# RoyiAvital/QuadraticProgramSolver

Hardware: AMD Instinct MI355X
Metric: ADMM iterations/sec (higher is better)
Workload: dtype f64

## Files before the change

### quadraticprogramsolver_amd/csrc/k_loop.hip

```cpp
#include <cstdlib>

#include "qps_kernels.h"
#include "wave_reduce.h"
#include <hip/hip_ext.h>

namespace qps {

namespace {

template <typename T> __device__ __forceinline__ T wave_sum(T v) { return wave_sum_all(v); }
__device__ __forceinline__ unsigned long long absbits(double v) { return (unsigned long long)__double_as_longlong(fabs(v)); }
__device__ __forceinline__ unsigned long long wave_max_u64(unsigned long long v) {
#pragma unroll
    for (int o = 32; o > 0; o >>= 1) { unsigned long long t = __shfl_xor(v, o, 64); v = t > v ? t : v; }
    return v;
}

template <typename T, int RB, int TRI, int THREADS>
__global__ __launch_bounds__(THREADS) void k_gemv_rows(const T* __restrict__ S, int64_t ld, const T* __restrict__ v,
                                                   T* __restrict__ out, const T* __restrict__ out0, T alpha, T beta,
                                                   int r0, int c0, int c1, BatchStride bs) {
    using V = typename VecOf<T>::type;
    if (bs.active && !bs.active[blockIdx.y]) return;
    S += (int64_t)blockIdx.y * bs.mat; v += (int64_t)blockIdx.y * bs.vin; out += (int64_t)blockIdx.y * bs.vout;
    if (out0) out0 += (int64_t)blockIdx.y * bs.vout;
    constexpr int VN = VecOf<T>::N;
    constexpr int CHUNK = THREADS * VN;
    const int tid = threadIdx.x;
    const int rb = r0 + (TRI == 1 ? (int)(gridDim.x - 1 - blockIdx.x) : (int)blockIdx.x) * RB;
    int cb = c0, ce = c1;
    if (TRI == 1) ce = min(c1, rb + RB);
    if (TRI == 2) cb = max(c0, rb);
    T acc[RB];
#pragma unroll
    for (int i = 0; i < RB; ++i) acc[i] = T(0);
    const T* Srow = S + (int64_t)rb * ld;
#pragma unroll 4
    for (int c = cb + tid * VN; c < ce; c += CHUNK) {
        const V vv = *reinterpret_cast<const V*>(v + c);
        const T* vp = reinterpret_cast<const T*>(&vv);
#pragma unroll
        for (int i = 0; i < RB; ++i) {
            typedef T NV __attribute__((ext_vector_type(VN)));
            const NV* src = reinterpret_cast<const NV*>(Srow + (int64_t)i * ld + c);
            const NV a = (TRI == 0) ? __builtin_nontemporal_load(src) : *src;
            T ap[VN];
#pragma unroll
            for (int e = 0; e < VN; ++e) ap[e] = a[e];
#pragma unroll
            for (int e = 0; e < VN; ++e) {
                bool ok = true;
                if (TRI == 1) ok = (c + e) <= (rb + i);
                if (TRI == 2) ok = (c + e) >= (rb + i);
                acc[i] += ok ? ap[e] * vp[e] : T(0);
            }
        }
    }
    __shared__ T red[THREADS / 64][RB];
#pragma unroll
    for (int i = 0; i < RB; ++i) acc[i] = wave_sum(acc[i]);
    if ((tid & 63) == 0) {
#pragma unroll
        for (int i = 0; i < RB; ++i) red[tid >> 6][i] = acc[i];
    }
    __syncthreads();
    if (tid < RB) {
        T s = T(0);
#pragma unroll
        for (int w = 0; w < THREADS / 64; ++w) s += red[w][tid];
        T r = alpha * s;
        if (beta != T(0)) r += beta * out0[rb + tid];
        out[rb + tid] = r;
    }
}

constexpr int GC_RT = 32;
template <typename T>
__global__ __launch_bounds__(256) void k_gemv_cols(const T* __restrict__ S, int64_t ld, const T* __restrict__ va,
                                                   const T* __restrict__ vb, T ca, T cb, T* __restrict__ part,
                                                   int64_t part_ld, int ncols) {
    using V = typename VecOf<T>::type;
    constexpr int VN = VecOf<T>::N;
    const int c = (blockIdx.x * 256 + threadIdx.x) * VN;
    if (c >= ncols) return;
    const int rt = blockIdx.y;
    const int rbase = rt * GC_RT;
    T acc[VN];
#pragma unroll
    for (int e = 0; e < VN; ++e) acc[e] = T(0);
    const T* Sp = S + (int64_t)rbase * ld + c;
#pragma unroll 8
    for (int i = 0; i < GC_RT; ++i) {
        T w = ca * va[rbase + i];
        if (vb) w += cb * vb[rbase + i];
        typedef T NV __attribute__((ext_vector_type(VN)));
        const NV a = __builtin_nontemporal_load(reinterpret_cast<const NV*>(Sp + (int64_t)i * ld));
#pragma unroll
        for (int e = 0; e < VN; ++e) acc[e] += a[e] * w;
    }
    V o;
    T* op = reinterpret_cast<T*>(&o);
#pragma unroll
    for (int e = 0; e < VN; ++e) op[e] = acc[e];
    *reinterpret_cast<V*>(part + (int64_t)rt * part_ld + c) = o;
}

template <typename T>
__global__ __launch_bounds__(256) void k_colsum(const T* __restrict__ part, int64_t part_ld, int ntiles,
                                                const T* __restrict__ a0, T s0, const T* __restrict__ a1, T s1,
                                                T* __restrict__ out, int ncols, BatchStride bs) {
    using V = typename VecOf<T>::type;
    constexpr int VN = VecOf<T>::N;
    if (bs.active && !bs.active[blockIdx.y]) return;
    part += (int64_t)blockIdx.y * bs.mat; out += (int64_t)blockIdx.y * bs.vout;
    if (a0) a0 += (int64_t)blockIdx.y * bs.vin;
    if (a1) a1 += (int64_t)blockIdx.y * bs.vin;
    constexpr int COLS = 128 / (int)sizeof(T);
    constexpr int CL = COLS / VN;
    constexpr int TL = 256 / CL;
    const int cl = threadIdx.x % CL, tl = threadIdx.x / CL;
    const int c = blockIdx.x * COLS + cl * VN;
    T acc[VN];
#pragma unroll
    for (int e = 0; e < VN; ++e) acc[e] = T(0);
    if (c < ncols) {
        int t = tl;
        for (; t + 7 * TL < ntiles; t += 8 * TL) {
            V v[8];
#pragma unroll
            for (int j = 0; j < 8; ++j) v[j] = *reinterpret_cast<const V*>(part + (int64_t)(t + TL * j) * part_ld + c);
#pragma unroll
            for (int j = 0; j < 8; ++j) {
                const T* vp = reinterpret_cast<const T*>(&v[j]);
#pragma unroll
                for (int e = 0; e < VN; ++e) acc[e] += vp[e];
            }
        }
        for (; t < ntiles; t += TL) {
            const V v = *reinterpret_cast<const V*>(part + (int64_t)t * part_ld + c);
            const T* vp = reinterpret_cast<const T*>(&v);
#pragma unroll
            for (int e = 0; e < VN; ++e) acc[e] += vp[e];
        }
    }
    __shared__ T red[TL][COLS + 1];
#pragma unroll
    for (int e = 0; e < VN; ++e) red[tl][cl * VN + e] = acc[e];
    __syncthreads();
    constexpr int PL = 256 / COLS;
    static_assert(TL % PL == 0 && (PL == 16 || PL == 8), "slab lanes per output");
    const int o = threadIdx.x / PL, pl = threadIdx.x % PL;
    T s = T(0);
#pragma unroll
    for (int k = 0; k < TL / PL; ++k) s += red[pl * (TL / PL) + k][o];
    s = (PL == 16) ? row16_sum_last(s) : oct_sum_all(s);
    const int oc = blockIdx.x * COLS + o;
    if (pl == PL - 1 && oc < ncols) {
        T r = s;
        if (a0) r += s0 * a0[oc];
        if (a1) r += s1 * a1[oc];
        out[oc] = r;
    }
}

template <typename T>
__global__ __launch_bounds__(256) void k_admm_update(int NP, int MP, const T* __restrict__ xx, const T* __restrict__ zz,
                                                     T* __restrict__ x, T* __restrict__ xp, T* __restrict__ z,
                                                     T* __restrict__ zp, T* __restrict__ y, const T* __restrict__ l,
                                                     const T* __restrict__ u, T alpha, T rho) {
    const int i = blockIdx.x * 256 + threadIdx.x;
    const T alpha1 = T(1) - alpha, rho1 = T(1) / rho;
    if (i < NP) {
        const T xo = x[i];
        xp[i] = xo;
        x[i] = alpha * xx[i] + alpha1 * xo;
    }
    if (i < MP) {
        const T zo = z[i], yo = y[i], zt = zz[i];
        zp[i] = zo;
        T t = alpha * zt + alpha1 * zo + rho1 * yo;
        const T lo = l[i], hi = u[i];
        const T zn = t > hi ? hi : (t < lo ? lo : t);
        z[i] = zn;
        y[i] = yo + rho * (alpha * zt + alpha1 * zo - zn);
    }
}

template <typename T>
__global__ __launch_bounds__(256) void k_check_norms(int n, int m, const T* __restrict__ Ax, const T* __restrict__ Px,
                                                     const T* __restrict__ Aty, const T* __restrict__ q,
                                                     const T* __restrict__ x, const T* __restrict__ xp,
                                                     const T* __restrict__ z, const T* __restrict__ zp,
                                                     unsigned long long* __restrict__ slots, int dual_only, BatchStride bs) {
    if (bs.active && !bs.active[blockIdx.y]) return;
    {
        const int64_t on = (int64_t)blockIdx.y * bs.vin, om = (int64_t)blockIdx.y * bs.vout;
        Ax += om; z += om; zp += om; Px += on; Aty += on; q += on; x += on; xp += on; slots += (int64_t)blockIdx.y * 16;
    }
    unsigned long long v[9];
#pragma unroll
    for (int k = 0; k < 9; ++k) v[k] = 0ull;
    for (int i = blockIdx.x * 256 + threadIdx.x; i < max(n, m); i += gridDim.x * 256) {
        if (i < m && !dual_only) {
            const double ax = (double)Ax[i], zi = (double)z[i];
            v[0] = max(v[0], absbits((double)(Ax[i] - z[i])));
            v[2] = max(v[2], absbits(ax));
            v[3] = max(v[3], absbits(zi));
            v[8] = max(v[8], absbits((double)(z[i] - zp[i])));
        }
        if (i < n) {
            v[1] = max(v[1], absbits((double)(Px[i] + q[i] + Aty[i])));
            v[4] = max(v[4], absbits((double)Px[i]));
            v[5] = max(v[5], absbits((double)Aty[i]));
            v[6] = max(v[6], absbits((double)q[i]));
            if (!dual_only) v[7] = max(v[7], absbits((double)(x[i] - xp[i])));
        }
    }
#pragma unroll
    for (int k = 0; k < 9; ++k) {
        v[k] = wave_max_u64(v[k]);
        if ((threadIdx.x & 63) == 0 && v[k] != 0ull) atomicMax(&slots[k], v[k]);
    }
}

__device__ __forceinline__ double jmax(double a, double b) { return (isnan(a) || isnan(b)) ? (double)NAN : (a > b ? a : b); }

__global__ void k_check_decide(const unsigned long long* __restrict__ slots, double* __restrict__ res, CheckScalars cs,
                               const double* __restrict__ rho_arr, const double* __restrict__ rhorho_arr,
                               const int* __restrict__ active) {
    if (threadIdx.x != 0) return;
    const int b = blockIdx.x;
    if (active && !active[b]) return;
    slots += (int64_t)b * 16; res += (int64_t)b * 8;
    if (rho_arr) { cs.rho = rho_arr[b]; cs.rhorho = rhorho_arr[b]; cs.convFlag = 1; }
    double nv[9];
    for (int k = 0; k < 9; ++k) nv[k] = __longlong_as_double((long long)slots[k]);
    const double MIN_VAL_RHO = 1e-3, MAX_VAL_RHO = 1e6;
    const double normResPrim = nv[0], normResDual = nv[1];
    const double maxNormPrim = jmax(nv[2], nv[3]);
    const double maxNormDual = jmax(jmax(nv[4], nv[5]), nv[6]);
    double rhorho = cs.rhorho;
    if (cs.adptRho) {
        const double numeratorVal = normResPrim * maxNormDual;
        const double denominatorVal = normResDual * maxNormPrim;
        const double t = cs.rho * sqrt(numeratorVal / denominatorVal);
        rhorho = t > MAX_VAL_RHO ? MAX_VAL_RHO : (t < MIN_VAL_RHO ? MIN_VAL_RHO : t);
    }
    const double epsPrim = cs.epsAbs + cs.epsRel * maxNormPrim;
    const double epsDual = cs.epsAbs + cs.epsRel * maxNormDual;
    int flag = cs.convFlag;
    if ((normResPrim < epsPrim) && (normResDual < epsDual)) flag = 3;
    if ((nv[7] <= cs.epsAdmm) && (nv[8] <= cs.epsAdmm)) flag = 2;
    res[0] = normResPrim; res[1] = normResDual; res[2] = maxNormPrim; res[3] = maxNormDual;
    res[4] = rhorho; res[5] = (double)flag; res[6] = nv[7]; res[7] = nv[8];
}

template <typename T> __global__ void k_fill(T* p, int64_t n, T v) {
    int64_t i = (int64_t)blockIdx.x * 256 + threadIdx.x;
    if (i < n) p[i] = v;
}
template <typename T> __global__ void k_convert(const double* __restrict__ s, T* __restrict__ d, int64_t n) {
    int64_t i = (int64_t)blockIdx.x * 256 + threadIdx.x;
    if (i < n) d[i] = (T)s[i];
}
template <typename T> __global__ void k_convert_back(const T* __restrict__ s, double* __restrict__ d, int64_t n) {
    int64_t i = (int64_t)blockIdx.x * 256 + threadIdx.x;
    if (i < n) d[i] = (double)s[i];
}

}

static int env_int(const char* name, int dflt) { const char* e = getenv(name); return e ? atoi(e) : dflt; }

template <typename T, int RB, int TH>
static void gemv_rows_launch(hipStream_t st, const T* S, int64_t ld, const T* v, T* out, const T* out0, T alpha, T beta, int r0,
                             int r1, int c0, int c1, int tri, BatchStride bs) {
    dim3 grid((r1 - r0 + RB - 1) / RB, bs.count);
#define QPS_GR(TRI) hipLaunchKernelGGL((k_gemv_rows<T, RB, TRI, TH>), grid, dim3(TH), 0, st, S, ld, v, out, out0, alpha, beta, r0, c0, c1, bs)
    if (tri == 0) QPS_GR(0); else if (tri == 1) QPS_GR(1); else QPS_GR(2);
#undef QPS_GR
}

template <typename T>
void gemv_rows(hipStream_t st, const T* S, int64_t ld, const T* v, T* out, const T* out0, T alpha, T beta, int r0, int r1,
               int c0, int c1, int tri, BatchStride bs) {
    if (r1 <= r0) return;
    static const int wide_th = env_int("QPS_GEMV_WIDE_THREADS", 512);
    static const int wide_rb = env_int("QPS_GEMV_WIDE_RB", 2);
    const bool wide = (c1 - c0) >= 4 * 256 * VecOf<T>::N;
    if (!wide) { gemv_rows_launch<T, 4, 256>(st, S, ld, v, out, out0, alpha, beta, r0, r1, c0, c1, tri, bs); return; }
#define QPS_W(RB, TH) gemv_rows_launch<T, RB, TH>(st, S, ld, v, out, out0, alpha, beta, r0, r1, c0, c1, tri, bs)
    if (wide_th == 512) { if (wide_rb == 4) QPS_W(4, 512); else QPS_W(VecOf<T>::N == 2 ? 2 : 4, 512); }
    else if (wide_th == 256) { if (wide_rb == 4) QPS_W(4, 256); else QPS_W(VecOf<T>::N == 2 ? 2 : 4, 256); }
    else { if (wide_rb == 4) QPS_W(4, 1024); else QPS_W(VecOf<T>::N == 2 ? 2 : 4, 1024); }
#undef QPS_W
}

int gemv_cols_tiles(int nrows) { return (nrows + GC_RT - 1) / GC_RT; }

template <typename T>
int gemv_cols_partial(hipStream_t st, const T* S, int64_t ld, const T* va, const T* vb, T ca, T cb, T* part,
                      int64_t part_ld, int nrows, int ncols) {
    constexpr int VN = VecOf<T>::N;
    const int tiles = gemv_cols_tiles(nrows);
    if (tiles == 0) return 0;
    dim3 grid((ncols + 256 * VN - 1) / (256 * VN), tiles), block(256);
    hipLaunchKernelGGL((k_gemv_cols<T>), grid, block, 0, st, S, ld, va, vb, ca, cb, part, part_ld, ncols);
    return tiles;
}

template <typename T>
void colsum(hipStream_t st, const T* part, int64_t part_ld, int ntiles, const T* a0, T s0, const T* a1, T s1, T* out,
            int ncols, BatchStride bs) {
    constexpr int cols_wg = 128 / (int)sizeof(T);
    if (g_launch_timing.start) {
        const LaunchTiming lt = g_launch_timing;
        g_launch_timing = LaunchTiming();
        hipExtLaunchKernelGGL((k_colsum<T>), dim3((ncols + cols_wg - 1) / cols_wg, bs.count), dim3(256), 0, st, lt.start, lt.stop, 0, part, part_ld, ntiles, a0, s0, a1, s1, out, ncols, bs);
        return;
    }
    hipLaunchKernelGGL((k_colsum<T>), dim3((ncols + cols_wg - 1) / cols_wg, bs.count), dim3(256), 0, st, part, part_ld, ntiles, a0, s0, a1, s1, out, ncols, bs);
}

template <typename T>
void admm_update(hipStream_t st, int NP, int MP, const T* xx, const T* zz, T* x, T* xp, T* z, T* zp, T* y, const T* l,
                 const T* u, T alpha, T rho) {
    const int N = NP > MP ? NP : MP;
    hipLaunchKernelGGL((k_admm_update<T>), dim3((N + 255) / 256), dim3(256), 0, st, NP, MP, xx, zz, x, xp, z, zp, y, l, u, alpha, rho);
}

template <typename T>
void check_convergence(hipStream_t st, int n, int m, const T* Ax, const T* Px, const T* Aty, const T* q, const T* x,
                       const T* xp, const T* z, const T* zp, unsigned long long* scratch, double* res_dev, CheckScalars cs,
                       int dual_only, BatchStride bs, const double* rho_arr, const double* rhorho_arr) {
    if (!dual_only) (void)hipMemsetAsync(scratch, 0, 16 * sizeof(unsigned long long) * bs.count, st);
    const int N = n > m ? n : m;
    int blocks = (N + 255) / 256;
    if (blocks > 1024) blocks = 1024;
    if (blocks < 1) blocks = 1;
    hipLaunchKernelGGL((k_check_norms<T>), dim3(blocks, bs.count), dim3(256), 0, st, n, m, Ax, Px, Aty, q, x, xp, z, zp, scratch, dual_only, bs);
    hipLaunchKernelGGL(k_check_decide, dim3(bs.count), dim3(64), 0, st, scratch, res_dev, cs, rho_arr, rhorho_arr, bs.active);
}

template <typename T> void fill(hipStream_t st, T* p, int64_t n, T v) {
    if (n <= 0) return;
    hipLaunchKernelGGL((k_fill<T>), dim3((unsigned)((n + 255) / 256)), dim3(256), 0, st, p, n, v);
}
template <typename T> void convert_copy(hipStream_t st, const double* src, T* dst, int64_t n) {
    if (n <= 0) return;
    hipLaunchKernelGGL((k_convert<T>), dim3((unsigned)((n + 255) / 256)), dim3(256), 0, st, src, dst, n);
}
template <typename T> void convert_back(hipStream_t st, const T* src, double* dst, int64_t n) {
    if (n <= 0) return;
    hipLaunchKernelGGL((k_convert_back<T>), dim3((unsigned)((n + 255) / 256)), dim3(256), 0, st, src, dst, n);
}

#define INST(T)                                                                                                              \
    template void gemv_rows<T>(hipStream_t, const T*, int64_t, const T*, T*, const T*, T, T, int, int, int, int, int, BatchStride); \
    template int gemv_cols_partial<T>(hipStream_t, const T*, int64_t, const T*, const T*, T, T, T*, int64_t, int, int);      \
    template void colsum<T>(hipStream_t, const T*, int64_t, int, const T*, T, const T*, T, T*, int, BatchStride);            \
    template void admm_update<T>(hipStream_t, int, int, const T*, const T*, T*, T*, T*, T*, T*, const T*, const T*, T, T);   \
    template void check_convergence<T>(hipStream_t, int, int, const T*, const T*, const T*, const T*, const T*, const T*,    \
                                       const T*, const T*, unsigned long long*, double*, CheckScalars, int, BatchStride,     \
                                       const double*, const double*);                                                        \
    template void fill<T>(hipStream_t, T*, int64_t, T);                                                                      \
    template void convert_copy<T>(hipStream_t, const double*, T*, int64_t);                                                  \
    template void convert_back<T>(hipStream_t, const T*, double*, int64_t);
INST(double)
INST(float)
#undef INST

}
```

### quadraticprogramsolver_amd/csrc/k_pass_kernel.h

```cpp
#pragma once
#include <cstdlib>

#include "qps_kernels.h"
#include "wave_reduce.h"
#include <hip/hip_ext.h>

namespace qps {

namespace {

__device__ __forceinline__ unsigned long long absbits(double v) { return (unsigned long long)__double_as_longlong(fabs(v)); }
__device__ __forceinline__ unsigned long long umax(unsigned long long a, unsigned long long b) { return a > b ? a : b; }

template <typename T, int THREADS, int KC, int R, bool CHECK>
struct Pass {
    using V = typename VecOf<T>::type;
    static constexpr int VN = VecOf<T>::N;
    static constexpr int CHUNK = THREADS * VN;
    static constexpr int WAVES = THREADS / 64;

    static __device__ __forceinline__ void load_tile(V (&a)[R][KC], const T* __restrict__ A, int64_t ld, int row, int NP, int tid) {
#pragma unroll
        for (int i = 0; i < R; ++i)
#pragma unroll
            for (int k = 0; k < KC; ++k) {
                const int c = tid * VN + k * CHUNK;
                if (c < NP) {
                    typedef T NV __attribute__((ext_vector_type(VN)));
                    const NV t = __builtin_nontemporal_load(reinterpret_cast<const NV*>(A + (int64_t)(row + i) * ld + c));
                    T* p = reinterpret_cast<T*>(&a[i][k]);
#pragma unroll
                    for (int e = 0; e < VN; ++e) p[e] = t[e];
                }
                else {
                    T* p = reinterpret_cast<T*>(&a[i][k]);
#pragma unroll
                    for (int e = 0; e < VN; ++e) p[e] = T(0);
                }
            }
    }
};

template <typename T, int THREADS, int KC, int R, bool CHECK, int MODE>
__global__ __launch_bounds__(THREADS) void k_apass(const T* __restrict__ A, int64_t ld, int NP, int MP, int rows_per_wg,
                                                   const T* __restrict__ xx, const T* __restrict__ x_old, T* __restrict__ x_new,
                                                   T* __restrict__ z, T* __restrict__ y, const T* __restrict__ l,
                                                   const T* __restrict__ u, T alpha, T rho, T* __restrict__ part,
                                                   T* __restrict__ part2, int64_t part_ld, unsigned long long* __restrict__ slots,
                                                   PassBatch pb) {
    using PS = Pass<T, THREADS, KC, R, CHECK>;
    if (pb.count > 1 || pb.active) {
        const int b = blockIdx.y;
        if (pb.active && !pb.active[b]) return;
        A += (int64_t)b * MP * ld; xx += (int64_t)b * NP; x_old += (int64_t)b * NP; x_new += (int64_t)b * NP;
        z += (int64_t)b * MP; y += (int64_t)b * MP; l += (int64_t)b * MP; u += (int64_t)b * MP;
        part += (int64_t)b * pb.slabs * part_ld; part2 += (int64_t)b * pb.slabs * part_ld; slots += (int64_t)b * 16;
        if (pb.rho_arr) rho = (T)pb.rho_arr[b];
    }
    using V = typename PS::V;
    constexpr int VN = PS::VN, CHUNK = PS::CHUNK, WAVES = PS::WAVES;
    const int tid = threadIdx.x, g = blockIdx.x;
    const int row0 = g * rows_per_wg;
    const int row1 = min(MP, row0 + rows_per_wg);
    const T alpha1 = T(1) - alpha, rho1 = T(1) / rho;

    __shared__ T red[WAVES][R];
    __shared__ T red2[WAVES][R];
    __shared__ T wsh[R];
    __shared__ T ysh[R];

    V xv[KC];
    V xn[CHECK ? KC : 1];
    unsigned long long mdx = 0ull;
#pragma unroll
    for (int k = 0; k < KC; ++k) {
        const int c = tid * VN + k * CHUNK;
        T* xp_ = reinterpret_cast<T*>(&xv[k]);
        if (c < NP) {
            xv[k] = *reinterpret_cast<const V*>(xx + c);
            if (CHECK) {
                const V xo = *reinterpret_cast<const V*>(x_old + c);
                const T* xop = reinterpret_cast<const T*>(&xo);
                V xnv;
                T* xnp = reinterpret_cast<T*>(&xnv);
#pragma unroll
                for (int e = 0; e < VN; ++e) {
                    xnp[e] = alpha * xp_[e] + alpha1 * xop[e];
                    if (CHECK) mdx = umax(mdx, absbits((double)(xnp[e] - xop[e])));
                }
                if (g == 0) *reinterpret_cast<V*>(x_new + c) = xnv;
                if (CHECK) xn[k] = xnv;
            }
        } else {
#pragma unroll
            for (int e = 0; e < VN; ++e) xp_[e] = T(0);
            if (CHECK) { T* q_ = reinterpret_cast<T*>(&xn[k]);
#pragma unroll
                for (int e = 0; e < VN; ++e) q_[e] = T(0); }
        }
    }
    if (CHECK && g == 0) {
#pragma unroll
        for (int o = 32; o > 0; o >>= 1) mdx = umax(mdx, (unsigned long long)__shfl_xor(mdx, o, 64));
        if ((tid & 63) == 0 && mdx) atomicMax(&slots[7], mdx);
    }

    T acc[KC][VN];
    T acc2[CHECK ? KC : 1][VN];
#pragma unroll
    for (int k = 0; k < KC; ++k)
#pragma unroll
        for (int e = 0; e < VN; ++e) { acc[k][e] = T(0); if (CHECK) acc2[k][e] = T(0); }

    unsigned long long m_res = 0ull, m_ax = 0ull, m_z = 0ull, m_dz = 0ull;

    V bufA[R][KC], bufB[R][KC];
    T zA = T(0), yA = T(0), lA = T(0), uA = T(0), zB = T(0), yB = T(0), lB = T(0), uB = T(0);

    auto prefetch_rows = [&](int row, T& zo, T& yo, T& lo, T& hi) {
        if (tid < R) { zo = z[row + tid]; yo = y[row + tid]; lo = l[row + tid]; hi = u[row + tid]; }
    };
    auto process = [&](V (&a)[R][KC], int row, T zo, T yo, T lo, T hi) {
        T d[R], d2[CHECK ? R : 1];
#pragma unroll
        for (int i = 0; i < R; ++i) {
            T s = T(0), s2 = T(0);
#pragma unroll
            for (int k = 0; k < KC; ++k) {
                const T* ap = reinterpret_cast<const T*>(&a[i][k]);
                const T* xp_ = reinterpret_cast<const T*>(&xv[k]);
                const T* xq_ = reinterpret_cast<const T*>(&xn[CHECK ? k : 0]);
#pragma unroll
                for (int e = 0; e < VN; ++e) { s += ap[e] * xp_[e]; if (CHECK) s2 += ap[e] * xq_[e]; }
            }
            d[i] = wave_sum_all(s);
            if (CHECK) d2[i] = wave_sum_all(s2);
        }
        if ((tid & 63) == 0) {
#pragma unroll
            for (int i = 0; i < R; ++i) { red[tid >> 6][i] = d[i]; if (CHECK) red2[tid >> 6][i] = d2[i]; }
        }
        __syncthreads();
        if (tid < R) {
            T zt = T(0), ax = T(0);
#pragma unroll
            for (int w = 0; w < WAVES; ++w) { zt += red[w][tid]; if (CHECK) ax += red2[w][tid]; }
            T zn, yn;
            if (MODE == 0) {
                const T t = alpha * zt + alpha1 * zo + rho1 * yo;
                zn = t > hi ? hi : (t < lo ? lo : t);
                yn = yo + rho * (alpha * zt + alpha1 * zo - zn);
                wsh[tid] = rho * zn - yn;
            } else if (MODE == 2) {
                zn = lo * zt - alpha * (lo * yo);
                yn = yo;
                wsh[tid] = lo * yo;
            } else {
                const T gb = lo, vr = zt;
                if (row + tid < pb.pq_me) {
                    zn = T(0);
                    yn = yo - rho * gb; yn += rho * vr;
                    wsh[tid] = rho * gb - yn;
                } else {
                    T sv = gb - rho1 * yo; sv += -vr; zn = sv > T(0) ? sv : T(0);
                    T zz_ = yo + rho * (zn - gb); zz_ += rho * vr; yn = zz_ > T(0) ? zz_ : T(0);
                    wsh[tid] = rho * (gb - zn) - yn;
                }
            }
            z[row + tid] = zn;
            if (MODE != 2) y[row + tid] = yn;
            if (CHECK) {
                ysh[tid] = yn;
                m_res = umax(m_res, absbits((double)(ax - zn)));
                m_ax = umax(m_ax, absbits((double)ax));
                m_z = umax(m_z, absbits((double)zn));
                m_dz = umax(m_dz, absbits((double)(zn - zo)));
            }
        }
        __syncthreads();
#pragma unroll
        for (int i = 0; i < R; ++i) {
            const T w = wsh[i];
            const T yw = CHECK ? ysh[i] : T(0);
#pragma unroll
            for (int k = 0; k < KC; ++k) {
                const T* ap = reinterpret_cast<const T*>(&a[i][k]);
#pragma unroll
                for (int e = 0; e < VN; ++e) { acc[k][e] += ap[e] * w; if (CHECK) acc2[k][e] += ap[e] * yw; }
            }
        }
    };

    if (row0 < row1) {
        PS::load_tile(bufA, A, ld, row0, NP, tid);
        prefetch_rows(row0, zA, yA, lA, uA);
    }
    for (int row = row0; row < row1; row += 2 * R) {
        const bool haveB = row + R < row1;
        if (haveB) { PS::load_tile(bufB, A, ld, row + R, NP, tid); prefetch_rows(row + R, zB, yB, lB, uB); }
        process(bufA, row, zA, yA, lA, uA);
        if (haveB) {
            if (row + 2 * R < row1) { PS::load_tile(bufA, A, ld, row + 2 * R, NP, tid); prefetch_rows(row + 2 * R, zA, yA, lA, uA); }
            process(bufB, row + R, zB, yB, lB, uB);
        }
    }

    if (!CHECK && MODE != 2 && g == 0) {
        V xo[KC];
#pragma unroll
        for (int k = 0; k < KC; ++k) xo[k] = *reinterpret_cast<const V*>(x_old + min(tid * VN + k * CHUNK, NP - VN));
#pragma unroll
        for (int k = 0; k < KC; ++k) {
            const int c = tid * VN + k * CHUNK;
            if (c < NP) {
                const T* xp_ = reinterpret_cast<const T*>(&xv[k]);
                const T* xop = reinterpret_cast<const T*>(&xo[k]);
                V xnv; T* xnp = reinterpret_cast<T*>(&xnv);
#pragma unroll
                for (int e = 0; e < VN; ++e) xnp[e] = alpha * xp_[e] + alpha1 * xop[e];
                *reinterpret_cast<V*>(x_new + c) = xnv;
            }
        }
    }

#pragma unroll
    for (int k = 0; k < KC; ++k) {
        const int c = tid * VN + k * CHUNK;
        if (c < NP) {
            V o; T* op = reinterpret_cast<T*>(&o);
#pragma unroll
            for (int e = 0; e < VN; ++e) op[e] = acc[k][e];
#if QPS_NT_SLABS
            { typedef T NVS __attribute__((ext_vector_type(VN))); NVS ov;
#pragma unroll
              for (int e = 0; e < VN; ++e) ov[e] = op[e];
              __builtin_nontemporal_store(ov, reinterpret_cast<NVS*>(part + (int64_t)g * part_ld + c)); }
#else
            *reinterpret_cast<V*>(part + (int64_t)g * part_ld + c) = o;
#endif
            if (CHECK) {
#pragma unroll
                for (int e = 0; e < VN; ++e) op[e] = acc2[k][e];
                *reinterpret_cast<V*>(part2 + (int64_t)g * part_ld + c) = o;
            }
        }
    }
    if (CHECK && tid < R) {
        if (m_res) atomicMax(&slots[0], m_res);
        if (m_ax) atomicMax(&slots[2], m_ax);
        if (m_z) atomicMax(&slots[3], m_z);
        if (m_dz) atomicMax(&slots[8], m_dz);
    }
}

template <typename T, int THREADS, int KC, int R, int RC, int MODE>
void launch_pass(hipStream_t st, bool check, int G, const T* A, int64_t ld, int NP, int MP, int rows_per_wg, const T* xx,
                 const T* x_old, T* x_new, T* z, T* y, const T* l, const T* u, T alpha, T rho, T* part, T* part2,
                 int64_t part_ld, unsigned long long* slots, PassBatch pb) {
    if constexpr (MODE == 0) {
        if (check) {
            if (g_launch_timing.start) {
                const LaunchTiming lt = g_launch_timing;
                g_launch_timing = LaunchTiming();
                hipExtLaunchKernelGGL((k_apass<T, THREADS, KC, RC, true, 0>), dim3(G, pb.count), dim3(THREADS), 0, st, lt.start, lt.stop, 0, A, ld, NP, MP, rows_per_wg, xx, x_old, x_new, z, y, l, u, alpha, rho, part, part2, part_ld, slots, pb);
            } else {
                hipLaunchKernelGGL((k_apass<T, THREADS, KC, RC, true, 0>), dim3(G, pb.count), dim3(THREADS), 0, st, A, ld, NP, MP, rows_per_wg, xx, x_old, x_new, z, y, l, u, alpha, rho, part, part2, part_ld, slots, pb);
            }
            return;
        }
    }
    if (g_launch_timing.start) {
        const LaunchTiming lt = g_launch_timing;
        g_launch_timing = LaunchTiming();
        hipExtLaunchKernelGGL((k_apass<T, THREADS, KC, R, false, MODE>), dim3(G, pb.count), dim3(THREADS), 0, st, lt.start, lt.stop, 0, A, ld, NP, MP, rows_per_wg, xx, x_old, x_new, z, y, l, u, alpha, rho, part, part2, part_ld, slots, pb);
        return;
    }
    hipLaunchKernelGGL((k_apass<T, THREADS, KC, R, false, MODE>), dim3(G, pb.count), dim3(THREADS), 0, st, A, ld, NP, MP, rows_per_wg, xx, x_old, x_new, z, y, l, u, alpha, rho, part, part2, part_ld, slots, pb);
}

}

}
```

### quadraticprogramsolver_amd/csrc/k_sparse.hip

```cpp
#include <algorithm>

#include "qps_internal.h"
#include "qps_kernels.h"
#include "qps_ldl.h"
#include "qps_polish.h"
#include "qps_proxqp.h"
#include "k_proxqp_rows.h"
#include "wave_reduce.h"
#include "spmv_layout.h"
#include <hip/hip_ext.h>

namespace qps {

namespace {

struct CgState { double res2, prev2, tol, uc; int iters, done, maxiter, pad; };
using layout::STREAM_NNZ;

__device__ __forceinline__ double block_sum_256(double v, double* sh) {
    v = wave_sum_all(v);
    if ((threadIdx.x & 63) == 0) sh[threadIdx.x >> 6] = v;
    __syncthreads();
    const double r = sh[0] + sh[1] + sh[2] + sh[3];
    __syncthreads();
// ... 487 lines not shown
    const int row = (prow ? blockIdx.x : blockIdx.x - nbn) * 256 + threadIdx.x;
    double d = 0.0;
    if (row < (prow ? n : m)) {
        const T* p0 = pp + (prow ? 0 : n) + row;
        T s = T(0);
#pragma unroll 8
        for (int b = 0; b < nblk; ++b) s += p0[(int64_t)b * stride];
        if (prow) { const T ui = u[row]; pu[row] = s; d = (double)ui * ((double)s + (double)sigma * (double)ui); }
        else { v[row] = s; d = (double)rho * (double)s * (double)s; }
    }
    d = block_sum_256(d, sh);
    if (threadIdx.x == 0) part_uc[blockIdx.x] = d;
}
template <typename T>
__global__ __launch_bounds__(256) void k_cg_combine_update(int n, const T* __restrict__ pu, const T* __restrict__ pat, int nblk, int64_t stride, T rho, T sigma,
                                                           const T* __restrict__ u, int nparts_uc, const double* __restrict__ part_uc, T* __restrict__ x,
                                                           T* __restrict__ r, double* __restrict__ part_rr, const CgState* __restrict__ st) {
    if (st->done) return;
    __shared__ double sh[4];
    double uc = 0.0;
    for (int i = threadIdx.x; i < nparts_uc; i += 256) uc += part_uc[i];
    uc = block_sum_256(uc, sh);
    const T alpha = (T)(st->res2 / uc);
    const int i = blockIdx.x * 256 + threadIdx.x;
    double d = 0.0;
    if (i < n) {
        T s = T(0);
#pragma unroll 8
        for (int b = 0; b < nblk; ++b) s += pat[(int64_t)b * stride + i];
        const T ui = u[i];
        const T c = pu[i] + rho * s + sigma * ui;
        x[i] += alpha * ui;
        const T ri = r[i] - alpha * c;
        r[i] = ri;
        d = (double)ri * (double)ri;
    }
    d = block_sum_256(d, sh);
    if (threadIdx.x == 0) part_rr[blockIdx.x] = d;
}

template <typename T>
__global__ __launch_bounds__(256) void k_cg_init(int n, const T* __restrict__ b, const T* __restrict__ c, T* __restrict__ r,
                                                 T* __restrict__ u, double* __restrict__ partial) {
    __shared__ double sh[4];
    const int i = blockIdx.x * 256 + threadIdx.x;
    double d = 0.0;
    if (i < n) { const T ri = b[i] - c[i]; r[i] = ri; u[i] = T(0); d = (double)ri * (double)ri; }
    d = block_sum_256(d, sh);
    if (threadIdx.x == 0) partial[blockIdx.x] = d;
}
__global__ __launch_bounds__(256) void k_cg_init_final(int nparts, const double* __restrict__ partial, CgState* st, double abstol, double reltol, int maxiter) {
    __shared__ double sh[4];
    double d = 0.0;
    for (int i = threadIdx.x; i < nparts; i += 256) d += partial[i];
    d = block_sum_256(d, sh);
    if (threadIdx.x == 0) {
        const double residual = sqrt(d);
        st->res2 = d; st->prev2 = 1.0;
        st->tol = fmax(reltol * residual, abstol);
        st->iters = 0; st->maxiter = maxiter;
        st->done = (!(residual <= st->tol) && 0 < maxiter) ? 0 : 1;
    }
}
template <typename T>
__global__ __launch_bounds__(256) void k_cg_update_xr(int n, int nparts_uc, const double* __restrict__ partial_uc,
                                                      const T* __restrict__ u, const T* __restrict__ c, T* __restrict__ x,
                                                      T* __restrict__ r, double* __restrict__ partial_rr, const CgState* __restrict__ st) {
    if (st->done) return;
    __shared__ double sh[4];
    double uc = 0.0;
    for (int i = threadIdx.x; i < nparts_uc; i += 256) uc += partial_uc[i];
    uc = block_sum_256(uc, sh);
    const T alpha = (T)(st->res2 / uc);
    const int i = blockIdx.x * 256 + threadIdx.x;
    double d = 0.0;
    if (i < n) {
        x[i] += alpha * u[i];
        const T ri = r[i] - alpha * c[i];
        r[i] = ri;
        d = (double)ri * (double)ri;
    }
    d = block_sum_256(d, sh);
    if (threadIdx.x == 0) partial_rr[blockIdx.x] = d;
}
__global__ __launch_bounds__(256) void k_cg_finish(int nparts, const double* __restrict__ partial_rr, CgState* st) {
    if (st->done) return;
    __shared__ double sh[4];
    double d = 0.0;
    for (int i = threadIdx.x; i < nparts; i += 256) d += partial_rr[i];
    d = block_sum_256(d, sh);
    if (threadIdx.x == 0) {
        st->prev2 = st->res2; st->res2 = d; st->iters += 1;
        const double residual = sqrt(d);
        if (residual <= st->tol || st->iters >= st->maxiter) st->done = 1;
    }
}
template <typename T>
__global__ __launch_bounds__(256) void k_cg_next_u(int n, int nparts, const double* __restrict__ partial_rr, const T* __restrict__ r,
                                                   T* __restrict__ u, const CgState* __restrict__ cur, CgState* __restrict__ nxt, int first) {
    __shared__ double sh[4];
    if (cur->done) { if (blockIdx.x == 0 && threadIdx.x == 0) *nxt = *cur; return; }
    double res2 = cur->res2, prev2 = cur->prev2; int iters = cur->iters, done = 0;
    if (!first) {
        double d = 0.0;
        for (int i = threadIdx.x; i < nparts; i += 256) d += partial_rr[i];
        d = block_sum_256(d, sh);
        prev2 = res2; res2 = d; iters += 1;
        if (sqrt(d) <= cur->tol || iters >= cur->maxiter) done = 1;
    }
    if (blockIdx.x == 0 && threadIdx.x == 0) {
        CgState s = *cur; s.res2 = res2; s.prev2 = prev2; s.iters = iters; s.done = done; *nxt = s;
    }
    if (done) return;
    const T beta = (T)(res2 / prev2);
    const int i = blockIdx.x * 256 + threadIdx.x;
    if (i < n) u[i] = r[i] + beta * u[i];
}
template <typename T>
__global__ __launch_bounds__(256) void k_axpby(int n, T a, const T* __restrict__ x, T b, const T* __restrict__ y, T* __restrict__ out) {
    const int i = blockIdx.x * 256 + threadIdx.x;
    if (i < n) out[i] = a * x[i] + b * y[i];
}

template <typename T>
__global__ __launch_bounds__(256) void k_build_reduced(int64_t nnz, const T* __restrict__ vP, const T* __restrict__ vAA, const T* __restrict__ dg, T sigma, T rho, T* __restrict__ out) {
    const int64_t i = (int64_t)blockIdx.x * 256 + threadIdx.x;
    if (i < nnz) out[i] = vP[i] + sigma * dg[i] + rho * vAA[i];
}
template <typename T>
__global__ __launch_bounds__(256) void k_refresh_values(int64_t count, const int* __restrict__ src, const T* __restrict__ va, T* __restrict__ dst) {
    const int64_t i = (int64_t)blockIdx.x * 256 + threadIdx.x;
    if (i < count) { const int k = src[i]; dst[i] = k >= 0 ? va[k] : T(0); }
}

struct Csr {
    int nrows = 0; int64_t nnz = 0; int* rp = nullptr; int* ci = nullptr; void* va = nullptr; int* rb = nullptr; int nblocks = 0;
    bool blocked = false; int ncols = 0, nblk = 0, wpb = 0; int* brp = nullptr; unsigned short* bci = nullptr; void* bva = nullptr;
    int* task_ptr = nullptr; int4* tasks = nullptr; int per = 1, lpr4 = 0; void* partial = nullptr;
    int* lr_ptr = nullptr; int4* lr_desc = nullptr;
    bool sell = false; int nsl = 0, win = layout::SIGMA, nwin = 0, staged = 0; int* wg_ptr = nullptr; int* sl_off = nullptr; unsigned short* sl_perm = nullptr; void* s_cols = nullptr; void* s_vals = nullptr;
    int* src = nullptr; int64_t src_n = 0; int* lsrc = nullptr; int64_t lsrc_n = 0;
};

template <typename T> struct SparseSolver : SolverBase {
    StreamLease lease; DeviceOwner mem; std::unique_ptr<StagedUploader> up;
    Csr A, At, P, PA;
    Csr Lm; T *L_vP = nullptr, *L_vAA = nullptr, *L_dg = nullptr;
    int explicit_state = 0;
    bool cg_explicit = false; bool L_valid = false; double L_rho = 0, L_sigma = 0; int num_L_builds = 0;
    T *q = nullptr, *l = nullptr, *u = nullptr, *x = nullptr, *xp = nullptr, *z = nullptr, *zp = nullptr, *y = nullptr;
    T *xx = nullptr, *zz = nullptr, *w = nullptr, *tt = nullptr, *cu = nullptr, *cu2 = nullptr, *cr = nullptr, *cc = nullptr, *tm = nullptr;
    T *Ax = nullptr, *Px = nullptr, *Aty = nullptr;
    double *part_uc = nullptr, *part_rr = nullptr; int part_uc_cap = 0; CgState* state = nullptr; CgState* state_host = nullptr;
    unsigned long long* scratch = nullptr; double* res_dev = nullptr; double* res_host = nullptr; double* stage = nullptr;
    int nb_n = 0, nb_op = 0; int64_t cg_total = 0; int last_cg = 4;
    double eps_pcg = 1e-6; int itr_pcg = 1000;
    int cat_spmv, cat_op, cat_vec, cat_chk, cat_ldl, cat_pa = 0, cat_at = 0; int prof_calls = 0;
    std::vector<int64_t> hPcp, hPri, hAcp, hAri; std::vector<double> hPnz, hAnz;
    std::unique_ptr<SparseLdl<T>> ldl; bool ldl_valid = false; double ldl_rho = 0, ldl_sigma = 0; int plugin_kind = QPS_LINSYS_CG;
    int num_factorizations = 0; bool ldl_unfit = false;
    struct IterGraph { double rho, sigma, alpha; hipGraphExec_t exec; };
    std::vector<IterGraph> graphs; bool graphs_disabled = false;
    void drop_graphs() { for (auto& gr : graphs) (void)hipGraphExecDestroy(gr.exec); graphs.clear(); }
    hipGraphExec_t iter_graph(double rho, double sigma, double alpha) {
        for (auto& gr : graphs) if (gr.rho == rho && gr.sigma == sigma && gr.alpha == alpha) return gr.exec;
        if (graphs_disabled) return nullptr;
        if (graphs.size() >= 8) drop_graphs();
        hipGraph_t graph = nullptr; hipGraphExec_t exec = nullptr;
        if (hipStreamBeginCapture(st, hipStreamCaptureModeThreadLocal) != hipSuccess) { (void)hipGetLastError(); graphs_disabled = true; return nullptr; }
        ldl->iterate(x, xp, q, z, zp, y, l, u, alpha, rho, sigma, true);
        if (hipStreamEndCapture(st, &graph) != hipSuccess || graph == nullptr) { (void)hipGetLastError(); graphs_disabled = true; return nullptr; }
        const hipError_t e = hipGraphInstantiate(&exec, graph, nullptr, nullptr, 0);
        (void)hipGraphDestroy(graph);
        if (e != hipSuccess) { (void)hipGetLastError(); graphs_disabled = true; return nullptr; }
        graphs.push_back({rho, sigma, alpha, exec});
        return exec;
    }

    template <typename V> V* upload_array(const std::vector<V>& v, int64_t min_count = 1) {
        V* d = mem.dalloc<V>(std::max<int64_t>((int64_t)v.size(), min_count), st);
        if (!v.empty()) up->copy(d, v.data(), sizeof(V) * v.size());
        return d;
    }
    void build_blocked(Csr& M, const layout::CsrHost& H, bool with_src = false) {
        static const int wgs_env = [] { const char* e = getenv("QPS_SPMV_WGS"); return e ? atoi(e) : 0; }();
        const int wgs = wgs_env > 0 ? wgs_env : 512;
        M.ncols = H.ncols;
        const char* e = getenv("QPS_SPMV_SELL");
        if (!(e && atoi(e) == 0)) {
            layout::SellLayout<T> L;
            const char* es = getenv("QPS_SPMV_STAGED");
            if (layout::build_sell<T>(H, wgs, L, with_src, !(es && atoi(es) == 0))) {
                M.nblk = L.nblk; M.nsl = L.nsl; M.wpb = L.wpb; M.win = L.win; M.nwin = L.nwin; M.staged = L.staged;
                if (with_src) { M.src = upload_array(L.src); M.src_n = (int64_t)L.src.size(); M.lsrc = upload_array(L.lsrc); M.lsrc_n = (int64_t)L.lsrc.size(); }
                M.s_cols = upload_array(L.cols); M.s_vals = upload_array(L.vals);
                M.bci = upload_array(L.lci); M.bva = upload_array(L.lva);
                M.sl_off = upload_array(L.sl_off); M.sl_perm = upload_array(L.perm); M.wg_ptr = upload_array(L.wg_ptr);
                M.lr_ptr = upload_array(L.lr_ptr); M.lr_desc = reinterpret_cast<int4*>(upload_array(L.lr));
                M.partial = mem.dalloc<T>((int64_t)L.nblk * H.nrows + 64, st);
                M.blocked = true; M.sell = true;
                return;
            }
        }
        layout::TaskLayout<T> L;
        try { layout::build_tasks<T>(H, wgs, L, with_src); }
        catch (const std::length_error& ex) { throw QpsError(QPS_ERR_BAD_DIMENSION, ex.what()); }
        M.nblk = L.nblk; M.wpb = L.wpb; M.per = L.per; M.lpr4 = L.lpr4;
        if (with_src) { M.src = upload_array(L.src); M.src_n = (int64_t)L.src.size(); }
        M.brp = upload_array(L.brp); M.bci = upload_array(L.bci); M.bva = upload_array(L.bva);
        M.task_ptr = upload_array(L.task_ptr); M.tasks = reinterpret_cast<int4*>(upload_array(L.tasks));
        M.lr_ptr = upload_array(L.lr_ptr); M.lr_desc = reinterpret_cast<int4*>(upload_array(L.lr));
        M.partial = mem.dalloc<T>((int64_t)L.nblk * H.nrows + 64, st);
        M.blocked = true;
    }
    void upload_csr(Csr& M, const layout::CsrHost& H, bool with_src = false) {
        M.nrows = H.nrows; M.nnz = (int64_t)H.ci.size();
        {
            const char* e = getenv("QPS_SPMV_BLOCKED");
            const int64_t nblk_ = (H.ncols + BlkOf<T>::CB - 1) / BlkOf<T>::CB;
            const bool want = e ? atoi(e) != 0 : (M.nnz >= 200000 && nblk_ * (int64_t)H.nrows <= M.nnz);
            if (want && H.nrows > 0 && H.ncols > 0) build_blocked(M, H, with_src);
        }
        M.rp = upload_array(H.rp); M.ci = upload_array(H.ci);
        {
            std::vector<T> v(H.va.begin(), H.va.end());
            M.va = upload_array(v);
        }
        const std::vector<int> rbv = layout::stream_row_blocks(H);
        M.nblocks = (int)rbv.size() - 1;
        M.rb = upload_array(rbv);
    }
    void upload_vec(const double* h, T* d, int64_t count) { HIPC(upload_staged<T>(st, stage, h, d, count)); }
    void download_vec(const T* d, double* h, int64_t count) { HIPC(download_staged<T>(st, stage, d, h, count)); }
    bool explicit_prepare(bool forced) {
        if (explicit_state != 0) {
            if (forced && explicit_state < 0) throw QpsError(QPS_ERR_UNSUPPORTED, "QPS_LINSYS_CG_EXPLICIT: the reduced matrix of this handle cannot be formed (too many entries, or the handle's "
                                                                                  "host copies were released to the direct plugin before the first CG request)");
            return explicit_state > 0;
        }
        explicit_state = -1;
        if (hPcp.empty() || hAcp.empty()) { if (forced) return explicit_prepare(true); return false; }
        const int64_t pnnz = (int64_t)hPri.size(), annz = (int64_t)hAri.size();
        layout::CsrHost Ph, Ah, Ath, Lh; std::vector<double> vAA, dg;
        try {
            Ph = layout::csc_as_transposed_csr(n, n, hPcp, hPri, hPnz);
            layout::csc_to_csr_pair(m, n, hAcp, hAri, hAnz, Ah, Ath);
            if (!forced && layout::ata_work(Ah) > 16 * (pnnz + annz)) return false;
            const int64_t cap = forced ? 1900000000LL : (3 * (pnnz + 2 * annz)) / 2 + n;
            if (!layout::reduced_matrix(Ph, Ah, Ath, cap, Lh, vAA, dg)) { if (forced) return explicit_prepare(true); return false; }
        } catch (const std::length_error& ex) { throw QpsError(QPS_ERR_BAD_DIMENSION, ex.what()); }
        up.reset(new StagedUploader(st));
        upload_csr(Lm, Lh, true);
        std::vector<T> t1(Lh.va.begin(), Lh.va.end()), t2(vAA.begin(), vAA.end()), t3(dg.begin(), dg.end());
        L_vP = upload_array(t1); L_vAA = upload_array(t2); L_dg = upload_array(t3);
        up.reset();
        HIPC(hipStreamSynchronize(st));
        if (dot_parts(Lm) + 64 > part_uc_cap) {
            mem.release(part_uc); part_uc = nullptr;
            part_uc_cap = dot_parts(Lm) + 64; part_uc = mem.dalloc<double>(part_uc_cap, st);
        }
        explicit_state = 1; L_valid = false;
        return true;
    }
    void reduced_values(double rho, double sigma) {
        if (L_valid && L_rho == rho && L_sigma == sigma) return;
        const int64_t nnz = Lm.nnz;
        if (nnz > 0) hipLaunchKernelGGL((k_build_reduced<T>), dim3((unsigned)((nnz + 255) / 256)), dim3(256), 0, st, nnz, L_vP, L_vAA, L_dg, (T)sigma, (T)rho, static_cast<T*>(Lm.va));
        if (Lm.blocked) {
            T* main_vals = static_cast<T*>(Lm.sell ? Lm.s_vals : Lm.bva);
            if (Lm.src_n > 0) hipLaunchKernelGGL((k_refresh_values<T>), dim3((unsigned)((Lm.src_n + 255) / 256)), dim3(256), 0, st, Lm.src_n, Lm.src, static_cast<const T*>(Lm.va), main_vals);
            if (Lm.sell && Lm.lsrc_n > 0)
                hipLaunchKernelGGL((k_refresh_values<T>), dim3((unsigned)((Lm.lsrc_n + 255) / 256)), dim3(256), 0, st, Lm.lsrc_n, Lm.lsrc, static_cast<const T*>(Lm.va), static_cast<T*>(Lm.bva));
        }
        L_valid = true; L_rho = rho; L_sigma = sigma; ++num_L_builds;
    }
    int resolve_cg(int linsys, double rho, double sigma) {
        const char* e = getenv("QPS_CG_EXPLICIT");
        cg_explicit = linsys == QPS_LINSYS_CG_EXPLICIT ? explicit_prepare(true) : (!(e && atoi(e) == 0) && explicit_prepare(false));
        if (cg_explicit) reduced_values(rho, sigma);
        return QPS_LINSYS_CG;
    }
    int resolve_kind(int linsys, double rho, double sigma, bool force) {
        int kind = linsys;
        if (linsys == QPS_LINSYS_AUTO) kind = qps_linsys_auto(n, m, P.nnz, A.nnz, 1);
        if (kind != QPS_LINSYS_KKT_LDL) return resolve_cg(linsys, rho, sigma);
        if (ldl_unfit && linsys == QPS_LINSYS_AUTO) return resolve_cg(linsys, rho, sigma);
        try { ldl_prepare(rho, sigma, force); }
        catch (const QpsError& e) {
            if (linsys == QPS_LINSYS_AUTO && e.code == QPS_ERR_UNSUPPORTED) { ldl_unfit = true; return resolve_cg(linsys, rho, sigma); }
            throw;
        }
        return QPS_LINSYS_KKT_LDL;
    }
    void ldl_prepare(double rho, double sigma, bool force) {
        if (!ldl) {
            if (n + m > 2000000000LL) throw QpsError(QPS_ERR_BAD_DIMENSION, "KKT matrix too large for the sparse direct plugin");
            const char *e1 = getenv("QPS_LDL_MAX_TAIL"), *e2 = getenv("QPS_LDL_MIN_LEVEL"), *e3 = getenv("QPS_LDL_MAX_LEVELS");
            const int max_tail = e1 ? atoi(e1) : 8192, min_level = e2 ? atoi(e2) : 64, max_levels = e3 ? atoi(e3) : 4096;
            LdlSymbolic sym;
            try { sym = ldl_analyze((int)n, (int)m, hPcp.data(), hPri.data(), hAcp.data(), hAri.data(), 0, max_tail, min_level, max_levels); }
            catch (const std::runtime_error& e) { throw QpsError(QPS_ERR_UNSUPPORTED, e.what()); }
            ldl = make_sparse_ldl<T>(st, std::move(sym), hPnz.data(), (int64_t)hPnz.size(), hAnz.data(), (int64_t)hAnz.size());
            ldl_valid = false;
            for (auto* v : {&hPcp, &hPri, &hAcp, &hAri}) std::vector<int64_t>().swap(*v);
            std::vector<double>().swap(hPnz); std::vector<double>().swap(hAnz);
        }
        if (force || !ldl_valid || ldl_rho != rho || ldl_sigma != sigma) {
            ldl_valid = false;
            ++num_factorizations;
            ldl->factorize(rho, sigma);
            ldl_valid = true; ldl_rho = rho; ldl_sigma = sigma;
        }
    }

    SparseSolver(int dev, int64_t n_, int64_t m_, int dt, const int64_t* Pcp, const int64_t* Pri, const double* Pnz,
                 const int64_t* Acp, const int64_t* Ari, const double* Anz, const double* qh, const double* lh, const double* uh, int base) {
        device = dev; n = n_; m = m_; dtype = dt; sparse = true;
        HIPC(hipSetDevice(device));
        st = prof.st = lease.acquire(device);
        void* const pinned = lease.res.pinned;
        up.reset(new StagedUploader(st));
        if (Pcp[n] - base > 2000000000LL || Acp[n] - base > 2000000000LL) throw QpsError(QPS_ERR_BAD_DIMENSION, "more than 2^31 non-zeros");
        layout::canonical_csc(n, Pcp, Pri, Pnz, base, hPcp, hPri, hPnz);
        layout::canonical_csc(n, Acp, Ari, Anz, base, hAcp, hAri, hAnz);
        const int64_t pnnz = (int64_t)hPri.size(), annz = (int64_t)hAri.size();
        layout::CsrHost Ph, Ah, Ath;
        try {
            Ph = layout::csc_as_transposed_csr(n, n, hPcp, hPri, hPnz);
            layout::csc_to_csr_pair(m, n, hAcp, hAri, hAnz, Ah, Ath);
        } catch (const std::length_error& ex) { throw QpsError(QPS_ERR_BAD_DIMENSION, ex.what()); }
        upload_csr(P, Ph);
        upload_csr(At, Ath);
        upload_csr(A, Ah);
        const char* fuse_env = getenv("QPS_SPMV_FUSEPA");
        if (m > 0 && P.blocked && A.blocked && At.blocked && pnnz + annz < 2000000000LL && !(fuse_env && atoi(fuse_env) == 0)) {
            const layout::CsrHost Sh = layout::stack_rows(Ph, Ah);
            PA.nrows = (int)(n + m); PA.nnz = pnnz + annz;
            build_blocked(PA, Sh);
        }
        const int64_t nn = n + 64, mm = m + 64;
        q = mem.dalloc<T>(nn, st); x = mem.dalloc<T>(nn, st); xp = mem.dalloc<T>(nn, st); xx = mem.dalloc<T>(nn, st); tt = mem.dalloc<T>(nn, st);
        cu = mem.dalloc<T>(nn, st); cu2 = mem.dalloc<T>(nn, st); cr = mem.dalloc<T>(nn, st); cc = mem.dalloc<T>(nn, st); Px = mem.dalloc<T>(nn, st); Aty = mem.dalloc<T>(nn, st);
        l = mem.dalloc<T>(mm, st); u = mem.dalloc<T>(mm, st); z = mem.dalloc<T>(mm, st); zp = mem.dalloc<T>(mm, st); y = mem.dalloc<T>(mm, st); zz = mem.dalloc<T>(mm, st);
        w = mem.dalloc<T>(mm, st); tm = mem.dalloc<T>(mm, st); Ax = mem.dalloc<T>(mm, st);
        nb_n = (int)((n + 255) / 256);
        part_uc_cap = std::max(std::max(At.nblocks, P.nblocks), nb_n + (int)((m + 255) / 256)) + 64;
        part_uc = mem.dalloc<double>(part_uc_cap, st); part_rr = mem.dalloc<double>(nb_n + 64, st);
        state = reinterpret_cast<CgState*>(mem.dalloc<double>(16, st));
        state_host = reinterpret_cast<CgState*>(pinned);
        scratch = mem.dalloc<unsigned long long>(16, st); res_dev = mem.dalloc<double>(16, st);
        res_host = reinterpret_cast<double*>(static_cast<char*>(pinned) + 128);
        stage = mem.dalloc<double>(std::max(nn, mm) + 64, st);
        upload_vec(qh, q, n); upload_vec(lh, l, m); upload_vec(uh, u, m);
        const double s = sizeof(T);
        auto spmv_bytes = [&](const Csr& M, int cols) { return (double)M.nnz * (s + 4) + M.nrows * 4.0 + s * (M.nrows + cols); };
        cat_spmv = prof.category("spmv(A / A')", 0.5 * (spmv_bytes(A, (int)n) + spmv_bytes(At, (int)m)));
        cat_op = prof.category("cg_iteration(A u, P u + rho A'. + sigma u, axpys)", spmv_bytes(A, (int)n) + spmv_bytes(At, (int)m) + spmv_bytes(P, (int)n) + s * 10.0 * n);
        cat_vec = prof.category("admm_update", s * (3.0 * n + 7.0 * m));
        cat_chk = prof.category("check_convergence", spmv_bytes(A, (int)n) + spmv_bytes(At, (int)m) + spmv_bytes(P, (int)n));
        cat_ldl = prof.category("kkt_ldl_solve(rhs, level sweeps, dense tail, post)", 0.0);
        cat_pa = prof.category("spmv_blk([P;A] u, x block in LDS)", (double)(pnnz + annz) * (s + 4) + (double)(n + m) * 4.0 + s * (double)(n + m + n));
        cat_at = prof.category("spmv_blk(A' v, x block in LDS)", spmv_bytes(At, (int)m));
        up.reset();
    }
    ~SparseSolver() override {
        (void)hipSetDevice(device);
        (void)hipStreamSynchronize(st);
        drop_graphs();
        prof.release_events();
    }

    void spmv(const Csr& M, const T* xin, T* out, T a, const T* v0, T b0, const T* v1, T b1, const CgState* stt,
              const T* dotv = nullptr, double* partial = nullptr) {
        if (M.nblocks <= 0) return;
        if (M.blocked) {
            spmv_blk(M, xin, stt);
            hipLaunchKernelGGL((k_spmv_combine<T>), dim3((M.nrows + 255) / 256), dim3(256), 0, st, M.nrows, static_cast<const T*>(M.partial), M.nblk, (int64_t)M.nrows, a,
                               (const T*)nullptr, 0, (int64_t)0, T(0), v0, b0, v1, b1, out, dotv, partial, stt);
            return;
        }
        hipLaunchKernelGGL((k_spmv_stream<T>), dim3(M.nblocks), dim3(256), 0, st, M.rb, M.rp, M.ci, static_cast<const T*>(M.va), xin, out, a,
                           v0, b0, v1, b1, dotv, partial, stt);
    }
    void spmv_blk(const Csr& M, const T* xin, const CgState* stt, CgFuse<T> fu = CgFuse<T>()) {
        const LaunchTiming lt = g_launch_timing;
        g_launch_timing = LaunchTiming();
        if (M.sell) {
            const SellDims sd{M.nrows, M.ncols, M.nsl, M.wpb, M.win, M.nwin, M.staged};
            using CV = typename SellOf<T>::CV; using V = typename VecOf<T>::type;
            if (lt.start) hipExtLaunchKernelGGL((k_spmv_sell<T>), dim3(M.wpb, M.nblk), dim3(BTHREADS), 0, st, lt.start, lt.stop, 0, sd, M.wg_ptr, M.sl_off, M.sl_perm,
                                                static_cast<const CV*>(M.s_cols), static_cast<const V*>(M.s_vals), M.bci, static_cast<const T*>(M.bva), M.lr_ptr, M.lr_desc, xin,
                                                static_cast<T*>(M.partial), stt, fu);
            else hipLaunchKernelGGL((k_spmv_sell<T>), dim3(M.wpb, M.nblk), dim3(BTHREADS), 0, st, sd, M.wg_ptr, M.sl_off, M.sl_perm, static_cast<const CV*>(M.s_cols),
                                    static_cast<const V*>(M.s_vals), M.bci, static_cast<const T*>(M.bva), M.lr_ptr, M.lr_desc, xin, static_cast<T*>(M.partial), stt, fu);
            return;
        }
#define QPS_BLK(LPR)                                                                                                                        \
        do {                                                                                                                                \
            if (lt.start) hipExtLaunchKernelGGL((k_spmv_blk<T, LPR>), dim3(M.wpb, M.nblk), dim3(BTHREADS), 0, st, lt.start, lt.stop, 0, M.nrows, M.ncols, M.task_ptr, \
                                                M.tasks, M.per, M.brp, M.bci, static_cast<const T*>(M.bva), M.lr_ptr, M.lr_desc, xin, static_cast<T*>(M.partial), stt, fu); \
            else hipLaunchKernelGGL((k_spmv_blk<T, LPR>), dim3(M.wpb, M.nblk), dim3(BTHREADS), 0, st, M.nrows, M.ncols, M.task_ptr, M.tasks, M.per, M.brp, M.bci, \
                                    static_cast<const T*>(M.bva), M.lr_ptr, M.lr_desc, xin, static_cast<T*>(M.partial), stt, fu);             \
        } while (0)
        if (M.lpr4) QPS_BLK(4); else QPS_BLK(8);
#undef QPS_BLK
    }
    int dot_parts(const Csr& M) const { return M.blocked ? (M.nrows + 255) / 256 : M.nblocks; }
    void op_reduced(const T* uin, T* cout, double rho, double sigma, double* partial, const CgState* stt) {
        if (m > 0 && P.blocked && A.blocked && At.blocked) {
            spmv_blk(P, uin, stt);
            spmv(A, uin, tm, T(1), nullptr, T(0), nullptr, T(0), stt);
            spmv_blk(At, tm, stt);
            hipLaunchKernelGGL((k_spmv_combine<T>), dim3(nb_n), dim3(256), 0, st, (int)n, static_cast<const T*>(P.partial), P.nblk, (int64_t)n, T(1),
                               static_cast<const T*>(At.partial), At.nblk, (int64_t)n, (T)rho, uin, (T)sigma, (const T*)nullptr, T(0), cout, partial ? uin : nullptr, partial, stt);
            return;
        }
        spmv(P, uin, cout, T(1), uin, (T)sigma, nullptr, T(0), stt, (m > 0) ? nullptr : uin, (m > 0) ? nullptr : partial);
        if (m > 0) {
            spmv(A, uin, tm, T(1), nullptr, T(0), nullptr, T(0), stt);
            spmv(At, tm, cout, (T)rho, cout, T(1), nullptr, T(0), stt, uin, partial);
        }
    }
    int op_parts() const { return (m > 0 && P.blocked && A.blocked && At.blocked) ? nb_n : (m > 0 ? dot_parts(At) : dot_parts(P)); }

    int cg(double rho, double sigma) {
        CgState* slot[2] = {state, state + 1};
        int cur = 0;
        auto apply_op = [&](const T* uin, T* cout, double* partial, const CgState* stt) {
            if (cg_explicit) spmv(Lm, uin, cout, T(1), nullptr, T(0), nullptr, T(0), stt, partial ? uin : nullptr, partial);
            else op_reduced(uin, cout, rho, sigma, partial, stt);
        };
        const int parts_op = cg_explicit ? dot_parts(Lm) : op_parts();
        const bool fused_pa = PA.blocked && !cg_explicit;
        apply_op(xx, cc, nullptr, nullptr);
        T* ub[2] = {cu, cu2}; int ui = 0;
        hipLaunchKernelGGL((k_cg_init<T>), dim3(nb_n), dim3(256), 0, st, (int)n, tt, cc, cr, ub[ui], part_rr);
        hipLaunchKernelGGL(k_cg_init_final, dim3(1), dim3(256), 0, st, nb_n, part_rr, slot[cur], eps_pcg,
                           sizeof(T) == 8 ? 1.4901161193847656e-08 : 3.4526698300124393e-04, itr_pcg);
        HIPC(hipMemcpyAsync(state_host + 1, slot[cur], sizeof(CgState), hipMemcpyDeviceToHost, st));
        int launched = 0, batch = std::max(1, std::min(last_cg, 64));
        for (;;) {
            for (int b = 0; b < batch; ++b) {
                ProfScope ps(prof, cat_op, 2);
                if (fused_pa) {
                    CgFuse<T> fu; fu.r = cr; fu.uold = ub[ui]; fu.unew = ub[ui ^ 1]; fu.part_rr = part_rr; fu.nparts = nb_n;
                    fu.cur = slot[cur]; fu.nxt = slot[cur ^ 1]; fu.first = b == 0 ? 1 : 0;
                    const bool sample = prof.level == 2 || (prof.level == 1 && b == 0 && launched == 0 && prof_calls % 8 == 0);
                    { ProfLaunchScope ps2(prof, cat_pa, sample ? 1 : 3); spmv_blk(PA, cr, nullptr, fu); }
                    cur ^= 1; ui ^= 1;
                    const T* pp = static_cast<const T*>(PA.partial);
                    const int nb_m = (int)((m + 255) / 256);
                    hipLaunchKernelGGL((k_cg_combine_pa<T>), dim3((unsigned)(nb_n + nb_m)), dim3(256), 0, st, (int)n, (int)m, nb_n, pp, PA.nblk, (int64_t)(n + m), ub[ui],
                                       (T)sigma, (T)rho, cc, tm, part_uc, slot[cur]);
                    { ProfLaunchScope ps2(prof, cat_at, sample ? 1 : 3); spmv_blk(At, tm, slot[cur]); }
                    hipLaunchKernelGGL((k_cg_combine_update<T>), dim3(nb_n), dim3(256), 0, st, (int)n, cc, static_cast<const T*>(At.partial), At.nblk, (int64_t)n, (T)rho,
                                       (T)sigma, ub[ui], nb_n + nb_m, part_uc, xx, cr, part_rr, slot[cur]);
                    continue;
                } else {
                    hipLaunchKernelGGL((k_cg_next_u<T>), dim3(nb_n), dim3(256), 0, st, (int)n, nb_n, part_rr, cr, ub[ui], slot[cur], slot[cur ^ 1], b == 0 ? 1 : 0);
                    cur ^= 1;
                    apply_op(ub[ui], cc, part_uc, slot[cur]);
                }
                hipLaunchKernelGGL((k_cg_update_xr<T>), dim3(nb_n), dim3(256), 0, st, (int)n, parts_op, part_uc, ub[ui], cc, xx, cr, part_rr, slot[cur]);
            }
            hipLaunchKernelGGL(k_cg_finish, dim3(1), dim3(256), 0, st, nb_n, part_rr, slot[cur]);
            launched += batch;
            HIPC(hipMemcpyAsync(state_host, slot[cur], sizeof(CgState), hipMemcpyDeviceToHost, st));
            HIPC(hipStreamSynchronize(st));
            prof.harvest();
            if (state_host->done || launched >= itr_pcg) break;
            {
                const double r0 = std::sqrt(state_host[1].res2), r1 = std::sqrt(state_host->res2), tol = state_host->tol;
                int left = std::max(launched, 1);
                if (r1 > 0 && r0 > r1 && tol > 0 && r1 > tol) {
                    const double per_it = std::log(r0 / r1) / std::max(1, state_host->iters);
                    left = (int)std::ceil(std::log(r1 / tol) / per_it);
                }
                batch = std::max(1, std::min(std::min(std::max(left, 2), std::max(launched, 2)), std::min(64, itr_pcg - launched)));
            }
        }
        last_cg = state_host->iters;
        ++prof_calls;
        cg_total += state_host->iters;
        return state_host->iters;
    }

    void linear_solve(double rho, double sigma) {
        if (plugin_kind == QPS_LINSYS_KKT_LDL) {
            ProfScope ps(prof, cat_ldl, 2);
            ldl->solve(x, q, z, y, rho, sigma, xx, zz);
            return;
        }
        if (m > 0) hipLaunchKernelGGL((k_axpby<T>), dim3((unsigned)((m + 255) / 256)), dim3(256), 0, st, (int)m, (T)rho, z, T(-1), y, w);
        {
            ProfScope ps(prof, cat_spmv, 2);
            if (m > 0) spmv(At, w, tt, T(1), x, (T)sigma, q, T(-1), nullptr);
            else hipLaunchKernelGGL((k_axpby<T>), dim3(nb_n), dim3(256), 0, st, (int)n, (T)sigma, x, T(-1), q, tt);
        }
        cg(rho, sigma);
        {
            ProfScope ps(prof, cat_spmv, 2);
            if (m > 0) spmv(A, xx, zz, T(1), nullptr, T(0), nullptr, T(0), nullptr);
        }
    }

    void solve(double* xh, const qps_params& p, qps_info* info) override {
        HIPC(hipSetDevice(device));
        const double t0 = now_s();
        double rho = p.rho; const double sigma = p.sigma, alpha = p.alpha;
        eps_pcg = p.epsPcg; itr_pcg = p.numItrPcg;
        const double epsAdmm = std::fmin(p.epsAbs, p.epsRel) * 1e-2;
        int convFlag = QPS_CONV_NUM_ITR;
        if (p.linsys == QPS_LINSYS_CHOLESKY) throw QpsError(QPS_ERR_UNSUPPORTED, "CSR handles offer QPS_LINSYS_CG, QPS_LINSYS_CG_EXPLICIT and QPS_LINSYS_KKT_LDL (create with dense_path=1 for the reduced Cholesky path)");
        plugin_kind = resolve_kind(p.linsys, rho, sigma, !p.reuseFactor);
        upload_vec(xh, x, n);
        const size_t nb_ = sizeof(T) * (size_t)(n + 64), mb_ = sizeof(T) * (size_t)(m + 64);
        HIPC(hipMemsetAsync(xp, 0, nb_, st)); HIPC(hipMemsetAsync(xx, 0, nb_, st));
        HIPC(hipMemsetAsync(z, 0, mb_, st)); HIPC(hipMemsetAsync(y, 0, mb_, st)); HIPC(hipMemsetAsync(zp, 0, mb_, st));
        HIPC(hipStreamSynchronize(st));
        const double t1 = now_s();
        double rhorho = rho; int ii = 0, nref = 0; double resP = NAN, resD = NAN, tref = 0;
        cg_total = 0; last_cg = 4;
        const int NPv = (int)n, MPv = (int)m;
        static const int graph_env = [] { const char* e = getenv("QPS_GRAPH"); return e ? atoi(e) : -1; }();
        const bool use_graph = plugin_kind == QPS_LINSYS_KKT_LDL && prof.level == 0 && graph_env != 0;
        bool ldl_rhs_ready = false;
        for (ii = 1; ii <= p.numIterations; ++ii) {
            if (p.adptRho && ((rhorho * p.fctrRho < rho) || (rhorho > p.fctrRho * rho))) {
                rho = rhorho; ++nref;
                if (plugin_kind == QPS_LINSYS_CG && cg_explicit) { const double ta = now_s(); reduced_values(rho, sigma); tref += now_s() - ta; }
                if (plugin_kind == QPS_LINSYS_KKT_LDL) { const double ta = now_s(); ldl_prepare(rho, sigma, true); tref += now_s() - ta; ldl_rhs_ready = false; }
            }
            if (plugin_kind == QPS_LINSYS_KKT_LDL && prof.level < 2) {
                if (use_graph && ldl_rhs_ready && ii % p.numItrConv != 0) {
                    hipGraphExec_t ge = iter_graph(rho, sigma, alpha);
                    if (ge) { HIPC(hipGraphLaunch(ge, st)); continue; }
                }
                ldl->iterate(x, xp, q, z, zp, y, l, u, alpha, rho, sigma, ldl_rhs_ready);
                ldl_rhs_ready = true;
            } else {
            linear_solve(rho, sigma);
            {
                ProfScope ps(prof, cat_vec, 2);
                admm_update<T>(st, NPv, MPv, xx, zz, x, xp, z, zp, y, l, u, (T)alpha, (T)rho);
            }
            }
            if (ii % p.numItrConv == 0) {
                {
                    ProfScope ps(prof, cat_chk, 2);
                    if (m > 0) spmv(A, x, Ax, T(1), nullptr, T(0), nullptr, T(0), nullptr);
                    spmv(P, x, Px, T(1), nullptr, T(0), nullptr, T(0), nullptr);
                    if (m > 0) spmv(At, y, Aty, T(1), nullptr, T(0), nullptr, T(0), nullptr);
                    else HIPC(hipMemsetAsync(Aty, 0, nb_, st));
                    CheckScalars cs{p.epsAbs, p.epsRel, epsAdmm, rho, rhorho, p.adptRho, convFlag};
                    check_convergence<T>(st, (int)n, (int)m, Ax, Px, Aty, q, x, xp, z, zp, scratch, res_dev, cs);
                }
                HIPC(hipMemcpyAsync(res_host, res_dev, 8 * sizeof(double), hipMemcpyDeviceToHost, st));
                HIPC(hipStreamSynchronize(st));
                prof.harvest();
                resP = res_host[0]; resD = res_host[1]; rhorho = res_host[4]; convFlag = (int)res_host[5];
                if (convFlag != QPS_CONV_NUM_ITR) break;
            }
        }
        HIPC(hipStreamSynchronize(st));
        prof.harvest();
        const double t2 = now_s();
        PolishReport pr;
        if (p.polish) polish_device(p, &pr);
        download_vec(x, xh, n);
        if (info) {
            info->convFlag = convFlag; info->iterations = ii > p.numIterations ? p.numIterations : ii;
            info->numRefactor = nref; info->cgIterations = (int)cg_total; info->rhoFinal = rho; info->rhoProposed = rhorho;
            info->resPrim = resP; info->resDual = resD; info->tSetup = t1 - t0; info->tLoop = t2 - t1; info->tRefactor = tref;
            info->trsvBlock = 0; info->sweepVariant = 0; info->sweepGaveUp = 0; info->cgExplicit = (plugin_kind == QPS_LINSYS_CG && cg_explicit) ? 1 : 0;
            info->polishFlag = pr.flag; info->polishIterations = pr.minresIterations; info->tPolish = pr.seconds;
        }
    }
    void get_dual(double* zh, double* yh) override {
        HIPC(hipSetDevice(device));
        if (zh) download_vec(z, zh, m);
        if (yh) download_vec(y, yh, m);
    }
    void polish_device(const qps_params& p, PolishReport* pr) {
        PolishProduct<T> kmat = [&](const T* v, T delta, T* out, const T* mask, T* scratch) {
            spmv(P, v, out, T(1), v, delta, nullptr, T(0), nullptr);
            if (m <= 0) return;
            spmv(A, v, out + n, T(1), nullptr, T(0), nullptr, T(0), nullptr);
            polish_mask_rows<T>(st, (int)m, mask, v + n, delta, out + n, scratch);
            spmv(At, scratch, out, T(1), out, T(1), nullptr, T(0), nullptr);
        };
        polish_with<T>(st, n, m, (int)n, (int)m, q, l, u, y, x, p, pr, kmat);
    }
    void polish(double* xh, const double* yh, const qps_params& p, qps_polish_report* rep) override {
        HIPC(hipSetDevice(device));
        upload_vec(xh, x, n); upload_vec(yh, y, m);
        PolishReport pr;
        polish_device(p, &pr);
        download_vec(x, xh, n);
        if (rep) {
            rep->flag = pr.flag; rep->refinements = pr.refinements; rep->minresIterations = pr.minresIterations;
            rep->numActiveLower = pr.numLower; rep->numActiveUpper = pr.numUpper; rep->reserved0 = 0; rep->relres = pr.relres; rep->seconds = pr.seconds;
        }
    }
    void operator_apply(int op, const double* in, double* out, double rho, double sigma) override {
        HIPC(hipSetDevice(device));
        if (op == QPS_OP_AT) {
            upload_vec(in, w, m);
            if (m > 0) spmv(At, w, cc, T(1), nullptr, T(0), nullptr, T(0), nullptr); else HIPC(hipMemsetAsync(cc, 0, sizeof(T) * (size_t)(n + 64), st));
            download_vec(cc, out, n);
            return;
        }
        upload_vec(in, cu, n);
        if (op == QPS_OP_P) { spmv(P, cu, cc, T(1), nullptr, T(0), nullptr, T(0), nullptr); download_vec(cc, out, n); }
        else if (op == QPS_OP_A) { if (m > 0) spmv(A, cu, tm, T(1), nullptr, T(0), nullptr, T(0), nullptr); download_vec(tm, out, m); }
        else if (op == QPS_OP_PA) {
            if (PA.blocked) {
                spmv_blk(PA, cu, nullptr);
                DeviceOwner tmp_mem;
                T* both = tmp_mem.dalloc<T>(n + m + 64, st);
                hipLaunchKernelGGL((k_spmv_combine<T>), dim3((unsigned)((n + m + 255) / 256)), dim3(256), 0, st, (int)(n + m), static_cast<const T*>(PA.partial), PA.nblk, (int64_t)(n + m),
                                   T(1), (const T*)nullptr, 0, (int64_t)0, T(0), (const T*)nullptr, T(0), (const T*)nullptr, T(0), both, (const T*)nullptr, (double*)nullptr, (const CgState*)nullptr);
                download_vec(both, out, n); download_vec(both + n, out + n, m);
            } else {
                spmv(P, cu, cc, T(1), nullptr, T(0), nullptr, T(0), nullptr); download_vec(cc, out, n);
                if (m > 0) spmv(A, cu, tm, T(1), nullptr, T(0), nullptr, T(0), nullptr);
                download_vec(tm, out + n, m);
            }
        } else if (op == QPS_OP_REDUCED) { op_reduced(cu, cc, rho, sigma, nullptr, nullptr); download_vec(cc, out, n); }
        else throw QpsError(QPS_ERR_BAD_ARGUMENT, "unknown qps_operator_kind");
    }
    void linsys_set_cg(double eps, int itr) override { eps_pcg = eps; itr_pcg = itr; }
    void linsys_init(double rho, double sigma, int linsys, int) override {
        HIPC(hipSetDevice(device));
        if (linsys != QPS_LINSYS_AUTO && linsys != QPS_LINSYS_CG && linsys != QPS_LINSYS_KKT_LDL && linsys != QPS_LINSYS_CG_EXPLICIT)
            throw QpsError(QPS_ERR_UNSUPPORTED, "CSR handles offer QPS_LINSYS_CG, QPS_LINSYS_CG_EXPLICIT and QPS_LINSYS_KKT_LDL (create with dense_path=1 for the reduced Cholesky path)");
        plugin_kind = resolve_kind(linsys, rho, sigma, true);
        if (plugin_kind == QPS_LINSYS_KKT_LDL) return;
        HIPC(hipMemsetAsync(xx, 0, sizeof(T) * (size_t)(n + 64), st));
        cg_total = 0; last_cg = 4;
    }
    void linsys_solve(const double* xh, const double* zh, const double* yh, double rho, double sigma, int changed, double* xxh, double* zzh) override {
        HIPC(hipSetDevice(device));
        if (plugin_kind == QPS_LINSYS_KKT_LDL) {
            if (!ldl) throw QpsError(QPS_ERR_BAD_ARGUMENT, "qps_linsys_solve called before qps_linsys_init");
            if (changed) ldl_prepare(rho, sigma, true);
        }
        if (plugin_kind == QPS_LINSYS_CG && cg_explicit) reduced_values(rho, sigma);
        upload_vec(xh, x, n); upload_vec(zh, z, m); upload_vec(yh, y, m);
        linear_solve(rho, sigma);
        HIPC(hipStreamSynchronize(st));
        download_vec(xx, xxh, n); download_vec(zz, zzh, m);
    }
};


template <typename T> struct SparseProxQpSolver : ProxQpBase {
    std::unique_ptr<SparseSolver<T>> ss;
    DeviceOwner mem; hipStream_t st = nullptr;
    int mtot = 0;
    T *g = nullptr, *dual = nullptr, *slack = nullptr, *hvec = nullptr, *x = nullptr, *xx = nullptr, *v = nullptr, *de = nullptr, *di = nullptr;
    T *X1 = nullptr, *X2 = nullptr, *X3 = nullptr, *r1 = nullptr, *r2 = nullptr, *dx = nullptr, *dnu = nullptr, *zero_m = nullptr;
    unsigned long long* slots = nullptr; unsigned long long* slots_host = nullptr;
    std::vector<int64_t> kPcp, kPri, kAcp, kAri; std::vector<double> kPnz, kAnz;

    static dim3 g1(int64_t c) { return dim3((unsigned)((std::max<int64_t>(c, 1) + 255) / 256)); }

    SparseProxQpSolver(int dev, int64_t n_, int64_t me_, int64_t mi_, int dt, const int64_t* Pcp, const int64_t* Pri, const double* Pnz, const double* qh,
                       const int64_t* Acp, const int64_t* Ari, const double* Anz, const double* bh, const int64_t* Ccp, const int64_t* Cri, const double* Cnz,
                       const double* dh, int base) {
        device = dev; n = n_; me = me_; mi = mi_; mtot = (int)(me + mi);
        std::vector<int64_t> Gcp(n + 1, 0), Gri, P0cp(n + 1), P0ri((size_t)(Pcp[n] - base));
        std::vector<double> Gnz;
        for (int64_t j = 0; j <= n; ++j) P0cp[j] = Pcp[j] - base;
        for (size_t k = 0; k < P0ri.size(); ++k) P0ri[k] = Pri[k] - base;
        for (int64_t j = 0; j < n; ++j) {
            if (me > 0) for (int64_t k = Acp[j] - base; k < Acp[j + 1] - base; ++k) { Gri.push_back(Ari[k] - base); Gnz.push_back(Anz[k]); }
            if (mi > 0) for (int64_t k = Ccp[j] - base; k < Ccp[j + 1] - base; ++k) { Gri.push_back(Cri[k] - base + me); Gnz.push_back(Cnz[k]); }
            Gcp[j + 1] = (int64_t)Gri.size();
        }
        std::vector<double> zeros((size_t)std::max(mtot, 1), 0.0), gh((size_t)std::max(mtot, 1), 0.0);
        for (int64_t i = 0; i < me; ++i) gh[i] = bh[i];
        for (int64_t i = 0; i < mi; ++i) gh[me + i] = dh[i];
        static const int64_t dummy_i[1] = {0}; static const double dummy_d[1] = {0.0};
        ss.reset(new SparseSolver<T>(dev, n, mtot, dt, P0cp.data(), P0ri.empty() ? dummy_i : P0ri.data(), Pnz, Gcp.data(), Gri.empty() ? dummy_i : Gri.data(),
                                     Gnz.empty() ? dummy_d : Gnz.data(), qh, zeros.data(), zeros.data(), 0));
        st = ss->st;
        const int64_t nn = n + 64, mm = mtot + 64;
        g = mem.dalloc<T>(mm, st); dual = mem.dalloc<T>(mm, st); slack = mem.dalloc<T>(mm, st); hvec = mem.dalloc<T>(mm, st); v = mem.dalloc<T>(mm, st); de = mem.dalloc<T>(mm, st); di = mem.dalloc<T>(mm, st);
        r2 = mem.dalloc<T>(mm, st); dnu = mem.dalloc<T>(mm, st); zero_m = mem.dalloc<T>(mm, st);
        x = mem.dalloc<T>(nn, st); xx = mem.dalloc<T>(nn, st); X1 = mem.dalloc<T>(nn, st); X2 = mem.dalloc<T>(nn, st); X3 = mem.dalloc<T>(nn, st); r1 = mem.dalloc<T>(nn, st); dx = mem.dalloc<T>(nn, st);
        slots = mem.dalloc<unsigned long long>(16, st);
        slots_host = reinterpret_cast<unsigned long long*>(ss->lease.res.pinned);
        ss->upload_vec(gh.data(), g, mtot);
        layout::canonical_csc(n, P0cp.data(), P0ri.empty() ? dummy_i : P0ri.data(), Pnz, 0, kPcp, kPri, kPnz);
        if (me > 0) layout::canonical_csc(n, Acp, Ari, Anz, base, kAcp, kAri, kAnz);
        else kAcp.assign(n + 1, 0);
    }
    ~SparseProxQpSolver() override {
        (void)hipSetDevice(device);
        (void)hipStreamSynchronize(st);
    }
    void drop_init_copies() {
        for (auto* vv : {&kPcp, &kPri, &kAcp, &kAri}) std::vector<int64_t>().swap(*vv);
        std::vector<double>().swap(kPnz); std::vector<double>().swap(kAnz);
    }
    void set_state(const double* xh, const double* yh, const double* zh, const double* sh) override {
        HIPC(hipSetDevice(device));
        ss->upload_vec(xh, x, n); ss->upload_vec(yh, dual, me); ss->upload_vec(zh, dual + me, mi);
        HIPC(hipMemsetAsync(slack, 0, sizeof(T) * (size_t)(mtot + 64), st));
        ss->upload_vec(sh, slack + me, mi);
// ... 135 lines not shown
```

### quadraticprogramsolver_amd/csrc/k_trsv.hip

```cpp
#include <algorithm>
#include <cstdlib>

#include "qps_kernels.h"
#include "wave_reduce.h"
#include <hip/hip_ext.h>

namespace qps {

namespace {

template <typename T, int THREADS, int KC, int RB, bool DB = true>
__global__ __launch_bounds__(THREADS) void k_sweep_fused(const T* __restrict__ S, int64_t ld, int NP, const T* __restrict__ v,
                                                         T* __restrict__ part, int64_t part_ld, BatchStride bs) {
    using V = typename VecOf<T>::type;
    constexpr int VN = VecOf<T>::N, CHUNK = THREADS * VN, WAVES = THREADS / 64;
    if (bs.active && !bs.active[blockIdx.y]) return;
    S += (int64_t)blockIdx.y * bs.mat; v += (int64_t)blockIdx.y * bs.vin; part += (int64_t)blockIdx.y * bs.vout;
    const int tid = threadIdx.x, G = gridDim.x, g = blockIdx.x;
    const int ntiles = NP / RB;
    __shared__ T red[2][WAVES][RB];

    V xv[KC];
    T acc[KC][VN];
#pragma unroll
    for (int k = 0; k < KC; ++k) {
        const int c = tid * VN + k * CHUNK;
        if (c < NP) xv[k] = *reinterpret_cast<const V*>(v + c);
        else { T* p = reinterpret_cast<T*>(&xv[k]);
#pragma unroll
            for (int e = 0; e < VN; ++e) p[e] = T(0); }
#pragma unroll
        for (int e = 0; e < VN; ++e) acc[k][e] = T(0);
    }
    auto tile_row = [&](int it) { return (ntiles - 1 - (g + it * G)) * RB; };
    auto load = [&](V (&a)[RB][KC], int row) {
#pragma unroll
        for (int i = 0; i < RB; ++i)
#pragma unroll
            for (int k = 0; k < KC; ++k) {
                const int c = tid * VN + k * CHUNK;
                const int cc = min(min(c, (row + i) & ~(VN - 1)), NP - VN);
                a[i][k] = *reinterpret_cast<const V*>(S + (int64_t)(row + i) * ld + cc);
            }
    };
    constexpr bool SKIP = KC <= 2;
    const int wave_col0 = (tid & ~63) * VN;
    auto process = [&](V (&a)[RB][KC], int row, int par) {
#pragma unroll
        for (int i = 0; i < RB; ++i) {
            T s = T(0);
            if (SKIP && wave_col0 > row + i) { if ((tid & 63) == 0) red[par][tid >> 6][i] = T(0); continue; }
#pragma unroll
            for (int k = 0; k < KC; ++k) {
                const int c = tid * VN + k * CHUNK;
                T* ap = reinterpret_cast<T*>(&a[i][k]);
                const T* xp = reinterpret_cast<const T*>(&xv[k]);
#pragma unroll
                for (int e = 0; e < VN; ++e) {
                    if (c + e > row + i) ap[e] = T(0);
                    s += ap[e] * xp[e];
                }
            }
            s = wave_sum_all(s);
            if ((tid & 63) == 0) red[par][tid >> 6][i] = s;
        }
        __syncthreads();
#pragma unroll
        for (int i = 0; i < RB; ++i) {
            static_assert(WAVES <= 8, "one partial per lane of the first eight");
            if (SKIP && wave_col0 > row + i) continue;
            const T y = lanes8_sum_all(((tid & 63) < WAVES) ? red[par][tid & 63][i] : T(0));
#pragma unroll
            for (int k = 0; k < KC; ++k) {
                const T* ap = reinterpret_cast<const T*>(&a[i][k]);
#pragma unroll
                for (int e = 0; e < VN; ++e) acc[k][e] += ap[e] * y;
            }
        }
    };
    const int my_tiles = (ntiles - g + G - 1) / G;
    if constexpr (DB) {
        if (my_tiles > 0) {
            V bufA[RB][KC], bufB[RB][KC];
            load(bufA, tile_row(0));
            for (int it = 0; it < my_tiles; it += 2) {
                const bool haveB = it + 1 < my_tiles;
                load(bufB, tile_row(min(it + 1, my_tiles - 1)));
                process(bufA, tile_row(it), 0);
                load(bufA, tile_row(min(it + 2, my_tiles - 1)));
                if (haveB) process(bufB, tile_row(it + 1), 1);
            }
        }
    } else {
        V buf[RB][KC];
        for (int it = 0; it < my_tiles; ++it) { load(buf, tile_row(it)); process(buf, tile_row(it), it & 1); }
    }
#pragma unroll
    for (int k = 0; k < KC; ++k) {
        const int c = tid * VN + k * CHUNK;
        if (c < NP) {
            V o; T* op = reinterpret_cast<T*>(&o);
#pragma unroll
            for (int e = 0; e < VN; ++e) op[e] = acc[k][e];
#if QPS_NT_SLABS
            { typedef T NVS __attribute__((ext_vector_type(VN))); NVS ov;
#pragma unroll
              for (int e = 0; e < VN; ++e) ov[e] = op[e];
              __builtin_nontemporal_store(ov, reinterpret_cast<NVS*>(part + (int64_t)g * part_ld + c)); }
#else
            *reinterpret_cast<V*>(part + (int64_t)g * part_ld + c) = o;
#endif
        }
    }
}

template <typename T, int KCW, bool DB = true>
__global__ __launch_bounds__(512) void k_sweep_fused_wave(const T* __restrict__ S, int64_t ld, int NP, const T* __restrict__ v,
                                                          T* __restrict__ part, int64_t part_ld, BatchStride bs) {
    using V = typename VecOf<T>::type;
    constexpr int VN = VecOf<T>::N, CH = 64 * VN, WAVES = 8, COLS = KCW * CH;
    if (bs.active && !bs.active[blockIdx.y]) return;
    S += (int64_t)blockIdx.y * bs.mat; v += (int64_t)blockIdx.y * bs.vin; part += (int64_t)blockIdx.y * bs.vout;
    const int tid = threadIdx.x, lane = tid & 63, wave = tid >> 6, g = blockIdx.x;
    const int W = gridDim.x * WAVES, w = wave * gridDim.x + g;
    __shared__ T sh[WAVES][COLS];

    V xv[KCW];
    T acc[KCW][VN];
#pragma unroll
    for (int k = 0; k < KCW; ++k) {
        const int c = k * CH + lane * VN;
        xv[k] = *reinterpret_cast<const V*>(v + min(c, NP - VN));
        if (c >= NP) { T* p = reinterpret_cast<T*>(&xv[k]);
#pragma unroll
            for (int e = 0; e < VN; ++e) p[e] = T(0); }
#pragma unroll
        for (int e = 0; e < VN; ++e) acc[k][e] = T(0);
    }
    auto row_of = [&](int it) { return NP - 1 - (w + it * W); };
    auto load = [&](V (&a)[KCW], int r) {
#pragma unroll
        for (int k = 0; k < KCW; ++k) {
            const int c = k * CH + lane * VN;
            const int cc = min(min(c, r & ~(VN - 1)), NP - VN);
            a[k] = *reinterpret_cast<const V*>(S + (int64_t)r * ld + cc);
        }
    };
    auto process = [&](V (&a)[KCW], int r) {
        T s = T(0);
#pragma unroll
        for (int k = 0; k < KCW; ++k) {
            const int c = k * CH + lane * VN;
            T* ap = reinterpret_cast<T*>(&a[k]);
            const T* xp = reinterpret_cast<const T*>(&xv[k]);
#pragma unroll
            for (int e = 0; e < VN; ++e) {
                if (c + e > r) ap[e] = T(0);
                s += ap[e] * xp[e];
            }
        }
        const T y = wave_sum_all(s);
#pragma unroll
        for (int k = 0; k < KCW; ++k) {
            const T* ap = reinterpret_cast<const T*>(&a[k]);
#pragma unroll
            for (int e = 0; e < VN; ++e) acc[k][e] += ap[e] * y;
        }
    };
    const int mine = w < NP ? (NP - w + W - 1) / W : 0;
    if constexpr (!DB) {
        V buf[KCW];
        for (int it = 0; it < mine; ++it) { load(buf, row_of(it)); process(buf, row_of(it)); }
    } else if (mine > 0) {
        V bufA[KCW], bufB[KCW];
        load(bufA, row_of(0));
        for (int it = 0; it < mine; it += 2) {
            const int rb = row_of(min(it + 1, mine - 1));
            load(bufB, rb);
            process(bufA, row_of(it));
            load(bufA, row_of(min(it + 2, mine - 1)));
            if (it + 1 < mine) process(bufB, rb);
        }
    }
#pragma unroll
    for (int k = 0; k < KCW; ++k)
#pragma unroll
        for (int e = 0; e < VN; ++e) sh[wave][k * CH + lane * VN + e] = acc[k][e];
    __syncthreads();
    for (int c = tid; c < NP; c += 512) {
        T t = T(0);
#pragma unroll
        for (int q = 0; q < WAVES; ++q) t += sh[q][c];
        part[(int64_t)g * part_ld + c] = t;
    }
}

static bool sweep_wave() { static const bool on = [] { const char* e = getenv("QPS_SWEEP_WAVE"); return !(e && atoi(e) == 0); }(); return on; }
template <typename T> static bool sweep_wave_covers(int NP) { return sweep_wave() && NP <= 64 * VecOf<T>::N * 8; }

}

template <typename T> bool sweep_fused_supported(int NP) { return NP <= 16 * 512 * VecOf<T>::N && NP >= 1024; }

static int sweep_rb_env() { static int rb = [] { const char* e = getenv("QPS_SWEEP_RB"); return e ? atoi(e) : 0; }(); return rb; }
static int sweep_rb_for(int kc) {
    int rb = sweep_rb_env() > 0 ? sweep_rb_env() : (kc >= 4 ? 1 : (kc == 2 ? 2 : 4));
    if (rb != 1 && rb != 2 && rb != 4) rb = 2;
    if (kc > 4 && rb == 4) rb = 2;
    return rb;
}

template <typename T> int sweep_fused_slabs(int NP, int count) {
    if (sweep_wave_covers<T>(NP)) {
        const int per = count >= 256 ? 1 : 256 / (count < 1 ? 1 : count);
        return std::max(1, std::min(per, NP / 16));
    }
    const int kc0 = (NP + 512 * VecOf<T>::N - 1) / (512 * VecOf<T>::N);
    int RB = sweep_rb_for(kc0);
    if (NP > 8 * 512 * VecOf<T>::N) RB = 1;
    static const int total_env = [] { const char* e = getenv("QPS_SWEEP_WGS"); return e ? atoi(e) : 0; }();
    const int kc = (NP + 512 * VecOf<T>::N - 1) / (512 * VecOf<T>::N);
    const int total = total_env > 0 ? total_env : (count <= 1 ? 256 : (kc <= 1 ? 1024 : (kc == 2 ? 512 : 256)));
    const int per = count >= total ? 1 : total / count;
    const int ntiles = NP / RB;
    return ntiles < per ? ntiles : per;
}

template <typename T>
int sweep_fused(hipStream_t st, const T* S, int64_t ld, int NP, const T* v, T* part, int64_t part_ld, BatchStride bs) {
    constexpr int TH = 512;
    const int chunk = TH * VecOf<T>::N;
    const int kc = (NP + chunk - 1) / chunk;
    const int G = sweep_fused_slabs<T>(NP, bs.count);
    dim3 grid(G, bs.count);
    const int rb = sweep_rb_for(kc);
    const LaunchTiming lt = g_launch_timing;
    g_launch_timing = LaunchTiming();
    if (sweep_wave_covers<T>(NP)) {
#define QPS_WV(KCW)                                                                                                                \
    do {                                                                                                                           \
        if (lt.start) hipExtLaunchKernelGGL((k_sweep_fused_wave<T, KCW>), grid, dim3(TH), 0, st, lt.start, lt.stop, 0, S, ld, NP, v, part, part_ld, bs); \
        else hipLaunchKernelGGL((k_sweep_fused_wave<T, KCW>), grid, dim3(TH), 0, st, S, ld, NP, v, part, part_ld, bs);              \
    } while (0)
        static const int wave_db = [] { const char* e = getenv("QPS_SWEEP_WAVE_DB"); return e ? atoi(e) : 0; }();
        if (NP <= 64 * VecOf<T>::N * 4) QPS_WV(4);
        else if (wave_db == 0) { if (lt.start) hipExtLaunchKernelGGL((k_sweep_fused_wave<T, 8, false>), grid, dim3(TH), 0, st, lt.start, lt.stop, 0, S, ld, NP, v, part, part_ld, bs); else hipLaunchKernelGGL((k_sweep_fused_wave<T, 8, false>), grid, dim3(TH), 0, st, S, ld, NP, v, part, part_ld, bs); }
        else QPS_WV(8);
#undef QPS_WV
        return G;
    }
#define QPS_S(KC, RB)                                                                                                              \
    do {                                                                                                                           \
        if (lt.start) hipExtLaunchKernelGGL((k_sweep_fused<T, TH, KC, RB>), grid, dim3(TH), 0, st, lt.start, lt.stop, 0, S, ld, NP, v, part, part_ld, bs); \
        else hipLaunchKernelGGL((k_sweep_fused<T, TH, KC, RB>), grid, dim3(TH), 0, st, S, ld, NP, v, part, part_ld, bs);            \
    } while (0)
#define QPS_SW(KC)                                                                                                                 \
    do {                                                                                                                           \
        if (lt.start) hipExtLaunchKernelGGL((k_sweep_fused<T, TH, KC, 1, false>), grid, dim3(TH), 0, st, lt.start, lt.stop, 0, S, ld, NP, v, part, part_ld, bs); \
        else hipLaunchKernelGGL((k_sweep_fused<T, TH, KC, 1, false>), grid, dim3(TH), 0, st, S, ld, NP, v, part, part_ld, bs);      \
    } while (0)
#define QPS_SR(KC) do { if (rb == 1) QPS_S(KC, 1); else if (rb == 2) QPS_S(KC, 2); else QPS_S(KC, 4); } while (0)
    if (kc > 8) { if (kc <= 12) QPS_SW(12); else QPS_SW(16); }
    else if (kc <= 1) QPS_SR(1);
    else if (kc <= 2) QPS_SR(2);
    else if (kc <= 4) QPS_SR(4);
    else { if (rb == 1) QPS_S(8, 1); else QPS_S(8, 2); }
#undef QPS_SR
#undef QPS_SW
#undef QPS_S
    return G;
}

#define INST(T)                                                     \
    template int sweep_fused_slabs<T>(int, int);                    \
    template int sweep_fused<T>(hipStream_t, const T*, int64_t, int, const T*, T*, int64_t, BatchStride); \
    template bool sweep_fused_supported<T>(int);
INST(double)
INST(float)
#undef INST

}
```

### quadraticprogramsolver_amd/csrc/qps_capi.hip

```cpp
#include "ldl_symbolic.h"
#include <atomic>
#include <memory>
#include <thread>

#include "batch_schedule.h"
#include "dense_chol.h"
#include "qps_internal.h"
#include "spmv_layout.h"
#include "qps_kernels.h"
#include "qps_polish.h"
#include "qps_proxqp.h"

using namespace qps;

namespace qps {
namespace {
constexpr size_t kPinnedBytes = 512, kRecycleBlockMax = (size_t)512 << 20;
constexpr int kRecyclePerDevice = 4;
std::mutex g_res_mu;
std::vector<HandleResources> g_res[kMaxDevices];
std::atomic<int> g_cus[kMaxDevices];
}
int current_device() { int dev = 0; if (hipGetDevice(&dev) != hipSuccess) { (void)hipGetLastError(); return 0; } return dev; }
int device_cu_count(int device) {
    if (device < 0 || device >= kMaxDevices) return 0;
    int c = g_cus[device].load(std::memory_order_acquire);
    if (c == 0) {
        if (hipDeviceGetAttribute(&c, hipDeviceAttributeMultiprocessorCount, device) != hipSuccess) { (void)hipGetLastError(); c = -1; }
        g_cus[device].store(c, std::memory_order_release);
    }
    return c > 0 ? c : 0;
}
HandleResources acquire_resources(int device, size_t block_need) {
    HandleResources r;
    {
        std::lock_guard<std::mutex> lk(g_res_mu);
        if (device >= 0 && device < kMaxDevices && !g_res[device].empty()) { r = g_res[device].back(); g_res[device].pop_back(); }
    }
    try {
        if (!r.st) HIPC(hipStreamCreateWithFlags(&r.st, hipStreamNonBlocking));
        if (!r.pinned) HIPC(hipHostMalloc(&r.pinned, kPinnedBytes));
    } catch (...) { recycle_resources(device, r); throw; }
    if (r.block && (r.block_bytes < block_need || r.block_bytes > 4 * block_need + ((size_t)1 << 20))) { (void)hipFree(r.block); r.block = nullptr; r.block_bytes = 0; }
    return r;
}
void recycle_resources(int device, HandleResources r) {
    if (r.block && r.block_bytes > kRecycleBlockMax) { (void)hipFree(r.block); r.block = nullptr; r.block_bytes = 0; }
    {
        std::lock_guard<std::mutex> lk(g_res_mu);
        if (device >= 0 && device < kMaxDevices && (int)g_res[device].size() < kRecyclePerDevice) { g_res[device].push_back(r); return; }
    }
    if (r.block) (void)hipFree(r.block);
    if (r.pinned) (void)hipHostFree(r.pinned);
    if (r.st) (void)hipStreamDestroy(r.st);
}
int host_threads() {
    static const int n = [] {
        const char* e = getenv("QPS_HOST_THREADS");
        const int hw = (int)std::max(1u, std::thread::hardware_concurrency());
        return std::max(1, std::min(e ? atoi(e) : 8, hw));
    }();
    return n;
}
namespace {
constexpr size_t kRingHalf = (size_t)32 << 20;
std::vector<PinnedRing> g_rings[kMaxDevices];
}
PinnedRing acquire_ring(int device) {
    PinnedRing r;
    {
        std::lock_guard<std::mutex> lk(g_res_mu);
        if (device >= 0 && device < kMaxDevices && !g_rings[device].empty()) { r = g_rings[device].back(); g_rings[device].pop_back(); }
    }
    if (!r.base) { HIPC(hipHostMalloc((void**)&r.base, 2 * kRingHalf)); r.half = kRingHalf; }
    return r;
}
void recycle_ring(int device, PinnedRing r) {
    if (!r.base) return;
    {
        std::lock_guard<std::mutex> lk(g_res_mu);
        if (device >= 0 && device < kMaxDevices && (int)g_rings[device].size() < kRecyclePerDevice) { g_rings[device].push_back(r); return; }
    }
    (void)hipHostFree(r.base);
}
thread_local LaunchTiming g_launch_timing;
ProfLaunchScope::ProfLaunchScope(Profiler& pr, int c, int lvl) : p(pr), cat(c), a(nullptr), b(nullptr), active(pr.on(lvl)) {
    if (active) { a = p.get(); b = p.get(); g_launch_timing.start = a; g_launch_timing.stop = b; }
}
ProfLaunchScope::~ProfLaunchScope() {
    if (!active) return;
    const bool consumed = (g_launch_timing.start == nullptr);
    g_launch_timing = LaunchTiming();
    if (consumed) p.pending.push_back({cat, a, b}); else { p.pool.push_back(a); p.pool.push_back(b); }
}
}

namespace {

thread_local std::string g_last_error;

template <typename T> struct DenseSolver : SolverBase {
    int NP = 0, MP = 0;
    T *A = nullptr, *P = nullptr, *q = nullptr, *l = nullptr, *u = nullptr;
    T *PI = nullptr, *AA = nullptr, *M = nullptr, *S = nullptr, *tmp = nullptr, *dinv = nullptr; int* fail = nullptr;
    T *x = nullptr, *xp = nullptr, *z = nullptr, *zp = nullptr, *y = nullptr, *xx = nullptr, *zz = nullptr, *tt = nullptr, *yv = nullptr;
    T *part = nullptr, *part2 = nullptr, *sw_part = nullptr, *Ax = nullptr, *Px = nullptr, *Aty = nullptr;
    T* At = nullptr; void* small_out = nullptr; void* small_out_host = nullptr; bool small_ok = false;
    StreamLease lease; Arena arena;
    double* stage_mat = nullptr; int64_t stage_mat_count = 0;
    int pass_slabs = 0, pass_rpw = 0;
    unsigned long long* scratch = nullptr; double* res_dev = nullptr; double* res_host = nullptr; double* stage = nullptr;
    bool have_AA = false, factor_valid = false; double fac_rho = 0, fac_sigma = 0; int fac_nb = 0;
    int nb = 2048; int part_tiles = 0; int num_factorizations = 0;
    unsigned long long* pub = nullptr; unsigned* abort_dev = nullptr; unsigned sweep_epoch = 0; bool blocked_off = false, fac_premul = false;
    bool use_blocked() const { return !blocked_off && trsv_blocked_supported<T>(NP, nb); }
    struct IterGraph { int count; const void* xa; double rho, sigma, alpha; int nb; hipGraphExec_t exec; };
    std::vector<IterGraph> graphs;
    bool graphs_disabled = false;
    void drop_graphs() { for (auto& gr : graphs) (void)hipGraphExecDestroy(gr.exec); graphs.clear(); }
    hipGraphExec_t iter_graph(int count, T* xa, T* xb, double rho, double sigma, double alpha) {
        for (auto& gr : graphs) if (gr.count == count && gr.xa == xa && gr.rho == rho && gr.sigma == sigma && gr.alpha == alpha && gr.nb == nb) return gr.exec;
        if (graphs_disabled) return nullptr;
        if (graphs.size() >= 8) drop_graphs();
        hipGraph_t graph = nullptr; hipGraphExec_t exec = nullptr;
        if (hipStreamBeginCapture(st, hipStreamCaptureModeThreadLocal) != hipSuccess) { (void)hipGetLastError(); graphs_disabled = true; return nullptr; }
        for (int k = 0; k < count; ++k) {
            colsum<T>(st, part, NP, pass_slabs, xa, (T)sigma, q, T(-1), tt, NP);
            sweeps();
            apass<T>(st, false, A, NP, NP, MP, xx, xa, xb, z, y, l, u, (T)alpha, (T)rho, part, part2, NP, scratch);
            std::swap(xa, xb);
        }
        if (hipStreamEndCapture(st, &graph) != hipSuccess || graph == nullptr) { (void)hipGetLastError(); graphs_disabled = true; return nullptr; }
        const hipError_t e = hipGraphInstantiate(&exec, graph, nullptr, nullptr, 0);
        (void)hipGraphDestroy(graph);
        if (e != hipSuccess) { (void)hipGetLastError(); graphs_disabled = true; return nullptr; }
        graphs.push_back({count, xa, rho, sigma, alpha, nb, exec});
        return exec;
    }
    int prof_iter = 0;
    int sample_lvl(int slot) const { return (prof.level == 1 && prof_iter % 50 == slot) ? 1 : 2; }
    int cat_atw, cat_colsum, cat_fwd, cat_bwd, cat_ax, cat_upd, cat_chk, cat_pass, cat_passchk, cat_sweep, cat_xsum, cat_small;

    DenseSolver(int dev, int64_t n_, int64_t m_, int dt) {
        device = dev; n = n_; m = m_; dtype = dt;
        HIPC(hipSetDevice(device));
        NP = roundup(n, 64); MP = roundup(m, 64);
        const int64_t nn = (int64_t)NP * NP;
        part_tiles = gemv_cols_tiles(MP);
        pass_slabs = apass_plan<T>(NP, MP, &pass_rpw);
        const int slabs = std::max(std::max(part_tiles, pass_slabs), 1);
        small_ok = admm_small_supported<T>((int)n, (int)m, NP, MP);
        stage_mat_count = std::max((int64_t)n * n, (int64_t)m * n);
        if (stage_mat_count > ((int64_t)1 << 20)) stage_mat_count = 0;
        auto layout = [&](Arena& ar) {
            A = ar.take<T>((int64_t)MP * NP); P = ar.take<T>(nn); q = ar.take<T>(NP); l = ar.take<T>(MP); u = ar.take<T>(MP);
            PI = ar.take<T>(nn); AA = ar.take<T>(nn); M = ar.take<T>(nn); S = ar.take<T>(nn); tmp = ar.take<T>(nn);
            dinv = ar.take<T>((int64_t)(NP / 64) * 4096); fail = ar.take<int>(4);
            x = ar.take<T>(NP); xp = ar.take<T>(NP); xx = ar.take<T>(NP); tt = ar.take<T>(NP); yv = ar.take<T>(NP);
            z = ar.take<T>(MP); zp = ar.take<T>(MP); y = ar.take<T>(MP); zz = ar.take<T>(MP);
            part = ar.take<T>((int64_t)slabs * NP);
            part2 = ar.take<T>((int64_t)slabs * NP);
            sw_part = ar.take<T>((int64_t)std::max(sweep_fused_slabs<T>(NP), 1) * NP);
            Ax = ar.take<T>(MP); Px = ar.take<T>(NP); Aty = ar.take<T>(NP);
            scratch = ar.take<unsigned long long>(16); res_dev = ar.take<double>(16);
            pub = ar.take<unsigned long long>(trsv_blocked_pub_words<T>(NP));
            abort_dev = reinterpret_cast<unsigned*>(res_dev + 14);
            stage = ar.take<double>((int64_t)NP + 2 * (int64_t)MP + 64);
            if (small_ok) { At = ar.take<T>((int64_t)NP * MP); small_out = ar.take<double>(32); }
            if (stage_mat_count > 0) stage_mat = ar.take<double>(stage_mat_count);
        };
        layout(arena);
        st = prof.st = lease.acquire(device, arena.planned());
        HandleResources& res = lease.res;
        char* const recycled = res.block; res.block = nullptr;
        arena.commit(st, recycled, res.block_bytes);
        layout(arena);
        res_host = reinterpret_cast<double*>(res.pinned);
        small_out_host = small_ok ? reinterpret_cast<char*>(res.pinned) + 16 * sizeof(double) : nullptr;
        const double s = sizeof(T);
        cat_atw = prof.category("gemv_cols(A'w)", s * ((double)m * n + m + n));
        cat_colsum = prof.category("colsum(rhs)", s * ((double)part_tiles * n + 3.0 * n));
        cat_fwd = prof.category("trsv_forward", s * ((double)n * (n + 1) / 2 + 2.0 * n));
        cat_bwd = prof.category("trsv_backward", s * ((double)n * (n + 1) / 2 + 2.0 * n));
        cat_ax = prof.category("gemv_rows(Ax~)", s * ((double)m * n + m + n));
        cat_upd = prof.category("admm_update", s * (3.0 * n + 7.0 * m));
        cat_chk = prof.category("check_convergence", s * (2.0 * m * n + (double)n * n + 4.0 * n + 4.0 * m));
        cat_pass = prof.category("apass(fused A-pass)", s * ((double)m * n + 3.0 * n + 6.0 * m));
        cat_passchk = prof.category("apass(check variant)", s * ((double)m * n + 4.0 * n + 6.0 * m));
        cat_sweep = prof.category("sweeps(fused fwd+bwd, triangle read once)", s * ((double)n * (n + 1) / 2 + 2.0 * n + (double)sweep_fused_slabs<T>(NP) * n));
        cat_xsum = prof.category("colsum(x~ slabs)", s * ((double)sweep_fused_slabs<T>(NP) * n + n));
        cat_small = prof.category("admm_small(whole loop in one launch; bytes per iteration)", s * ((double)m * n + (double)n * n) + s * (6.0 * n + 10.0 * m));
    }
    ~DenseSolver() override {
        (void)hipSetDevice(device);
        (void)hipStreamSynchronize(st);
        trsv_blocked_forget_stream(device, st);
        drop_graphs();
        prof.release_events();
        lease.res.block = arena.base; lease.res.block_bytes = arena.bytes; arena.base = nullptr;
    }

    void upload_vec(const double* h, T* d, int64_t count) { HIPC(upload_staged<T>(st, stage, h, d, count)); }
    void download_vec(const T* d, double* h, int64_t count) { HIPC(download_staged<T>(st, stage, d, h, count)); }
    void upload_matrix(const double* h, int64_t ldh, int rows, int cols, T* d, int64_t ldd) {
        if (rows <= 0 || cols <= 0) return;
        if (stage_mat && (int64_t)rows * cols <= stage_mat_count) {
            HIPC(hipMemcpy2DAsync(stage_mat, sizeof(double) * (size_t)rows, h, sizeof(double) * (size_t)ldh, sizeof(double) * (size_t)rows, (size_t)cols, hipMemcpyHostToDevice, st));
            import_colmajor<T>(st, stage_mat, rows, rows, cols, d, ldd);
            HIPC(hipStreamSynchronize(st));
            return;
        }
        const int64_t budget = (int64_t)32 << 20;
        int pc = (int)std::max<int64_t>(64, (budget / std::max(rows, 1)) / 64 * 64);
        DeviceOwner tmp_mem;
        double* buf = tmp_mem.alloc<double>((int64_t)rows * std::min(pc, cols));
        FastUploader fu(st, device);
        for (int c0 = 0; c0 < cols; c0 += pc) {
            const int nc = std::min(pc, cols - c0);
            if (ldh == rows) fu.copy(buf, h + (int64_t)c0 * ldh, sizeof(double) * (size_t)rows * (size_t)nc);
            else for (int c = 0; c < nc; ++c) fu.copy(buf + (int64_t)c * rows, h + (int64_t)(c0 + c) * ldh, sizeof(double) * (size_t)rows);
            import_colmajor<T>(st, buf, rows, rows, nc, d + c0, ldd);
            HIPC(hipStreamSynchronize(st));
        }
    }

    DenseChol<T> chol() const { return {st, (int)n, NP, MP, P, A, PI, AA, M, S, tmp, dinv, fail}; }
    void factorize(double rho, double sigma, bool rebuild_all) {
        const bool rebuild = rebuild_all || !have_AA;
        const DenseChol<T> c = chol();
        factor_valid = false;
        c.form(sigma, rho, rebuild, rebuild);
        have_AA = true;
        c.factor(nb, 1, use_blocked());
        char ctx[128]; snprintf(ctx, sizeof ctx, "rho=%g, sigma=%g; factorisation #%d of this handle", rho, sigma, ++num_factorizations);
        int f = 0;
        c.check("P + sigma I + rho A'A", ctx, &f);
        factor_valid = true; fac_rho = rho; fac_sigma = sigma; fac_nb = nb; fac_premul = use_blocked();
    }
    bool sweep_gave_up(bool fetched = false) {
        if (!fac_premul) return false;
        unsigned* h = reinterpret_cast<unsigned*>(res_host + 14);
        if (!fetched) {
            HIPC(hipMemcpyAsync(h, abort_dev, sizeof(unsigned), hipMemcpyDeviceToHost, st));
            HIPC(hipStreamSynchronize(st));
        }
        if (*h == 0u) return false;
        HIPC(hipMemsetAsync(abort_dev, 0, sizeof(unsigned), st));
        blocked_off = true; factor_valid = false;
        return true;
    }

    int sweep_variant() const { const int v = chol_sweep_variant<T>(NP, nb); return (fac_premul && v != 2) ? 5 : v; }
    void sweeps() {
        if (sweep_variant() != 5) {
            chol().sweeps(nb, tt, yv, xx, sw_part, BatchStride(), {&prof, cat_sweep, sample_lvl(13), cat_xsum, sample_lvl(21), cat_fwd, cat_bwd, 2});
            return;
        }
        if (sweep_epoch >= 0xfffffff0u) {
            HIPC(hipMemsetAsync(pub, 0, sizeof(unsigned long long) * (size_t)trsv_blocked_pub_words<T>(NP), st));
            sweep_epoch = 0;
        }
        TrsvBlockedPair gate(device, st);
        { ProfLaunchScope ps(prof, cat_fwd, sample_lvl(13)); trsv_blocked<T>(st, false, S, NP, NP, nb, tt, yv, pub, ++sweep_epoch, abort_dev); }
        { ProfLaunchScope ps(prof, cat_bwd, sample_lvl(21)); trsv_blocked<T>(st, true, S, NP, NP, nb, yv, xx, pub, ++sweep_epoch, abort_dev); }
    }
    void linear_solve(double rho, double sigma) {
        {
            ProfScope ps(prof, cat_atw, 1);
            gemv_cols_partial<T>(st, A, NP, z, y, (T)rho, T(-1), part, NP, MP, NP);
        }
        {
            ProfScope ps(prof, cat_colsum, 2);
            colsum<T>(st, part, NP, part_tiles, x, (T)sigma, q, T(-1), tt, NP);
        }
        sweeps();
        {
            ProfScope ps(prof, cat_ax, 2);
            gemv_rows<T>(st, A, NP, xx, zz, nullptr, T(1), T(0), 0, MP, 0, NP, 0);
        }
    }

    void solve(double* xh, const qps_params& p, qps_info* info) override {
        HIPC(hipSetDevice(device));
        blocked_off = false;
        int gave_up = 0; double t_lost = 0;
        const double t_begin = now_s();
        while (solve_once(xh, p, info)) {
            ++gave_up; t_lost = now_s() - t_begin;
            const int lvl = prof.level; prof.reset(); prof.level = lvl;
        }
        if (info) { info->sweepGaveUp = gave_up; info->cgExplicit = 0; info->tLoop += t_lost; }
    }
    bool solve_once(double* xh, const qps_params& p, qps_info* info) {
        if (p.linsys != QPS_LINSYS_AUTO && p.linsys != QPS_LINSYS_CHOLESKY)
            throw QpsError(QPS_ERR_UNSUPPORTED, "dense handles offer QPS_LINSYS_CHOLESKY only (qps_create_csc with dense_path = 0 for the CG and the sparse L D L' plugins)");
        const double t0 = now_s();
        nb = pick_nb<T>(p.trsvBlock, NP);
        double rho = p.rho, sigma = p.sigma; const double alpha = p.alpha;
        const double epsAdmm = std::fmin(p.epsAbs, p.epsRel) * 1e-2;
        int convFlag = QPS_CONV_NUM_ITR;
        const bool reuse = p.reuseFactor && factor_valid && fac_rho == rho && fac_sigma == sigma && fac_nb == nb && fac_premul == use_blocked();
        if (!reuse) factorize(rho, sigma, !p.reuseFactor || !have_AA || fac_sigma != sigma);
        upload_vec(xh, x, n);
        HIPC(hipMemsetAsync(xp, 0, sizeof(T) * NP, st));
        HIPC(hipMemsetAsync(z, 0, sizeof(T) * std::max(MP, 64), st));
        HIPC(hipMemsetAsync(y, 0, sizeof(T) * std::max(MP, 64), st));
        HIPC(hipMemsetAsync(zp, 0, sizeof(T) * std::max(MP, 64), st));
        HIPC(hipStreamSynchronize(st));
        const double t1 = now_s();
        double rhorho = rho;
        int ii = 0, nref = 0; double tref = 0, resP = NAN, resD = NAN;
        if (small_ok && p.loopVariant == 0 && (NP + nb - 1) / nb == 1) {
            transpose_small<T>(st, A, NP, MP, At);
            int it = 0;
            while (it < p.numIterations) {
                {
                    ProfScope ps(prof, cat_small, 1);
                    admm_small<T>(st, (int)n, (int)m, NP, MP, it, p.numIterations, p.numItrConv, p.adptRho, rho, rhorho, sigma, alpha, p.epsAbs,
                                  p.epsRel, epsAdmm, p.fctrRho, A, At, P, S, q, l, u, x, xp, z, y, small_out);
                }
                HIPC(hipMemcpyAsync(small_out_host, small_out, admm_small_out_bytes(), hipMemcpyDeviceToHost, st));
                HIPC(hipStreamSynchronize(st));
                prof.harvest();
                int last = 0, flag = 1, need = 0; double r8[8];
                admm_small_read(small_out_host, &last, &flag, &need, r8);
                it = last; convFlag = flag; rhorho = r8[4];
                if (!std::isnan(r8[0]) || !std::isnan(r8[1])) { resP = r8[0]; resD = r8[1]; }
                if (flag != QPS_CONV_NUM_ITR) break;
                if (need && it < p.numIterations) {
                    rho = rhorho; ++nref;
                    const double ta = now_s();
                    factorize(rho, sigma, false);
                    tref += now_s() - ta;
                }
            }
            ii = it;
            const double t2s = now_s();
            PolishReport prs;
            if (p.polish) polish_dense<T>(st, n, m, NP, MP, P, A, q, l, u, y, x, part, p, &prs);
            download_vec(x, xh, n);
            if (info) {
                info->convFlag = convFlag; info->iterations = ii; info->numRefactor = nref; info->cgIterations = 0;
                info->rhoFinal = rho; info->rhoProposed = rhorho; info->resPrim = resP; info->resDual = resD;
                info->tSetup = t1 - t0; info->tLoop = t2s - t1; info->tRefactor = tref;
                info->polishFlag = prs.flag; info->polishIterations = prs.minresIterations; info->tPolish = prs.seconds;
                info->trsvBlock = nb; info->sweepVariant = 4;
            }
            return false;
        }
        const bool fused = pass_slabs > 0 && p.loopVariant != 1;
        int rhs_slabs = 0;
        static const int graph_env = [] { const char* e = getenv("QPS_GRAPH"); return e ? atoi(e) : -1; }();
        const bool use_graph = fused && prof.level == 0 && p.numItrConv >= 3 && !fac_premul && (graph_env >= 0 ? graph_env != 0 : NP <= 2048);
        for (ii = 1; ii <= p.numIterations; ++ii) {
            bool changed = false;
            if (p.adptRho && ((rhorho * p.fctrRho < rho) || (rhorho > p.fctrRho * rho))) {
                rho = rhorho; ++nref; changed = true;
                const double ta = now_s();
                factorize(rho, sigma, false);
                tref += now_s() - ta;
            }
            const bool check = (ii % p.numItrConv == 0);
            if (use_graph && !changed && !check && rhs_slabs == pass_slabs) {
                int run = std::min(p.numItrConv - ii % p.numItrConv, p.numIterations - ii + 1) & ~1;
                hipGraphExec_t ge = run >= 2 ? iter_graph(run, x, xp, rho, sigma, alpha) : nullptr;
                if (ge) {
                    HIPC(hipGraphLaunch(ge, st));
                    ii += run - 1;
                    continue;
                }
            }
            if (!fused) {
                linear_solve(rho, sigma);
                {
                    ProfScope ps(prof, cat_upd, 2);
                    admm_update<T>(st, NP, MP, xx, zz, x, xp, z, zp, y, l, u, (T)alpha, (T)rho);
                }
                if (check) {
                    ProfScope ps(prof, cat_chk, 2);
                    gemv_rows<T>(st, A, NP, x, Ax, nullptr, T(1), T(0), 0, MP, 0, NP, 0);
                    gemv_rows<T>(st, P, NP, x, Px, nullptr, T(1), T(0), 0, NP, 0, NP, 0);
                    gemv_cols_partial<T>(st, A, NP, y, nullptr, T(1), T(0), part, NP, MP, NP);
                    colsum<T>(st, part, NP, part_tiles, nullptr, T(0), nullptr, T(0), Aty, NP);
                    CheckScalars cs{p.epsAbs, p.epsRel, epsAdmm, rho, rhorho, p.adptRho, convFlag};
                    check_convergence<T>(st, (int)n, (int)m, Ax, Px, Aty, q, x, xp, z, zp, scratch, res_dev, cs);
                }
            } else {
                if (changed && rhs_slabs > 0) {
                    ProfScope ps(prof, cat_atw, 2);
                    rhs_slabs = gemv_cols_partial<T>(st, A, NP, z, y, (T)rho, T(-1), part, NP, MP, NP);
                }
                prof_iter = ii;
                {
                    ProfLaunchScope ps(prof, cat_colsum, sample_lvl(29));
                    colsum<T>(st, part, NP, rhs_slabs, x, (T)sigma, q, T(-1), tt, NP);
                }
                sweeps();
                if (check) HIPC(hipMemsetAsync(scratch, 0, 16 * sizeof(unsigned long long), st));
                {
                    const int lvl = (prof.level == 1 && (check || ii % 50 != 38)) ? 3 : 1;
                    ProfLaunchScope ps(prof, check ? cat_passchk : cat_pass, lvl);
                    apass<T>(st, check, A, NP, NP, MP, xx, x, xp, z, y, l, u, (T)alpha, (T)rho, part, part2, NP, scratch);
                }
                std::swap(x, xp);
                rhs_slabs = pass_slabs;
                if (check) {
                    ProfScope ps(prof, cat_chk, 2);
                    colsum<T>(st, part2, NP, pass_slabs, nullptr, T(0), nullptr, T(0), Aty, NP);
                    gemv_rows<T>(st, P, NP, x, Px, nullptr, T(1), T(0), 0, NP, 0, NP, 0);
                    CheckScalars cs{p.epsAbs, p.epsRel, epsAdmm, rho, rhorho, p.adptRho, convFlag};
                    check_convergence<T>(st, (int)n, (int)m, Ax, Px, Aty, q, x, xp, z, zp, scratch, res_dev, cs, 1);
                }
            }
            if (check) {
                HIPC(hipMemcpyAsync(res_host, res_dev, 15 * sizeof(double), hipMemcpyDeviceToHost, st));
                HIPC(hipStreamSynchronize(st));
                prof.harvest();
                if (sweep_gave_up(true)) return true;
                resP = res_host[0]; resD = res_host[1]; rhorho = res_host[4]; convFlag = (int)res_host[5];
                if (convFlag != QPS_CONV_NUM_ITR) break;
            }
        }
        HIPC(hipStreamSynchronize(st));
        prof.harvest();
        if (sweep_gave_up()) return true;
        const double t2 = now_s();
        PolishReport pr;
        if (p.polish) polish_dense<T>(st, n, m, NP, MP, P, A, q, l, u, y, x, part, p, &pr);
        download_vec(x, xh, n);
        if (info) {
            info->convFlag = convFlag; info->iterations = ii > p.numIterations ? p.numIterations : ii;
            info->numRefactor = nref; info->cgIterations = 0; info->rhoFinal = rho; info->rhoProposed = rhorho;
            info->resPrim = resP; info->resDual = resD; info->tSetup = t1 - t0; info->tLoop = t2 - t1; info->tRefactor = tref;
            info->polishFlag = pr.flag; info->polishIterations = pr.minresIterations; info->tPolish = pr.seconds;
            info->trsvBlock = nb; info->sweepVariant = sweep_variant();
        }
        return false;
    }
    void polish(double* xh, const double* yh, const qps_params& p, qps_polish_report* rep) override {
        HIPC(hipSetDevice(device));
        upload_vec(xh, x, n); upload_vec(yh, y, m);
        PolishReport pr;
        polish_dense<T>(st, n, m, NP, MP, P, A, q, l, u, y, x, part, p, &pr);
        download_vec(x, xh, n);
        if (rep) {
            rep->flag = pr.flag; rep->refinements = pr.refinements; rep->minresIterations = pr.minresIterations;
            rep->numActiveLower = pr.numLower; rep->numActiveUpper = pr.numUpper; rep->reserved0 = 0; rep->relres = pr.relres; rep->seconds = pr.seconds;
        }
    }
    void get_dual(double* zh, double* yh) override {
        HIPC(hipSetDevice(device));
        if (zh) download_vec(z, zh, m);
        if (yh) download_vec(y, yh, m);
    }
    void linsys_init(double rho, double sigma, int linsys, int nbreq) override {
        HIPC(hipSetDevice(device));
        if (linsys != QPS_LINSYS_AUTO && linsys != QPS_LINSYS_CHOLESKY) throw QpsError(QPS_ERR_UNSUPPORTED, "dense handles support QPS_LINSYS_CHOLESKY only");
        nb = pick_nb<T>(nbreq, NP);
        blocked_off = false;
        factorize(rho, sigma, true);
    }
    void linsys_solve(const double* xh, const double* zh, const double* yh, double rho, double sigma, int changed,
                      double* xxh, double* zzh) override {
        HIPC(hipSetDevice(device));
        if (!factor_valid && !changed) throw QpsError(QPS_ERR_BAD_ARGUMENT, "qps_linsys_solve called before qps_linsys_init");
        if (changed) factorize(rho, sigma, false);
        upload_vec(xh, x, n); upload_vec(zh, z, m); upload_vec(yh, y, m);
        linear_solve(rho, sigma);
        if (sweep_gave_up()) { factorize(rho, sigma, false); linear_solve(rho, sigma); }
        download_vec(xx, xxh, n); download_vec(zz, zzh, m);
    }
    void operator_apply(int op, const double* in, double* out, double rho, double sigma) override {
        HIPC(hipSetDevice(device));
        auto Pin = [&](T* dst) { gemv_rows<T>(st, P, NP, xx, dst, nullptr, T(1), T(0), 0, NP, 0, NP, 0); };
        auto Ain = [&](T* dst) { if (m > 0) gemv_rows<T>(st, A, NP, xx, dst, nullptr, T(1), T(0), 0, MP, 0, NP, 0); };
        auto Atv = [&](const T* v, T* dst) {
            if (m > 0) { gemv_cols_partial<T>(st, A, NP, v, nullptr, T(1), T(0), part, NP, MP, NP); colsum<T>(st, part, NP, part_tiles, nullptr, T(0), nullptr, T(0), dst, NP); }
            else HIPC(hipMemsetAsync(dst, 0, sizeof(T) * NP, st));
        };
        if (op == QPS_OP_AT) { upload_vec(in, zz, m); Atv(zz, Aty); download_vec(Aty, out, n); return; }
        upload_vec(in, xx, n);
        if (op == QPS_OP_P) { Pin(Px); download_vec(Px, out, n); }
        else if (op == QPS_OP_A) { Ain(Ax); download_vec(Ax, out, m); }
        else if (op == QPS_OP_PA) { Pin(Px); Ain(Ax); download_vec(Px, out, n); download_vec(Ax, out + n, m); }
        else if (op == QPS_OP_REDUCED) {
            Pin(Px); Ain(Ax); Atv(Ax, Aty);
            std::vector<double> a((size_t)n), b((size_t)n);
            download_vec(Px, a.data(), n); download_vec(Aty, b.data(), n);
            for (int64_t i = 0; i < n; ++i) out[i] = a[(size_t)i] + rho * b[(size_t)i] + sigma * in[i];
        } else throw QpsError(QPS_ERR_BAD_ARGUMENT, "unknown qps_operator_kind");
    }
};

struct BatchSolverBase {
    int device = 0; int64_t n = 0, m = 0; int count = 0; std::string err; Profiler prof;
    virtual ~BatchSolverBase() {}
    virtual void solve_batch(double* x, const qps_params& p, qps_info* infos) = 0;
    virtual void get_dual(double* z, double* y) = 0;
};

template <typename T> struct BatchedDenseSolver : BatchSolverBase {
    StreamLease lease; DeviceOwner mem; hipStream_t st = nullptr;
    int NP = 0, MP = 0, nb = 0, slabs = 0, rpw = 0, part_tiles = 0;
    T *A = nullptr, *P = nullptr, *q = nullptr, *l = nullptr, *u = nullptr, *PI = nullptr, *AA = nullptr, *M = nullptr, *S = nullptr,
      *tmp = nullptr, *dinv = nullptr;
    T *x = nullptr, *xp = nullptr, *xres = nullptr, *z = nullptr, *y = nullptr, *xx = nullptr, *tt = nullptr, *yv = nullptr, *part = nullptr,
      *part2 = nullptr, *part_tmp = nullptr, *sw_part = nullptr, *Px = nullptr, *Aty = nullptr;
    int* fail = nullptr; int* d_active = nullptr; double *d_rho = nullptr, *d_rhorho = nullptr;
    unsigned long long* scratch = nullptr; double* res_dev = nullptr; double* res_host = nullptr; double* stage = nullptr;
    int* h_int = nullptr; double* h_dbl = nullptr;
    bool have_AA = false; double fac_sigma = -1; int fac_nb = -1; std::vector<double> fac_rho;
    char* sb_args = nullptr; void* sb_host = nullptr;
    int cat_pass = 0, cat_sweep = 0;

    BatchedDenseSolver(int dev, int cnt, int64_t n_, int64_t m_) {
        device = dev; n = n_; m = m_; count = cnt;
        HIPC(hipSetDevice(device));
        st = prof.st = lease.acquire(device);
        NP = roundup(n, 64); MP = roundup(m, 64);
        slabs = apass_plan<T>(NP, MP, &rpw, count);
        {
            const double s = sizeof(T), c = cnt;
            cat_pass = prof.category("apass(fused A-pass, batched)", c * s * ((double)m * n + 3.0 * n + 6.0 * m));
            cat_sweep = prof.category("sweeps(fused fwd+bwd, batched, triangle read once)", c * s * ((double)n * (n + 1) / 2 + 2.0 * n));
        }
        part_tiles = gemv_cols_tiles(MP);
        const int64_t nn = (int64_t)NP * NP, c = count;
        A = mem.dalloc<T>(c * MP * NP, st); P = mem.dalloc<T>(c * nn, st); PI = mem.dalloc<T>(c * nn, st); AA = mem.dalloc<T>(c * nn, st); M = mem.dalloc<T>(c * nn, st);
        S = mem.dalloc<T>(c * nn, st); tmp = mem.dalloc<T>(c * nn, st); dinv = mem.dalloc<T>(c * (int64_t)(NP / 64) * 4096, st);
        q = mem.dalloc<T>(c * NP, st); l = mem.dalloc<T>(c * MP, st); u = mem.dalloc<T>(c * MP, st);
        x = mem.dalloc<T>(c * NP, st); xp = mem.dalloc<T>(c * NP, st); xres = mem.dalloc<T>(c * NP, st); xx = mem.dalloc<T>(c * NP, st); tt = mem.dalloc<T>(c * NP, st);
        yv = mem.dalloc<T>(c * NP, st); Px = mem.dalloc<T>(c * NP, st); Aty = mem.dalloc<T>(c * NP, st); z = mem.dalloc<T>(c * MP, st); y = mem.dalloc<T>(c * MP, st);
        int rpw1 = 0;
        const int64_t part_slabs = std::max<int64_t>(std::max<int64_t>(c * slabs, apass_plan<T>(NP, MP, &rpw1, 1)), std::max(part_tiles, 1));
        part = mem.dalloc<T>(part_slabs * NP, st); part2 = mem.dalloc<T>(c * slabs * NP, st); part_tmp = mem.dalloc<T>((int64_t)std::max(part_tiles, 1) * NP, st);
        const int sw_slabs = sweep_fused_slabs<T>(NP, count); sw_part = mem.dalloc<T>(c * std::max(sw_slabs, 1) * NP, st);
        fail = mem.dalloc<int>(count + 4, st); d_active = mem.dalloc<int>(count + 4, st); d_rho = mem.dalloc<double>(count + 4, st); d_rhorho = mem.dalloc<double>(count + 4, st);
        scratch = mem.dalloc<unsigned long long>(16 * c, st); res_dev = mem.dalloc<double>(8 * c, st);
        res_host = mem.pinned<double>(8 * c); h_int = mem.pinned<int>(count + 4); h_dbl = mem.pinned<double>(2 * (count + 4));
        stage = mem.dalloc<double>(std::max<int64_t>((int64_t)MP * NP, nn) + 64, st);
    }
    ~BatchedDenseSolver() override {
        (void)hipSetDevice(device);
        (void)hipStreamSynchronize(st);
        prof.release_events();
    }
    std::unique_ptr<FastUploader> loader;
    void put_vec(const double* h, T* d, int64_t cnt_) {
        if (cnt_ <= 0) return;
        if (!loader) loader.reset(new FastUploader(st, device));
        loader->copy(stage, h, sizeof(double) * (size_t)cnt_);
        convert_copy<T>(st, stage, d, cnt_);
    }
    void put_matrix(const double* h, int rows, int cols, T* d) {
        if (rows <= 0 || cols <= 0) return;
        if (!loader) loader.reset(new FastUploader(st, device));
        loader->copy(stage, h, sizeof(double) * (size_t)rows * cols);
        import_colmajor<T>(st, stage, rows, rows, cols, d, NP);
    }
    void finish_loading() { HIPC(hipStreamSynchronize(st)); loader.reset(); }
    void get_dual(double* zh, double* yh) override {
        HIPC(hipSetDevice(device));
        for (int b = 0; b < count && m > 0; ++b) {
            if (zh) HIPC(download_staged<T>(st, stage, z + (int64_t)b * MP, zh + (int64_t)b * m, m));
            if (yh) HIPC(download_staged<T>(st, stage, y + (int64_t)b * MP, yh + (int64_t)b * m, m));
        }
    }
    void load_problem(int b, const double* Ph, const double* Ah, const double* qh, const double* lh, const double* uh) {
        put_matrix(Ph, (int)n, (int)n, P + (int64_t)b * NP * NP);
        put_matrix(Ah, (int)m, (int)n, A + (int64_t)b * MP * NP);
        put_vec(qh, q + (int64_t)b * NP, n); put_vec(lh, l + (int64_t)b * MP, m); put_vec(uh, u + (int64_t)b * MP, m);
    }
    DenseChol<T> chol() const { return {st, (int)n, NP, MP, P, A, PI, AA, M, S, tmp, dinv, fail}; }
    void push_state(const std::vector<double>& rho, const std::vector<double>& rhorho, const std::vector<int>& active) {
        for (int b = 0; b < count; ++b) { h_dbl[b] = rho[b]; h_dbl[count + 4 + b] = rhorho[b]; h_int[b] = active[b]; }
        HIPC(hipMemcpyAsync(d_rho, h_dbl, sizeof(double) * count, hipMemcpyHostToDevice, st));
        HIPC(hipMemcpyAsync(d_rhorho, h_dbl + count + 4, sizeof(double) * count, hipMemcpyHostToDevice, st));
        HIPC(hipMemcpyAsync(d_active, h_int, sizeof(int) * count, hipMemcpyHostToDevice, st));
        HIPC(hipStreamSynchronize(st));
    }

    void solve_batch(double* xh, const qps_params& p, qps_info* infos) override {
        HIPC(hipSetDevice(device));
        const double t0 = now_s();
        if (slabs <= 0) throw QpsError(QPS_ERR_UNSUPPORTED, "batched path needs m >= 1 and n within the fused-pass limit");
        nb = pick_nb<T>(p.trsvBlock, NP);
        const DenseChol<T> ch = chol();
        const char* what = "P + sigma I + rho A'A";
        const double sigma = p.sigma, alpha = p.alpha;
        const double epsAdmm = std::fmin(p.epsAbs, p.epsRel) * 1e-2;
        std::vector<double> rho(count, p.rho), rhorho(count, p.rho), resP(count, NAN), resD(count, NAN), tref(count, 0.0);
        std::vector<int> active(count, 1), conv(count, QPS_CONV_NUM_ITR), iters(count, p.numIterations), nref(count, 0), all(count);
        for (int b = 0; b < count; ++b) all[b] = b;
        HIPC(hipMemsetAsync(fail, 0, sizeof(int) * count, st));
        const bool rebuild = !(p.reuseFactor && have_AA && fac_sigma == sigma);
        if ((int)fac_rho.size() != count) fac_rho.assign(count, -1.0);
        std::vector<int> todo;
        for (int b = 0; b < count; ++b)
            if (rebuild || fac_rho[b] != p.rho || fac_nb != nb) todo.push_back(b);
        if ((int)todo.size() == count) { ch.form(sigma, p.rho, rebuild, rebuild, count); ch.factor(nb, count); }
        else for (int b : todo) { ch.at(b).form(sigma, p.rho, rebuild, rebuild); ch.at(b).factor(nb); }
        ch.check(what, "", h_int, count, &todo);
        have_AA = true; fac_sigma = sigma; fac_nb = nb;
        for (int b : todo) fac_rho[b] = p.rho;
        for (int b = 0; b < count; ++b) put_vec(xh + (int64_t)b * n, x + (int64_t)b * NP, n);
        loader.reset();
        HIPC(hipMemsetAsync(z, 0, sizeof(T) * (size_t)count * MP, st));
        HIPC(hipMemsetAsync(y, 0, sizeof(T) * (size_t)count * MP, st));
        push_state(rho, rhorho, active);
        const double t1 = now_s();
        BatchStride bsS; bsS.count = count; bsS.mat = (int64_t)NP * NP; bsS.vin = NP; bsS.vout = NP; bsS.active = d_active;
        BatchStride bsC; bsC.count = count; bsC.mat = (int64_t)slabs * NP; bsC.vin = NP; bsC.vout = NP; bsC.active = d_active;
        BatchStride bsK; bsK.count = count; bsK.vin = NP; bsK.vout = MP; bsK.active = d_active;
        PassBatch pb; pb.count = count; pb.slabs = slabs; pb.rho_arr = d_rho; pb.active = d_active;
        int rhs_slabs = 0, nactive = count, ii = 0;
        const int nblk = (NP + nb - 1) / nb;
        if (p.loopVariant == 0 && nblk == 1 && admm_small_batch_supported<T>(NP, MP)) {
            const size_t ab = admm_small_args_bytes(), ob = admm_small_out_bytes();
            if (!sb_host) { sb_args = mem.dalloc<char>((int64_t)(ab + ob) * count + 64, st); sb_host = mem.pinned<char>((ab + ob) * (size_t)count + 64); }
            char* args_h = static_cast<char*>(sb_host); char* outs_h = args_h + ab * count;
            char* args_d = sb_args; char* outs_d = sb_args + ab * count;
            std::vector<int> it(count, 0);
            HIPC(hipMemsetAsync(xp, 0, sizeof(T) * (size_t)count * NP, st));
            while (nactive > 0) {
                for (int b = 0; b < count; ++b)
                    admm_small_args_set(args_h, b, (int)n, (int)m, NP, MP, it[b], active[b] ? p.numIterations : it[b], p.numItrConv, p.adptRho, rho[b], rhorho[b],
                                        sigma, alpha, p.epsAbs, p.epsRel, epsAdmm, p.fctrRho);
                HIPC(hipMemcpyAsync(args_d, args_h, ab * count, hipMemcpyHostToDevice, st));
                admm_small_batch<T>(st, count, NP, MP, args_d, A, P, S, q, l, u, x, xp, z, y, outs_d);
                HIPC(hipMemcpyAsync(outs_h, outs_d, ob * count, hipMemcpyDeviceToHost, st));
                HIPC(hipStreamSynchronize(st));
                std::vector<int> changed;
                for (int b = 0; b < count; ++b) {
                    if (!active[b]) continue;
                    int last = 0, flag = QPS_CONV_NUM_ITR, need = 0; double r8[8];
                    admm_small_read(outs_h + ob * b, &last, &flag, &need, r8);
                    it[b] = last; rhorho[b] = r8[4];
                    if (!std::isnan(r8[0]) || !std::isnan(r8[1])) { resP[b] = r8[0]; resD[b] = r8[1]; }
                    if (flag != QPS_CONV_NUM_ITR) { conv[b] = flag; iters[b] = last; active[b] = 0; --nactive; }
                    else if (need && last < p.numIterations) { rho[b] = rhorho[b]; ++nref[b]; changed.push_back(b); }
                    else { iters[b] = p.numIterations; active[b] = 0; --nactive; }
                }
                if (!changed.empty()) {
                    const double ta = now_s();
                    const bool together = (int)changed.size() * 2 >= count;
                    if (together) { push_state(rho, rhorho, active); ch.form(sigma, 0.0, false, false, count, d_rho); ch.factor(nb, count); for (int b = 0; b < count; ++b) fac_rho[b] = rho[b]; }
                    else for (int b : changed) { ch.at(b).form(sigma, rho[b], false, false); ch.at(b).factor(nb); fac_rho[b] = rho[b]; }
                    ch.check(what, "", h_int, count, together ? &all : &changed);
                    const double dt = (now_s() - ta) / changed.size();
                    for (int b : changed) tref[b] += dt;
                }
            }
            HIPC(hipMemcpyAsync(xres, x, sizeof(T) * (size_t)count * NP, hipMemcpyDeviceToDevice, st));
        }
        for (ii = 1; ii <= p.numIterations && nactive > 0; ++ii) {
            std::vector<int> changed;
            if (p.adptRho)
                for (int b = 0; b < count; ++b)
                    if (active[b] && ((rhorho[b] * p.fctrRho < rho[b]) || (rhorho[b] > p.fctrRho * rho[b]))) {
                        rho[b] = rhorho[b]; ++nref[b]; changed.push_back(b);
                    }
            if (!changed.empty()) {
                const double ta = now_s();
                const bool together = (int)changed.size() * 2 >= count;
                if (together) {
                    push_state(rho, rhorho, active);
                    ch.form(sigma, 0.0, false, false, count, d_rho);
                    ch.factor(nb, count);
                    for (int b = 0; b < count; ++b) fac_rho[b] = rho[b];
                }
                for (int b : changed) {
                    if (!together) { ch.at(b).form(sigma, rho[b], false, false); ch.at(b).factor(nb); fac_rho[b] = rho[b]; }
                    if (rhs_slabs > 0) {
                        T* pb_ = part + (int64_t)b * slabs * NP;
                        gemv_cols_partial<T>(st, A + (int64_t)b * MP * NP, NP, z + (int64_t)b * MP, y + (int64_t)b * MP, (T)rho[b], T(-1), part_tmp, NP, MP, NP);
                        colsum<T>(st, part_tmp, NP, part_tiles, nullptr, T(0), nullptr, T(0), pb_, NP);
                        if (slabs > 1) HIPC(hipMemsetAsync(pb_ + NP, 0, sizeof(T) * (size_t)(slabs - 1) * NP, st));
                    }
                }
                ch.check(what, "", h_int, count, together ? &all : &changed);
                push_state(rho, rhorho, active);
                const double dt = (now_s() - ta) / changed.size();
                for (int b : changed) tref[b] += dt;
            }
            const bool check = (ii % p.numItrConv == 0);
            colsum<T>(st, part, NP, rhs_slabs, x, (T)sigma, q, T(-1), tt, NP, bsC);
            ch.sweeps(nb, tt, yv, xx, sw_part, bsS, {&prof, cat_sweep, (prof.level == 1 && ii % 50 == 13) ? 1 : 2});
            if (check) HIPC(hipMemsetAsync(scratch, 0, 16 * sizeof(unsigned long long) * count, st));
            {
                ProfLaunchScope ps(prof, cat_pass, (prof.level == 1 && !check && ii % 50 == 38) ? 1 : (check ? 3 : 2));
                apass<T>(st, check, A, NP, NP, MP, xx, x, xp, z, y, l, u, (T)alpha, T(1), part, part2, NP, scratch, pb);
            }
            std::swap(x, xp);
            rhs_slabs = slabs;
            if (check) {
                colsum<T>(st, part2, NP, slabs, nullptr, T(0), nullptr, T(0), Aty, NP, bsC);
                BatchStride bsP = bsS; bsP.mat = (int64_t)NP * NP;
                gemv_rows<T>(st, P, NP, x, Px, nullptr, T(1), T(0), 0, NP, 0, NP, 0, bsP);
                CheckScalars cs{p.epsAbs, p.epsRel, epsAdmm, 0.0, 0.0, p.adptRho, QPS_CONV_NUM_ITR};
                check_convergence<T>(st, (int)n, (int)m, (const T*)nullptr, Px, Aty, q, x, xp, z, z, scratch, res_dev, cs, 1, bsK, d_rho, d_rhorho);
                HIPC(hipMemcpyAsync(res_host, res_dev, 8 * sizeof(double) * count, hipMemcpyDeviceToHost, st));
                HIPC(hipStreamSynchronize(st));
                prof.harvest();
                bool any_done = false;
                for (int b = 0; b < count; ++b) {
                    if (!active[b]) continue;
                    const double* r = res_host + 8 * b;
                    resP[b] = r[0]; resD[b] = r[1]; rhorho[b] = r[4]; conv[b] = (int)r[5];
                    if (conv[b] != QPS_CONV_NUM_ITR) {
                        active[b] = 0; iters[b] = ii; --nactive; any_done = true;
                        HIPC(hipMemcpyAsync(xres + (int64_t)b * NP, x + (int64_t)b * NP, sizeof(T) * NP, hipMemcpyDeviceToDevice, st));
                    }
                }
                push_state(rho, rhorho, active);
                (void)any_done;
            }
        }
        for (int b = 0; b < count; ++b)
            if (active[b]) HIPC(hipMemcpyAsync(xres + (int64_t)b * NP, x + (int64_t)b * NP, sizeof(T) * NP, hipMemcpyDeviceToDevice, st));
        HIPC(hipStreamSynchronize(st));
        prof.harvest();
        const double t2 = now_s();
        std::vector<PolishReport> pol(count);
        if (p.polish)
            for (int b = 0; b < count; ++b)
                polish_dense<T>(st, n, m, NP, MP, P + (int64_t)b * NP * NP, A + (int64_t)b * MP * NP, q + (int64_t)b * NP, l + (int64_t)b * MP,
                                u + (int64_t)b * MP, y + (int64_t)b * MP, xres + (int64_t)b * NP, part, p, &pol[b]);
        for (int b = 0; b < count; ++b) {
            HIPC(download_staged<T>(st, stage, xres + (int64_t)b * NP, xh + (int64_t)b * n, n));
            if (infos) {
                qps_info& in = infos[b];
                in.convFlag = conv[b]; in.iterations = iters[b]; in.numRefactor = nref[b]; in.cgIterations = 0;
                in.rhoFinal = rho[b]; in.rhoProposed = rhorho[b]; in.resPrim = resP[b]; in.resDual = resD[b];
                in.tSetup = t1 - t0; in.tLoop = t2 - t1; in.tRefactor = tref[b];
                in.polishFlag = pol[b].flag; in.polishIterations = pol[b].minresIterations; in.tPolish = pol[b].seconds;
                in.trsvBlock = nb; in.sweepVariant = chol_sweep_variant<T>(NP, nb);
                in.sweepGaveUp = 0; in.cgExplicit = 0;
            }
        }
    }
};

struct Handle { SolverBase* impl = nullptr; std::vector<SolverBase*> batch; BatchSolverBase* fused_batch = nullptr; ProxQpBase* proxqp = nullptr; int64_t n = 0, m = 0; std::string err; };

int fail_with(Handle* h, int code, const std::string& msg) {
    g_last_error = msg;
    if (h) h->err = msg;
    return code;
}
bool all_finite(const double* p, int64_t count, bool allow_inf) {
    std::atomic<int> bad{0};
    host_parallel(count, (int64_t)1 << 20, [&](int, int64_t b, int64_t e) {
        for (int64_t i0 = b; i0 < e && !bad.load(std::memory_order_relaxed); i0 += 4096) {
            const int64_t i1 = std::min(e, i0 + 4096);
            int flag = 0;
            if (allow_inf) { for (int64_t i = i0; i < i1; ++i) flag |= (p[i] != p[i]); }
            else { for (int64_t i = i0; i < i1; ++i) flag |= !(std::fabs(p[i]) <= 1.7976931348623157e308); }
            if (flag) bad.store(1, std::memory_order_relaxed);
        }
    });
    return bad.load() == 0;
}
bool all_finite_matrix(const double* p, int64_t rows, int64_t cols, int64_t ld) {
    if (ld == rows) return all_finite(p, rows * cols, false);
    std::atomic<int> bad{0};
    host_parallel(cols, std::max<int64_t>(1, ((int64_t)1 << 20) / std::max<int64_t>(rows, 1)), [&](int, int64_t b, int64_t e) {
        for (int64_t j = b; j < e && !bad.load(std::memory_order_relaxed); ++j) {
            int flag = 0;
            for (int64_t i = 0; i < rows; ++i) flag |= !(std::fabs(p[i + j * ld]) <= 1.7976931348623157e308);
            if (flag) bad.store(1, std::memory_order_relaxed);
        }
    });
    return bad.load() == 0;
}
int64_t dense_asymmetry(const double* P, int64_t n, int64_t ldp) {
    const int64_t nb = (n + 63) / 64;
    std::atomic<int64_t> first{INT64_MAX};
    const int nt = (int)std::min<int64_t>(host_threads(), std::max<int64_t>(1, n * n / ((int64_t)1 << 20)));
    auto work = [&](int t) {
        for (int64_t b = t; b < nb; b += nt) {
            const int64_t j0 = b * 64;
            if (j0 >= first.load(std::memory_order_relaxed)) break;
            for (int64_t i0 = j0; i0 < n; i0 += 64) {
                const int64_t j1 = std::min(n, j0 + 64), i1 = std::min(n, i0 + 64);
                for (int64_t j = j0; j < j1; ++j)
                    for (int64_t i = std::max(i0, j + 1); i < i1; ++i)
                        if (P[i + j * ldp] != P[j + i * ldp]) { int64_t cur = first.load(); while (j < cur && !first.compare_exchange_weak(cur, j)) {} }
            }
        }
    };
    std::vector<std::thread> th;
    int started = 1;
    try { for (int t = 1; t < nt; ++t) { th.emplace_back(work, t); started = t + 1; } } catch (const std::system_error&) {}
    work(0);
    for (int t = started; t < nt; ++t) work(t);
    for (auto& x : th) x.join();
    const int64_t f = first.load();
    return f == INT64_MAX ? -1 : f;
}
int require_device(int device, const char* out_of_range = "device index out of range") {
    int cnt = 0;
    if (hipGetDeviceCount(&cnt) != hipSuccess || cnt <= 0) return fail_with(nullptr, QPS_ERR_NO_DEVICE, "no HIP device visible: libqps_hip has no CPU fallback");
    if (device < 0 || device >= cnt) return fail_with(nullptr, QPS_ERR_BAD_ARGUMENT, out_of_range);
    return QPS_OK;
}

template <typename F> int guarded(Handle* h, F&& f) {
    try { f(); return QPS_OK; }
    catch (const QpsError& e) { return fail_with(h, e.code, e.msg); }
    catch (const std::bad_alloc&) { return fail_with(h, QPS_ERR_OUT_OF_MEMORY, "host allocation failed"); }
    catch (const std::exception& e) { return fail_with(h, QPS_ERR_HIP, e.what()); }
}

int validate_params(Handle* h, const qps_params* p) {
    if (!p) return fail_with(h, QPS_ERR_BAD_ARGUMENT, "params is NULL");
    if (p->numIterations < 0) return fail_with(h, QPS_ERR_BAD_ARGUMENT, "numIterations must be >= 0");
    if (p->numItrConv <= 0) return fail_with(h, QPS_ERR_BAD_ARGUMENT, "numItrConv must be positive");
    if (!(p->rho > 0) || !std::isfinite(p->rho)) return fail_with(h, QPS_ERR_BAD_ARGUMENT, "rho must be positive and finite");
    if (!(p->sigma >= 0) || !std::isfinite(p->sigma)) return fail_with(h, QPS_ERR_BAD_ARGUMENT, "sigma must be non-negative and finite");
    if (!std::isfinite(p->alpha)) return fail_with(h, QPS_ERR_BAD_ARGUMENT, "alpha must be finite");
    if (std::isnan(p->epsAbs) || std::isnan(p->epsRel)) return fail_with(h, QPS_ERR_BAD_ARGUMENT, "epsAbs/epsRel must not be NaN");
    if (p->adptRho && !(p->fctrRho > 0)) return fail_with(h, QPS_ERR_BAD_ARGUMENT, "fctrRho must be positive");
    return QPS_OK;
}

SolverBase* make_dense(int device, int64_t n, int64_t m, int dtype, const double* P, int64_t ldp, const double* A, int64_t lda,
                       const double* q, const double* l, const double* u) {
    auto load = [&](auto s) -> SolverBase* {
        s->upload_matrix(P, ldp, (int)n, (int)n, s->P, s->NP);
        s->upload_matrix(A, lda, (int)m, (int)n, s->A, s->NP);
        s->upload_vec(q, s->q, n); s->upload_vec(l, s->l, m); s->upload_vec(u, s->u, m);
        return s.release();
    };
    if (dtype == QPS_F64) return load(std::make_unique<DenseSolver<double>>(device, n, m, dtype));
    return load(std::make_unique<DenseSolver<float>>(device, n, m, dtype));
}

}

extern "C" {

#define QPS_API __attribute__((visibility("default")))

QPS_API int32_t qps_default_params(qps_params* p) {
    if (!p) return QPS_ERR_BAD_ARGUMENT;
    memset(p, 0, sizeof(*p));
    p->numIterations = 5000; p->epsAbs = 1e-6; p->epsRel = 1e-6;
    p->rho = 1.0; p->sigma = 1e-6; p->alpha = 1.6; p->delta = 1e-6; p->adptRho = 0;
    p->fctrRho = 5.0; p->numItrConv = 25; p->numItrPolish = 10; p->epsMinres = 1e-6; p->numItrMinres = 500;
    p->linsys = QPS_LINSYS_AUTO; p->trsvBlock = 0; p->reuseFactor = 0; p->loopVariant = 0;
    p->epsPcg = 1e-6; p->numItrPcg = 1000;
    return QPS_OK;
}

// ... 420 lines not shown
```

### quadraticprogramsolver_amd/csrc/qps_internal.h

```cpp
#pragma once
#include <hip/hip_runtime.h>

#include <algorithm>
#include <chrono>
#include <cmath>
#include <cstdio>
#include <cstring>
#include <mutex>
#include <string>
#include <system_error>
#include <thread>
#include <vector>

#include "../../include/qps.h"

namespace qps {

struct QpsError { int code; std::string msg; QpsError(int c, std::string m) : code(c), msg(std::move(m)) {} };

inline double now_s() { return std::chrono::duration<double>(std::chrono::steady_clock::now().time_since_epoch()).count(); }
inline int roundup(int64_t v, int q) { return (int)(((v + q - 1) / q) * q); }

struct KernelStat { double seconds = 0; int64_t launches = 0; double algo_bytes = 0; };

struct Profiler {
    int level = 0;
    hipStream_t st = nullptr;
    struct Pending { int cat; hipEvent_t a, b; };
    std::vector<Pending> pending;
    std::vector<hipEvent_t> pool;
    std::vector<std::string> names;
    std::vector<KernelStat> stats;
    int category(const char* name, double bytes) {
        for (size_t i = 0; i < names.size(); ++i) if (names[i] == name) return (int)i;
        names.push_back(name); KernelStat s; s.algo_bytes = bytes; stats.push_back(s); return (int)names.size() - 1;
    }
    hipEvent_t get() { if (!pool.empty()) { hipEvent_t e = pool.back(); pool.pop_back(); return e; } hipEvent_t e; (void)hipEventCreate(&e); return e; }
    bool on(int cat_level) const { return level >= cat_level; }
    void begin(int cat, hipEvent_t& a) { a = get(); (void)hipEventRecord(a, st); (void)cat; }
    void end(int cat, hipEvent_t a) { hipEvent_t b = get(); (void)hipEventRecord(b, st); pending.push_back({cat, a, b}); }
    void harvest() {
        for (auto& p : pending) {
            float ms = 0; (void)hipEventElapsedTime(&ms, p.a, p.b);
            stats[p.cat].seconds += ms * 1e-3; stats[p.cat].launches += 1;
            pool.push_back(p.a); pool.push_back(p.b);
        }
        pending.clear();
    }
    void reset() { for (auto& s : stats) { s.seconds = 0; s.launches = 0; } }
    void release_events() {
        for (auto e : pool) (void)hipEventDestroy(e);
        for (auto& p : pending) { (void)hipEventDestroy(p.a); (void)hipEventDestroy(p.b); }
        pool.clear(); pending.clear();
    }
    ~Profiler() { for (auto e : pool) (void)hipEventDestroy(e); for (auto& p : pending) { (void)hipEventDestroy(p.a); (void)hipEventDestroy(p.b); } }
};
struct ProfLaunchScope {
    Profiler& p; int cat; hipEvent_t a, b; bool active;
    ProfLaunchScope(Profiler& pr, int c, int lvl);
    ~ProfLaunchScope();
};
struct ProfScope {
    Profiler& p; int cat; hipEvent_t a; bool active;
    ProfScope(Profiler& pr, int c, int lvl) : p(pr), cat(c), a(nullptr), active(pr.on(lvl)) { if (active) p.begin(cat, a); }
    ~ProfScope() { if (active) p.end(cat, a); }
};

#define HIPC(expr)                                                                                            \
    do {                                                                                                      \
        hipError_t e_ = (expr);                                                                               \
        if (e_ != hipSuccess) {                                                                               \
            char b_[512]; snprintf(b_, sizeof b_, "%s failed: %s (%s:%d)", #expr, hipGetErrorString(e_), __FILE__, __LINE__); \
            throw QpsError(e_ == hipErrorOutOfMemory ? QPS_ERR_OUT_OF_MEMORY : QPS_ERR_HIP, b_);               \
        }                                                                                                     \
    } while (0)

struct DeviceOwner {
    std::vector<void*> dev, host;
    DeviceOwner() = default;
    DeviceOwner(const DeviceOwner&) = delete;
    DeviceOwner& operator=(const DeviceOwner&) = delete;
    ~DeviceOwner() { for (void* p : dev) (void)hipFree(p); for (void* p : host) (void)hipHostFree(p); }
    template <typename T> T* alloc(int64_t count) {
        dev.push_back(nullptr);
        HIPC(hipMalloc(&dev.back(), sizeof(T) * (size_t)count));
        return static_cast<T*>(dev.back());
    }
    template <typename T> T* dalloc(int64_t count, hipStream_t st) {
        if (count < 64) count = 64;
        T* p = alloc<T>(count);
        HIPC(hipMemsetAsync(p, 0, sizeof(T) * (size_t)count, st));
        return p;
    }
    template <typename T> T* pinned(size_t count) {
        host.push_back(nullptr);
        HIPC(hipHostMalloc(&host.back(), sizeof(T) * count));
        return static_cast<T*>(host.back());
    }
    void release(void* p) {
        if (!p) return;
        auto it = std::find(dev.begin(), dev.end(), p);
        if (it != dev.end()) { (void)hipFree(p); dev.erase(it); return; }
        it = std::find(host.begin(), host.end(), p);
        if (it != host.end()) { (void)hipHostFree(p); host.erase(it); }
    }
};

struct StagedUploader {
    hipStream_t st; char* pin[2] = {nullptr, nullptr}; hipEvent_t ev[2] = {nullptr, nullptr}; bool busy[2] = {false, false};
    size_t cap; int cur = 0;
    explicit StagedUploader(hipStream_t s, size_t cap_ = (size_t)8 << 20) : st(s), cap(cap_) {}
    StagedUploader(const StagedUploader&) = delete;
    ~StagedUploader() {
        for (int k = 0; k < 2; ++k) {
            if (busy[k]) (void)hipEventSynchronize(ev[k]);
            if (ev[k]) (void)hipEventDestroy(ev[k]);
            if (pin[k]) (void)hipHostFree(pin[k]);
        }
    }
    void copy(void* dst, const void* src, size_t bytes) {
        const char* s_ = static_cast<const char*>(src); char* d_ = static_cast<char*>(dst);
        while (bytes > 0) {
            const int k = cur; cur ^= 1;
            if (!pin[k]) { HIPC(hipHostMalloc((void**)&pin[k], cap)); HIPC(hipEventCreateWithFlags(&ev[k], hipEventDisableTiming)); }
            if (busy[k]) { HIPC(hipEventSynchronize(ev[k])); busy[k] = false; }
            const size_t nb = bytes < cap ? bytes : cap;
            memcpy(pin[k], s_, nb);
            HIPC(hipMemcpyAsync(d_, pin[k], nb, hipMemcpyHostToDevice, st));
            HIPC(hipEventRecord(ev[k], st)); busy[k] = true;
            s_ += nb; d_ += nb; bytes -= nb;
        }
    }
};

int host_threads();
template <typename F> inline void host_parallel(int64_t count, int64_t min_per_thread, F&& f) {
    int nt = (int)std::min<int64_t>(host_threads(), std::max<int64_t>(1, count / std::max<int64_t>(1, min_per_thread)));
    if (nt <= 1) { f(0, (int64_t)0, count); return; }
    std::vector<std::thread> th;
    const int64_t per = (count + nt - 1) / nt;
    int started = 1;
    try { for (int t = 1; t < nt; ++t) { th.emplace_back([&, t] { f(t, std::min(count, t * per), std::min(count, (t + 1) * per)); }); started = t + 1; } }
    catch (const std::system_error&) {}
    f(0, (int64_t)0, std::min(count, per));
    for (int t = started; t < nt; ++t) f(t, std::min(count, t * per), std::min(count, (t + 1) * per));
    for (auto& x : th) x.join();
}
struct PinnedRing { char* base = nullptr; size_t half = 0; };
PinnedRing acquire_ring(int device);
void recycle_ring(int device, PinnedRing r);
struct FastUploader {
    hipStream_t st; int device; PinnedRing ring; hipEvent_t ev[2] = {nullptr, nullptr}; bool busy[2] = {false, false}; int cur = 0;
    FastUploader(hipStream_t s, int dev) : st(s), device(dev) { ring = acquire_ring(dev); }
    FastUploader(const FastUploader&) = delete;
    ~FastUploader() {
        for (int k = 0; k < 2; ++k) { if (busy[k]) (void)hipEventSynchronize(ev[k]); if (ev[k]) (void)hipEventDestroy(ev[k]); }
        recycle_ring(device, ring);
    }
    void copy(void* dst, const void* src, size_t bytes) {
        const char* s_ = static_cast<const char*>(src); char* d_ = static_cast<char*>(dst);
        while (bytes > 0) {
            const int k = cur; cur ^= 1;
            if (!ev[k]) HIPC(hipEventCreateWithFlags(&ev[k], hipEventDisableTiming));
            if (busy[k]) { HIPC(hipEventSynchronize(ev[k])); busy[k] = false; }
            const size_t nb = std::min(bytes, ring.half);
            char* pin = ring.base + (size_t)k * ring.half;
            host_parallel((int64_t)nb, (int64_t)2 << 20, [&](int, int64_t b, int64_t e) { if (e > b) memcpy(pin + b, s_ + b, (size_t)(e - b)); });
            HIPC(hipMemcpyAsync(d_, pin, nb, hipMemcpyHostToDevice, st));
            HIPC(hipEventRecord(ev[k], st)); busy[k] = true;
            s_ += nb; d_ += nb; bytes -= nb;
        }
    }
};

struct Arena {
    char* base = nullptr; size_t off = 0; bool planning = true;
    template <typename T> T* take(int64_t count) {
        if (count < 64) count = 64;
        off = (off + 255) & ~(size_t)255;
        T* p = planning ? nullptr : reinterpret_cast<T*>(base + off);
        off += sizeof(T) * (size_t)count;
        return p;
    }
    size_t bytes = 0;
    size_t planned() const { return ((off + 255) & ~(size_t)255) + 256; }
    void commit(hipStream_t st, char* recycled = nullptr, size_t recycled_bytes = 0) {
        const size_t need = planned();
        if (recycled) { base = recycled; bytes = recycled_bytes; }
        else { HIPC(hipMalloc((void**)&base, need)); bytes = need; }
        HIPC(hipMemsetAsync(base, 0, need, st));
        off = 0; planning = false;
    }
    Arena() = default;
    Arena(const Arena&) = delete;
    ~Arena() { if (base) (void)hipFree(base); }
};

struct HandleResources { hipStream_t st = nullptr; void* pinned = nullptr; char* block = nullptr; size_t block_bytes = 0; };
HandleResources acquire_resources(int device, size_t block_need);
void recycle_resources(int device, HandleResources r);
// ... 32 lines not shown
```

### quadraticprogramsolver_amd/csrc/qps_kernels.h

```cpp
#pragma once
#ifndef QPS_NT_SLABS
#define QPS_NT_SLABS 1
#endif
#include <hip/hip_runtime.h>
#include <stdint.h>

#include <atomic>
#include <thread>

namespace qps {

constexpr int kMaxDevices = 64;
int current_device();
int device_cu_count(int device);
struct PerDeviceOnce {
    std::atomic<unsigned char> state[kMaxDevices] = {};
    template <typename F> void once(int dev, F&& f) {
        if (dev < 0 || dev >= kMaxDevices) { f(); return; }
        if (state[dev].load(std::memory_order_acquire) == 2) return;
        unsigned char expect = 0;
        if (state[dev].compare_exchange_strong(expect, 1, std::memory_order_acq_rel)) { f(); state[dev].store(2, std::memory_order_release); return; }
        while (state[dev].load(std::memory_order_acquire) != 2) std::this_thread::yield();
    }
};

struct LaunchTiming { hipEvent_t start = nullptr, stop = nullptr; };
extern thread_local LaunchTiming g_launch_timing;


struct BatchStride { int count = 1; int64_t mat = 0, vin = 0, vout = 0; const int* active = nullptr; };

template <typename T> struct VecOf;
template <> struct VecOf<double> { using type = double2; static constexpr int N = 2; };
template <> struct VecOf<float>  { using type = float4;  static constexpr int N = 4; };

template <typename T>
void gemv_rows(hipStream_t st, const T* S, int64_t ld, const T* v, T* out, const T* out0, T alpha, T beta,
               int r0, int r1, int c0, int c1, int tri, BatchStride bs = BatchStride());

template <typename T>
int gemv_cols_partial(hipStream_t st, const T* S, int64_t ld, const T* va, const T* vb, T ca, T cb,
                      T* part, int64_t part_ld, int nrows, int ncols);
int gemv_cols_tiles(int nrows);

template <typename T>
void colsum(hipStream_t st, const T* part, int64_t part_ld, int ntiles, const T* a0, T s0, const T* a1, T s1,
            T* out, int ncols, BatchStride bs = BatchStride());

template <typename T>
void admm_update(hipStream_t st, int NP, int MP, const T* xx, const T* zz, T* x, T* xp, T* z, T* zp, T* y,
                 const T* l, const T* u, T alpha, T rho);

struct CheckScalars { double epsAbs, epsRel, epsAdmm, rho, rhorho; int adptRho; int convFlag; };
template <typename T>
void check_convergence(hipStream_t st, int n, int m, const T* Ax, const T* Px, const T* Aty, const T* q, const T* x,
                       const T* xp, const T* z, const T* zp, unsigned long long* scratch , double* res_dev,
                       CheckScalars cs, int dual_only = 0, BatchStride bs = BatchStride(), const double* rho_arr = nullptr,
                       const double* rhorho_arr = nullptr);

template <typename T> int apass_plan(int NP, int MP, int* rows_per_wg, int count = 1);
template <typename T> int apass_max_np();
struct PassBatch { int count = 1; int slabs = 0; const double* rho_arr = nullptr; const int* active = nullptr; int pq_me = 0; };
template <typename T>
void apass(hipStream_t st, bool check, const T* A, int64_t ld, int NP, int MP, const T* xx, const T* x_old, T* x_new, T* z,
           T* y, const T* l, const T* u, T alpha, T rho, T* part, T* part2, int64_t part_ld, unsigned long long* slots,
           PassBatch pb = PassBatch());
template <typename T> int apass_proxqp_slabs(int NP, int MP);
template <typename T>
int apass_kkt(hipStream_t st, const T* A, int64_t ld, int NP, int MP, const T* vx, const T* vlam, const T* mask, T delta, T* out_lam,
              T* part, int64_t part_ld);
template <typename T>
int apass_proxqp(hipStream_t st, const T* G, int64_t ld, int NP, int MP, int me, const T* x, T* x_scratch, T* slack, T* dual,
                 const T* g, T rho, T* part, int64_t part_ld);

template <typename T> bool sweep_fused_supported(int NP);
template <typename T> int sweep_fused_slabs(int NP, int count = 1);
template <typename T>
int sweep_fused(hipStream_t st, const T* S, int64_t ld, int NP, const T* v, T* part, int64_t part_ld, BatchStride bs = BatchStride());

template <typename T> bool admm_small_supported(int n, int m, int NP, int MP);
template <typename T> void transpose_small(hipStream_t st, const T* A, int NP, int MP, T* At);
template <typename T> bool admm_small_batch_supported(int NP, int MP);
size_t admm_small_args_bytes();
void admm_small_args_set(void* host_array, int idx, int n, int m, int NP, int MP, int it_begin, int it_end, int numItrConv, int adptRho, double rho,
                         double rhorho, double sigma, double alpha, double epsAbs, double epsRel, double epsAdmm, double fctrRho);
template <typename T>
void admm_small_batch(hipStream_t st, int count, int NP, int MP, const void* args_dev, const T* A, const T* P, const T* S, const T* q, const T* l,
                      const T* u, T* x, T* xp, T* z, T* y, void* outs_dev);
template <typename T>
void admm_small(hipStream_t st, int n, int m, int NP, int MP, int it_begin, int it_end, int numItrConv, int adptRho, double rho,
                double rhorho, double sigma, double alpha, double epsAbs, double epsRel, double epsAdmm, double fctrRho, const T* A,
                const T* At, const T* P, const T* S, const T* q, const T* l, const T* u, T* x, T* xp, T* z, T* y, void* out_dev);
size_t admm_small_out_bytes();
void admm_small_read(const void* host_copy, int* last_it, int* convFlag, int* need_rho, double* res8);

template <typename T> void fill(hipStream_t st, T* p, int64_t n, T v);
template <typename T> void convert_copy(hipStream_t st, const double* src, T* dst, int64_t n);
template <typename T> void convert_back(hipStream_t st, const T* src, double* dst, int64_t n);
template <typename T> inline hipError_t upload_staged(hipStream_t st, double* stage, const double* h, T* d, int64_t n) {
    if (n <= 0) return hipSuccess;
    const hipError_t e = hipMemcpyAsync(stage, h, sizeof(double) * (size_t)n, hipMemcpyHostToDevice, st);
    if (e != hipSuccess) return e;
    convert_copy<T>(st, stage, d, n);
    return hipStreamSynchronize(st);
}
template <typename T> inline hipError_t download_staged(hipStream_t st, double* stage, const T* d, double* h, int64_t n) {
    if (n <= 0) return hipSuccess;
    convert_back<T>(st, d, stage, n);
    const hipError_t e = hipMemcpyAsync(h, stage, sizeof(double) * (size_t)n, hipMemcpyDeviceToHost, st);
    return e != hipSuccess ? e : hipStreamSynchronize(st);
}

template <typename T>
void import_colmajor(hipStream_t st, const double* src, int64_t lds, int rows, int cols, T* dst, int64_t ldd);

template <typename T>
void gemm(hipStream_t st, int M, int N, int K, T alpha, const T* A, int64_t lda, bool a_kcontig, const T* B, int64_t ldb,
          bool b_kcontig, T beta, T* C, int64_t ldc, bool lower_only, int batch = 1, int64_t sA = 0, int64_t sB = 0,
          int64_t sC = 0, int ktri = 0);

template <typename T> void assemble_M(hipStream_t st, int NP, const T* PI, const T* AA, T rho, T* M, int batch = 1,
                                      const double* rho_arr = nullptr);
template <typename T> void make_PI(hipStream_t st, int n, int NP, const T* P, T sigma, T* PI, int batch = 1);

inline int64_t chol_scratch_elems(int NP) { return (int64_t)((NP / 64 + 1) / 2) * 3 * 4096 + 64; }
inline bool chol_scratch_fits(int NP) { return chol_scratch_elems(NP) <= (int64_t)NP * NP; }
template <typename T> void cholesky(hipStream_t st, int NP, T* M, T* dinv, int* fail_dev, int batch = 1, T* scratch = nullptr);

template <typename T> void build_sweep_matrix(hipStream_t st, int NP, int nb, const T* L, const T* dinv, T* S, T* tmp, int batch = 1, bool premul = false);

template <typename T> bool trsv_blocked_supported(int NP, int nb);
template <typename T> int64_t trsv_blocked_pub_words(int NP);
struct TrsvBlockedPair { int dev; hipStream_t stream; TrsvBlockedPair(int device, hipStream_t st); ~TrsvBlockedPair(); TrsvBlockedPair(const TrsvBlockedPair&) = delete; };
void trsv_blocked_forget_stream(int device, hipStream_t st);
template <typename T>
void trsv_blocked(hipStream_t st, bool bwd, const T* S, int64_t ld, int NP, int nb, const T* v, T* out, unsigned long long* pub,
                  unsigned epoch, unsigned* abort_word, int mode = 0);

}
```

Baseline: 14560.

## Fuse convergence check into one kernel and speculate iterations past checks with device stop flag

```diff
diff --git a/quadraticprogramsolver_amd/csrc/k_loop.hip b/quadraticprogramsolver_amd/csrc/k_loop.hip
--- a/quadraticprogramsolver_amd/csrc/k_loop.hip
+++ b/quadraticprogramsolver_amd/csrc/k_loop.hip
@@ -1,4 +1,6 @@
 #include <cstdlib>
+#include <initializer_list>
+#include <utility>
 
 #include "qps_kernels.h"
 #include "wave_reduce.h"
@@ -105,12 +107,13 @@
     *reinterpret_cast<V*>(part + (int64_t)rt * part_ld + c) = o;
 }
 
-template <typename T>
-__global__ __launch_bounds__(256) void k_colsum(const T* __restrict__ part, int64_t part_ld, int ntiles,
+template <typename T, bool GUARD>
+__device__ __forceinline__ void colsum_body(const T* __restrict__ part, int64_t part_ld, int ntiles,
                                                 const T* __restrict__ a0, T s0, const T* __restrict__ a1, T s1,
                                                 T* __restrict__ out, int ncols, BatchStride bs) {
     using V = typename VecOf<T>::type;
     constexpr int VN = VecOf<T>::N;
+    if (GUARD) { if (*bs.stop) return; }
     if (bs.active && !bs.active[blockIdx.y]) return;
     part += (int64_t)blockIdx.y * bs.mat; out += (int64_t)blockIdx.y * bs.vout;
     if (a0) a0 += (int64_t)blockIdx.y * bs.vin;
@@ -164,6 +167,19 @@
 }
 
 template <typename T>
+__global__ __launch_bounds__(256) void k_colsum(const T* __restrict__ part, int64_t part_ld, int ntiles,
+                                                const T* __restrict__ a0, T s0, const T* __restrict__ a1, T s1,
+                                                T* __restrict__ out, int ncols, BatchStride bs) {
+    colsum_body<T, false>(part, part_ld, ntiles, a0, s0, a1, s1, out, ncols, bs);
+}
+template <typename T>
+__global__ __launch_bounds__(256) void k_colsum_guarded(const T* __restrict__ part, int64_t part_ld, int ntiles,
+                                                const T* __restrict__ a0, T s0, const T* __restrict__ a1, T s1,
+                                                T* __restrict__ out, int ncols, BatchStride bs) {
+    colsum_body<T, true>(part, part_ld, ntiles, a0, s0, a1, s1, out, ncols, bs);
+}
+
+template <typename T>
 __global__ __launch_bounds__(256) void k_admm_update(int NP, int MP, const T* __restrict__ xx, const T* __restrict__ zz,
                                                      T* __restrict__ x, T* __restrict__ xp, T* __restrict__ z,
                                                      T* __restrict__ zp, T* __restrict__ y, const T* __restrict__ l,
@@ -186,21 +202,30 @@
     }
 }
 
-template <typename T>
-__global__ __launch_bounds__(256) void k_check_norms(int n, int m, const T* __restrict__ Ax, const T* __restrict__ Px,
-                                                     const T* __restrict__ Aty, const T* __restrict__ q,
-                                                     const T* __restrict__ x, const T* __restrict__ xp,
-                                                     const T* __restrict__ z, const T* __restrict__ zp,
-                                                     unsigned long long* __restrict__ slots, int dual_only, BatchStride bs) {
-    if (bs.active && !bs.active[blockIdx.y]) return;
+__device__ __forceinline__ double jmax(double a, double b) { return (isnan(a) || isnan(b)) ? (double)NAN : (a > b ? a : b); }
+
+constexpr int CHECK_TICKET = 15;
+
+template <typename T>
+__global__ __launch_bounds__(256) void k_check(int n, int m, const T* __restrict__ Ax, const T* __restrict__ Px,
+                                               const T* __restrict__ Aty, const T* __restrict__ q,
+                                               const T* __restrict__ x, const T* __restrict__ xp,
+                                               const T* __restrict__ z, const T* __restrict__ zp,
+                                               unsigned long long* __restrict__ slots, double* __restrict__ res, int res_stride,
+                                               CheckScalars cs, const double* __restrict__ rho_arr,
+                                               const double* __restrict__ rhorho_arr, int* __restrict__ stop,
+                                               const unsigned* __restrict__ abort_word, int dual_only, BatchStride bs) {
+    const int b = blockIdx.y;
+    if (bs.active && !bs.active[b]) return;
     {
-        const int64_t on = (int64_t)blockIdx.y * bs.vin, om = (int64_t)blockIdx.y * bs.vout;
-        Ax += om; z += om; zp += om; Px += on; Aty += on; q += on; x += on; xp += on; slots += (int64_t)blockIdx.y * 16;
+        const int64_t on = (int64_t)b * bs.vin, om = (int64_t)b * bs.vout;
+        Ax += om; z += om; zp += om; Px += on; Aty += on; q += on; x += on; xp += on; slots += (int64_t)b * 16;
     }
     unsigned long long v[9];
 #pragma unroll
     for (int k = 0; k < 9; ++k) v[k] = 0ull;
-    for (int i = blockIdx.x * 256 + threadIdx.x; i < max(n, m); i += gridDim.x * 256) {
+    const int N = dual_only ? n : max(n, m);
+    for (int i = blockIdx.x * 256 + threadIdx.x; i < N; i += gridDim.x * 256) {
         if (i < m && !dual_only) {
             const double ax = (double)Ax[i], zi = (double)z[i];
             v[0] = max(v[0], absbits((double)(Ax[i] - z[i])));
@@ -221,20 +246,19 @@
         v[k] = wave_max_u64(v[k]);
         if ((threadIdx.x & 63) == 0 && v[k] != 0ull) atomicMax(&slots[k], v[k]);
     }
-}
-
-__device__ __forceinline__ double jmax(double a, double b) { return (isnan(a) || isnan(b)) ? (double)NAN : (a > b ? a : b); }
-
-__global__ void k_check_decide(const unsigned long long* __restrict__ slots, double* __restrict__ res, CheckScalars cs,
-                               const double* __restrict__ rho_arr, const double* __restrict__ rhorho_arr,
-                               const int* __restrict__ active) {
-    if (threadIdx.x != 0) return;
-    const int b = blockIdx.x;
-    if (active && !active[b]) return;
-    slots += (int64_t)b * 16; res += (int64_t)b * 8;
+    __threadfence();
+    __shared__ int last;
+    __syncthreads();
+    if (threadIdx.x == 0) last = (atomicAdd(&slots[CHECK_TICKET], 1ull) == (unsigned long long)(gridDim.x - 1));
+    __syncthreads();
+    if (!last || threadIdx.x != 0) return;
+    __threadfence();
+
+    res += (int64_t)b * res_stride;
     if (rho_arr) { cs.rho = rho_arr[b]; cs.rhorho = rhorho_arr[b]; cs.convFlag = 1; }
     double nv[9];
-    for (int k = 0; k < 9; ++k) nv[k] = __longlong_as_double((long long)slots[k]);
+    for (int k = 0; k < 9; ++k) nv[k] = __longlong_as_double((long long)atomicExch(&slots[k], 0ull));
+    atomicExch(&slots[CHECK_TICKET], 0ull);
     const double MIN_VAL_RHO = 1e-3, MAX_VAL_RHO = 1e6;
     const double normResPrim = nv[0], normResDual = nv[1];
     const double maxNormPrim = jmax(nv[2], nv[3]);
@@ -253,6 +277,18 @@
     if ((nv[7] <= cs.epsAdmm) && (nv[8] <= cs.epsAdmm)) flag = 2;
     res[0] = normResPrim; res[1] = normResDual; res[2] = maxNormPrim; res[3] = maxNormDual;
     res[4] = rhorho; res[5] = (double)flag; res[6] = nv[7]; res[7] = nv[8];
+    if (stop) {
+        const int s = (flag != 1) || (cs.adptRho && ((rhorho * cs.fctrRho < cs.rho) || (rhorho > cs.fctrRho * cs.rho)));
+        __hip_atomic_store(stop, s, __ATOMIC_RELAXED, __HIP_MEMORY_SCOPE_AGENT);
+        res[8] = (double)s;
+    }
+    if (abort_word) *reinterpret_cast<unsigned*>(res + 14) = *abort_word;
+}
+
+struct ZeroList { void* p[8]; unsigned n16[8]; };
+__global__ __launch_bounds__(256) void k_zero_list(ZeroList zl) {
+    const unsigned i = blockIdx.x * 256 + threadIdx.x;
+    if (i < zl.n16[blockIdx.y]) static_cast<uint4*>(zl.p[blockIdx.y])[i] = make_uint4(0u, 0u, 0u, 0u);
 }
 
 template <typename T> __global__ void k_fill(T* p, int64_t n, T v) {
@@ -319,6 +355,7 @@
         hipExtLaunchKernelGGL((k_colsum<T>), dim3((ncols + cols_wg - 1) / cols_wg, bs.count), dim3(256), 0, st, lt.start, lt.stop, 0, part, part_ld, ntiles, a0, s0, a1, s1, out, ncols, bs);
         return;
     }
+    if (bs.stop) { hipLaunchKernelGGL((k_colsum_guarded<T>), dim3((ncols + cols_wg - 1) / cols_wg, bs.count), dim3(256), 0, st, part, part_ld, ntiles, a0, s0, a1, s1, out, ncols, bs); return; }
     hipLaunchKernelGGL((k_colsum<T>), dim3((ncols + cols_wg - 1) / cols_wg, bs.count), dim3(256), 0, st, part, part_ld, ntiles, a0, s0, a1, s1, out, ncols, bs);
 }
 
@@ -331,15 +368,27 @@
 
 template <typename T>
 void check_convergence(hipStream_t st, int n, int m, const T* Ax, const T* Px, const T* Aty, const T* q, const T* x,
-                       const T* xp, const T* z, const T* zp, unsigned long long* scratch, double* res_dev, CheckScalars cs,
-                       int dual_only, BatchStride bs, const double* rho_arr, const double* rhorho_arr) {
-    if (!dual_only) (void)hipMemsetAsync(scratch, 0, 16 * sizeof(unsigned long long) * bs.count, st);
-    const int N = n > m ? n : m;
+                       const T* xp, const T* z, const T* zp, unsigned long long* scratch, double* res_out, CheckScalars cs,
+                       int dual_only, BatchStride bs, const double* rho_arr, const double* rhorho_arr, int* stop,
+                       const unsigned* abort_word) {
+    const int N = dual_only ? n : (n > m ? n : m);
     int blocks = (N + 255) / 256;
     if (blocks > 1024) blocks = 1024;
     if (blocks < 1) blocks = 1;
-    hipLaunchKernelGGL((k_check_norms<T>), dim3(blocks, bs.count), dim3(256), 0, st, n, m, Ax, Px, Aty, q, x, xp, z, zp, scratch, dual_only, bs);
-    hipLaunchKernelGGL(k_check_decide, dim3(bs.count), dim3(64), 0, st, scratch, res_dev, cs, rho_arr, rhorho_arr, bs.active);
+    hipLaunchKernelGGL((k_check<T>), dim3(blocks, bs.count), dim3(256), 0, st, n, m, Ax, Px, Aty, q, x, xp, z, zp, scratch, res_out,
+                       bs.count > 1 ? 8 : 0, cs, rho_arr, rhorho_arr, stop, abort_word, dual_only, bs);
+}
+
+void zero_buffers(hipStream_t st, std::initializer_list<std::pair<void*, size_t>> bufs) {
+    ZeroList zl = {};
+    unsigned most = 0; int k = 0;
+    for (const auto& b : bufs) {
+        if (!b.first || b.second == 0 || k >= 8) continue;
+        zl.p[k] = b.first; zl.n16[k] = (unsigned)((b.second + 15) / 16);
+        most = zl.n16[k] > most ? zl.n16[k] : most; ++k;
+    }
+    if (k == 0) return;
+    hipLaunchKernelGGL(k_zero_list, dim3((most + 255) / 256, k), dim3(256), 0, st, zl);
 }
 
 template <typename T> void fill(hipStream_t st, T* p, int64_t n, T v) {
@@ -362,7 +411,7 @@
     template void admm_update<T>(hipStream_t, int, int, const T*, const T*, T*, T*, T*, T*, T*, const T*, const T*, T, T);   \
     template void check_convergence<T>(hipStream_t, int, int, const T*, const T*, const T*, const T*, const T*, const T*,    \
                                        const T*, const T*, unsigned long long*, double*, CheckScalars, int, BatchStride,     \
-                                       const double*, const double*);                                                        \
+                                       const double*, const double*, int*, const unsigned*);                                                     \
     template void fill<T>(hipStream_t, T*, int64_t, T);                                                                      \
     template void convert_copy<T>(hipStream_t, const double*, T*, int64_t);                                                  \
     template void convert_back<T>(hipStream_t, const T*, double*, int64_t);
diff --git a/quadraticprogramsolver_amd/csrc/k_pass_kernel.h b/quadraticprogramsolver_amd/csrc/k_pass_kernel.h
--- a/quadraticprogramsolver_amd/csrc/k_pass_kernel.h
+++ b/quadraticprogramsolver_amd/csrc/k_pass_kernel.h
@@ -41,14 +41,15 @@
     }
 };
 
-template <typename T, int THREADS, int KC, int R, bool CHECK, int MODE>
-__global__ __launch_bounds__(THREADS) void k_apass(const T* __restrict__ A, int64_t ld, int NP, int MP, int rows_per_wg,
+template <typename T, int THREADS, int KC, int R, bool CHECK, int MODE, bool GUARD>
+__device__ __forceinline__ void apass_body(const T* __restrict__ A, int64_t ld, int NP, int MP, int rows_per_wg,
                                                    const T* __restrict__ xx, const T* __restrict__ x_old, T* __restrict__ x_new,
                                                    T* __restrict__ z, T* __restrict__ y, const T* __restrict__ l,
                                                    const T* __restrict__ u, T alpha, T rho, T* __restrict__ part,
                                                    T* __restrict__ part2, int64_t part_ld, unsigned long long* __restrict__ slots,
                                                    PassBatch pb) {
     using PS = Pass<T, THREADS, KC, R, CHECK>;
+    if (GUARD) { if (*pb.stop) return; }
     if (pb.count > 1 || pb.active) {
         const int b = blockIdx.y;
         if (pb.active && !pb.active[b]) return;
@@ -253,6 +254,25 @@
     }
 }
 
+template <typename T, int THREADS, int KC, int R, bool CHECK, int MODE>
+__global__ __launch_bounds__(THREADS) void k_apass(const T* __restrict__ A, int64_t ld, int NP, int MP, int rows_per_wg,
+                                                   const T* __restrict__ xx, const T* __restrict__ x_old, T* __restrict__ x_new,
+                                                   T* __restrict__ z, T* __restrict__ y, const T* __restrict__ l,
+                                                   const T* __restrict__ u, T alpha, T rho, T* __restrict__ part,
+                                                   T* __restrict__ part2, int64_t part_ld, unsigned long long* __restrict__ slots,
+                                                   PassBatch pb) {
+    apass_body<T, THREADS, KC, R, CHECK, MODE, false>(A, ld, NP, MP, rows_per_wg, xx, x_old, x_new, z, y, l, u, alpha, rho, part, part2, part_ld, slots, pb);
+}
+template <typename T, int THREADS, int KC, int R>
+__global__ __launch_bounds__(THREADS) void k_apass_guarded(const T* __restrict__ A, int64_t ld, int NP, int MP, int rows_per_wg,
+                                                   const T* __restrict__ xx, const T* __restrict__ x_old, T* __restrict__ x_new,
+                                                   T* __restrict__ z, T* __restrict__ y, const T* __restrict__ l,
+                                                   const T* __restrict__ u, T alpha, T rho, T* __restrict__ part,
+                                                   T* __restrict__ part2, int64_t part_ld, unsigned long long* __restrict__ slots,
+                                                   PassBatch pb) {
+    apass_body<T, THREADS, KC, R, false, 0, true>(A, ld, NP, MP, rows_per_wg, xx, x_old, x_new, z, y, l, u, alpha, rho, part, part2, part_ld, slots, pb);
+}
+
 template <typename T, int THREADS, int KC, int R, int RC, int MODE>
 void launch_pass(hipStream_t st, bool check, int G, const T* A, int64_t ld, int NP, int MP, int rows_per_wg, const T* xx,
                  const T* x_old, T* x_new, T* z, T* y, const T* l, const T* u, T alpha, T rho, T* part, T* part2,
@@ -269,6 +289,12 @@
             return;
         }
     }
+    if constexpr (MODE == 0) {
+        if (pb.stop) {
+            hipLaunchKernelGGL((k_apass_guarded<T, THREADS, KC, R>), dim3(G, pb.count), dim3(THREADS), 0, st, A, ld, NP, MP, rows_per_wg, xx, x_old, x_new, z, y, l, u, alpha, rho, part, part2, part_ld, slots, pb);
+            return;
+        }
+    }
     if (g_launch_timing.start) {
         const LaunchTiming lt = g_launch_timing;
         g_launch_timing = LaunchTiming();
diff --git a/quadraticprogramsolver_amd/csrc/k_sparse.hip b/quadraticprogramsolver_amd/csrc/k_sparse.hip
--- a/quadraticprogramsolver_amd/csrc/k_sparse.hip
+++ b/quadraticprogramsolver_amd/csrc/k_sparse.hip
@@ -663,7 +663,7 @@
     T *xx = nullptr, *zz = nullptr, *w = nullptr, *tt = nullptr, *cu = nullptr, *cu2 = nullptr, *cr = nullptr, *cc = nullptr, *tm = nullptr;
     T *Ax = nullptr, *Px = nullptr, *Aty = nullptr;
     double *part_uc = nullptr, *part_rr = nullptr; int part_uc_cap = 0; CgState* state = nullptr; CgState* state_host = nullptr;
-    unsigned long long* scratch = nullptr; double* res_dev = nullptr; double* res_host = nullptr; double* stage = nullptr;
+    unsigned long long* scratch = nullptr; double* res_pin = nullptr; double* res_host = nullptr; double* stage = nullptr;
     int nb_n = 0, nb_op = 0; int64_t cg_total = 0; int last_cg = 4;
     double eps_pcg = 1e-6; int itr_pcg = 1000;
     int cat_spmv, cat_op, cat_vec, cat_chk, cat_ldl, cat_pa = 0, cat_at = 0; int prof_calls = 0;
@@ -859,8 +859,9 @@
         part_uc = mem.dalloc<double>(part_uc_cap, st); part_rr = mem.dalloc<double>(nb_n + 64, st);
         state = reinterpret_cast<CgState*>(mem.dalloc<double>(16, st));
         state_host = reinterpret_cast<CgState*>(pinned);
-        scratch = mem.dalloc<unsigned long long>(16, st); res_dev = mem.dalloc<double>(16, st);
+        scratch = mem.dalloc<unsigned long long>(16, st);
         res_host = reinterpret_cast<double*>(static_cast<char*>(pinned) + 128);
+        HIPC(hipHostGetDevicePointer(reinterpret_cast<void**>(&res_pin), res_host, 0));
         stage = mem.dalloc<double>(std::max(nn, mm) + 64, st);
         upload_vec(qh, q, n); upload_vec(lh, l, m); upload_vec(uh, u, m);
         const double s = sizeof(T);
@@ -1028,6 +1029,7 @@
         const size_t nb_ = sizeof(T) * (size_t)(n + 64), mb_ = sizeof(T) * (size_t)(m + 64);
         HIPC(hipMemsetAsync(xp, 0, nb_, st)); HIPC(hipMemsetAsync(xx, 0, nb_, st));
         HIPC(hipMemsetAsync(z, 0, mb_, st)); HIPC(hipMemsetAsync(y, 0, mb_, st)); HIPC(hipMemsetAsync(zp, 0, mb_, st));
+        HIPC(hipMemsetAsync(scratch, 0, 16 * sizeof(unsigned long long), st));
         HIPC(hipStreamSynchronize(st));
         const double t1 = now_s();
         double rhorho = rho; int ii = 0, nref = 0; double resP = NAN, resD = NAN, tref = 0;
@@ -1064,9 +1066,8 @@
                     if (m > 0) spmv(At, y, Aty, T(1), nullptr, T(0), nullptr, T(0), nullptr);
                     else HIPC(hipMemsetAsync(Aty, 0, nb_, st));
                     CheckScalars cs{p.epsAbs, p.epsRel, epsAdmm, rho, rhorho, p.adptRho, convFlag};
-                    check_convergence<T>(st, (int)n, (int)m, Ax, Px, Aty, q, x, xp, z, zp, scratch, res_dev, cs);
+                    check_convergence<T>(st, (int)n, (int)m, Ax, Px, Aty, q, x, xp, z, zp, scratch, res_pin, cs);
                 }
-                HIPC(hipMemcpyAsync(res_host, res_dev, 8 * sizeof(double), hipMemcpyDeviceToHost, st));
                 HIPC(hipStreamSynchronize(st));
                 prof.harvest();
                 resP = res_host[0]; resD = res_host[1]; rhorho = res_host[4]; convFlag = (int)res_host[5];
diff --git a/quadraticprogramsolver_amd/csrc/k_trsv.hip b/quadraticprogramsolver_amd/csrc/k_trsv.hip
--- a/quadraticprogramsolver_amd/csrc/k_trsv.hip
+++ b/quadraticprogramsolver_amd/csrc/k_trsv.hip
@@ -9,11 +9,12 @@
 
 namespace {
 
-template <typename T, int THREADS, int KC, int RB, bool DB = true>
-__global__ __launch_bounds__(THREADS) void k_sweep_fused(const T* __restrict__ S, int64_t ld, int NP, const T* __restrict__ v,
+template <typename T, int THREADS, int KC, int RB, bool DB, bool GUARD>
+__device__ __forceinline__ void sweep_fused_body(const T* __restrict__ S, int64_t ld, int NP, const T* __restrict__ v,
                                                          T* __restrict__ part, int64_t part_ld, BatchStride bs) {
     using V = typename VecOf<T>::type;
     constexpr int VN = VecOf<T>::N, CHUNK = THREADS * VN, WAVES = THREADS / 64;
+    if (GUARD) { if (*bs.stop) return; }
     if (bs.active && !bs.active[blockIdx.y]) return;
     S += (int64_t)blockIdx.y * bs.mat; v += (int64_t)blockIdx.y * bs.vin; part += (int64_t)blockIdx.y * bs.vout;
     const int tid = threadIdx.x, G = gridDim.x, g = blockIdx.x;
@@ -114,11 +115,23 @@
     }
 }
 
-template <typename T, int KCW, bool DB = true>
-__global__ __launch_bounds__(512) void k_sweep_fused_wave(const T* __restrict__ S, int64_t ld, int NP, const T* __restrict__ v,
+template <typename T, int THREADS, int KC, int RB, bool DB = true>
+__global__ __launch_bounds__(THREADS) void k_sweep_fused(const T* __restrict__ S, int64_t ld, int NP, const T* __restrict__ v,
+                                                         T* __restrict__ part, int64_t part_ld, BatchStride bs) {
+    sweep_fused_body<T, THREADS, KC, RB, DB, false>(S, ld, NP, v, part, part_ld, bs);
+}
+template <typename T, int THREADS, int KC, int RB, bool DB = true>
+__global__ __launch_bounds__(THREADS) void k_sweep_fused_guarded(const T* __restrict__ S, int64_t ld, int NP, const T* __restrict__ v,
+                                                         T* __restrict__ part, int64_t part_ld, BatchStride bs) {
+    sweep_fused_body<T, THREADS, KC, RB, DB, true>(S, ld, NP, v, part, part_ld, bs);
+}
+
+template <typename T, int KCW, bool DB, bool GUARD>
+__device__ __forceinline__ void sweep_fused_wave_body(const T* __restrict__ S, int64_t ld, int NP, const T* __restrict__ v,
                                                           T* __restrict__ part, int64_t part_ld, BatchStride bs) {
     using V = typename VecOf<T>::type;
     constexpr int VN = VecOf<T>::N, CH = 64 * VN, WAVES = 8, COLS = KCW * CH;
+    if (GUARD) { if (*bs.stop) return; }
     if (bs.active && !bs.active[blockIdx.y]) return;
     S += (int64_t)blockIdx.y * bs.mat; v += (int64_t)blockIdx.y * bs.vin; part += (int64_t)blockIdx.y * bs.vout;
     const int tid = threadIdx.x, lane = tid & 63, wave = tid >> 6, g = blockIdx.x;
@@ -195,6 +208,17 @@
     }
 }
 
+template <typename T, int KCW, bool DB = true>
+__global__ __launch_bounds__(512) void k_sweep_fused_wave(const T* __restrict__ S, int64_t ld, int NP, const T* __restrict__ v,
+                                                         T* __restrict__ part, int64_t part_ld, BatchStride bs) {
+    sweep_fused_wave_body<T, KCW, DB, false>(S, ld, NP, v, part, part_ld, bs);
+}
+template <typename T, int KCW, bool DB = true>
+__global__ __launch_bounds__(512) void k_sweep_fused_wave_guarded(const T* __restrict__ S, int64_t ld, int NP, const T* __restrict__ v,
+                                                         T* __restrict__ part, int64_t part_ld, BatchStride bs) {
+    sweep_fused_wave_body<T, KCW, DB, true>(S, ld, NP, v, part, part_ld, bs);
+}
+
 static bool sweep_wave() { static const bool on = [] { const char* e = getenv("QPS_SWEEP_WAVE"); return !(e && atoi(e) == 0); }(); return on; }
 template <typename T> static bool sweep_wave_covers(int NP) { return sweep_wave() && NP <= 64 * VecOf<T>::N * 8; }
 
@@ -239,24 +263,27 @@
     if (sweep_wave_covers<T>(NP)) {
 #define QPS_WV(KCW)                                                                                                                \
     do {                                                                                                                           \
-        if (lt.start) hipExtLaunchKernelGGL((k_sweep_fused_wave<T, KCW>), grid, dim3(TH), 0, st, lt.start, lt.stop, 0, S, ld, NP, v, part, part_ld, bs); \
+        if (bs.stop) hipLaunchKernelGGL((k_sweep_fused_wave_guarded<T, KCW>), grid, dim3(TH), 0, st, S, ld, NP, v, part, part_ld, bs); \
+        else if (lt.start) hipExtLaunchKernelGGL((k_sweep_fused_wave<T, KCW>), grid, dim3(TH), 0, st, lt.start, lt.stop, 0, S, ld, NP, v, part, part_ld, bs); \
         else hipLaunchKernelGGL((k_sweep_fused_wave<T, KCW>), grid, dim3(TH), 0, st, S, ld, NP, v, part, part_ld, bs);              \
     } while (0)
         static const int wave_db = [] { const char* e = getenv("QPS_SWEEP_WAVE_DB"); return e ? atoi(e) : 0; }();
         if (NP <= 64 * VecOf<T>::N * 4) QPS_WV(4);
-        else if (wave_db == 0) { if (lt.start) hipExtLaunchKernelGGL((k_sweep_fused_wave<T, 8, false>), grid, dim3(TH), 0, st, lt.start, lt.stop, 0, S, ld, NP, v, part, part_ld, bs); else hipLaunchKernelGGL((k_sweep_fused_wave<T, 8, false>), grid, dim3(TH), 0, st, S, ld, NP, v, part, part_ld, bs); }
+        else if (wave_db == 0) { if (bs.stop) hipLaunchKernelGGL((k_sweep_fused_wave_guarded<T, 8, false>), grid, dim3(TH), 0, st, S, ld, NP, v, part, part_ld, bs); else if (lt.start) hipExtLaunchKernelGGL((k_sweep_fused_wave<T, 8, false>), grid, dim3(TH), 0, st, lt.start, lt.stop, 0, S, ld, NP, v, part, part_ld, bs); else hipLaunchKernelGGL((k_sweep_fused_wave<T, 8, false>), grid, dim3(TH), 0, st, S, ld, NP, v, part, part_ld, bs); }
         else QPS_WV(8);
 #undef QPS_WV
         return G;
     }
 #define QPS_S(KC, RB)                                                                                                              \
     do {                                                                                                                           \
-        if (lt.start) hipExtLaunchKernelGGL((k_sweep_fused<T, TH, KC, RB>), grid, dim3(TH), 0, st, lt.start, lt.stop, 0, S, ld, NP, v, part, part_ld, bs); \
+        if (bs.stop) hipLaunchKernelGGL((k_sweep_fused_guarded<T, TH, KC, RB>), grid, dim3(TH), 0, st, S, ld, NP, v, part, part_ld, bs); \
+        else if (lt.start) hipExtLaunchKernelGGL((k_sweep_fused<T, TH, KC, RB>), grid, dim3(TH), 0, st, lt.start, lt.stop, 0, S, ld, NP, v, part, part_ld, bs); \
         else hipLaunchKernelGGL((k_sweep_fused<T, TH, KC, RB>), grid, dim3(TH), 0, st, S, ld, NP, v, part, part_ld, bs);            \
     } while (0)
 #define QPS_SW(KC)                                                                                                                 \
     do {                                                                                                                           \
-        if (lt.start) hipExtLaunchKernelGGL((k_sweep_fused<T, TH, KC, 1, false>), grid, dim3(TH), 0, st, lt.start, lt.stop, 0, S, ld, NP, v, part, part_ld, bs); \
+        if (bs.stop) hipLaunchKernelGGL((k_sweep_fused_guarded<T, TH, KC, 1, false>), grid, dim3(TH), 0, st, S, ld, NP, v, part, part_ld, bs); \
+        else if (lt.start) hipExtLaunchKernelGGL((k_sweep_fused<T, TH, KC, 1, false>), grid, dim3(TH), 0, st, lt.start, lt.stop, 0, S, ld, NP, v, part, part_ld, bs); \
         else hipLaunchKernelGGL((k_sweep_fused<T, TH, KC, 1, false>), grid, dim3(TH), 0, st, S, ld, NP, v, part, part_ld, bs);      \
     } while (0)
 #define QPS_SR(KC) do { if (rb == 1) QPS_S(KC, 1); else if (rb == 2) QPS_S(KC, 2); else QPS_S(KC, 4); } while (0)
diff --git a/quadraticprogramsolver_amd/csrc/qps_capi.hip b/quadraticprogramsolver_amd/csrc/qps_capi.hip
--- a/quadraticprogramsolver_amd/csrc/qps_capi.hip
+++ b/quadraticprogramsolver_amd/csrc/qps_capi.hip
@@ -15,7 +15,7 @@
 
 namespace qps {
 namespace {
-constexpr size_t kPinnedBytes = 512, kRecycleBlockMax = (size_t)512 << 20;
+constexpr size_t kPinnedBytes = 1024, kRecycleBlockMax = (size_t)512 << 20;
 constexpr int kRecyclePerDevice = 4;
 std::mutex g_res_mu;
 std::vector<HandleResources> g_res[kMaxDevices];
@@ -109,7 +109,9 @@
     StreamLease lease; Arena arena;
     double* stage_mat = nullptr; int64_t stage_mat_count = 0;
     int pass_slabs = 0, pass_rpw = 0;
-    unsigned long long* scratch = nullptr; double* res_dev = nullptr; double* res_host = nullptr; double* stage = nullptr;
+    static constexpr int kResSlot = 64;
+    unsigned long long* scratch = nullptr; double* res_pin = nullptr; double* res_host = nullptr; double* stage = nullptr;
+    int* stop_dev = nullptr; hipEvent_t check_ev = nullptr;
     bool have_AA = false, factor_valid = false; double fac_rho = 0, fac_sigma = 0; int fac_nb = 0;
     int nb = 2048; int part_tiles = 0; int num_factorizations = 0;
     unsigned long long* pub = nullptr; unsigned* abort_dev = nullptr; unsigned sweep_epoch = 0; bool blocked_off = false, fac_premul = false;
@@ -162,9 +164,9 @@
             part2 = ar.take<T>((int64_t)slabs * NP);
             sw_part = ar.take<T>((int64_t)std::max(sweep_fused_slabs<T>(NP), 1) * NP);
             Ax = ar.take<T>(MP); Px = ar.take<T>(NP); Aty = ar.take<T>(NP);
-            scratch = ar.take<unsigned long long>(16); res_dev = ar.take<double>(16);
+            scratch = ar.take<unsigned long long>(16); stop_dev = ar.take<int>(64);
             pub = ar.take<unsigned long long>(trsv_blocked_pub_words<T>(NP));
-            abort_dev = reinterpret_cast<unsigned*>(res_dev + 14);
+            abort_dev = ar.take<unsigned>(64);
             stage = ar.take<double>((int64_t)NP + 2 * (int64_t)MP + 64);
             if (small_ok) { At = ar.take<T>((int64_t)NP * MP); small_out = ar.take<double>(32); }
             if (stage_mat_count > 0) stage_mat = ar.take<double>(stage_mat_count);
@@ -176,6 +178,8 @@
         arena.commit(st, recycled, res.block_bytes);
         layout(arena);
         res_host = reinterpret_cast<double*>(res.pinned);
+        HIPC(hipHostGetDevicePointer(reinterpret_cast<void**>(&res_pin), res_host, 0));
+        HIPC(hipEventCreateWithFlags(&check_ev, hipEventDisableTiming));
         small_out_host = small_ok ? reinterpret_cast<char*>(res.pinned) + 16 * sizeof(double) : nullptr;
         const double s = sizeof(T);
         cat_atw = prof.category("gemv_cols(A'w)", s * ((double)m * n + m + n));
@@ -197,6 +201,7 @@
         trsv_blocked_forget_stream(device, st);
         drop_graphs();
         prof.release_events();
+        if (check_ev) (void)hipEventDestroy(check_ev);
         lease.res.block = arena.base; lease.res.block_bytes = arena.bytes; arena.base = nullptr;
     }
 
@@ -237,9 +242,9 @@
         c.check("P + sigma I + rho A'A", ctx, &f);
         factor_valid = true; fac_rho = rho; fac_sigma = sigma; fac_nb = nb; fac_premul = use_blocked();
     }
-    bool sweep_gave_up(bool fetched = false) {
+    bool sweep_gave_up(bool fetched = false, const double* res = nullptr) {
         if (!fac_premul) return false;
-        unsigned* h = reinterpret_cast<unsigned*>(res_host + 14);
+        unsigned* h = reinterpret_cast<unsigned*>(const_cast<double*>(res ? res : res_host) + 14);
         if (!fetched) {
             HIPC(hipMemcpyAsync(h, abort_dev, sizeof(unsigned), hipMemcpyDeviceToHost, st));
             HIPC(hipStreamSynchronize(st));
@@ -251,9 +256,10 @@
     }
 
     int sweep_variant() const { const int v = chol_sweep_variant<T>(NP, nb); return (fac_premul && v != 2) ? 5 : v; }
-    void sweeps() {
+    void sweeps(const int* stop = nullptr) {
         if (sweep_variant() != 5) {
-            chol().sweeps(nb, tt, yv, xx, sw_part, BatchStride(), {&prof, cat_sweep, sample_lvl(13), cat_xsum, sample_lvl(21), cat_fwd, cat_bwd, 2});
+            BatchStride bs; bs.stop = stop;
+            chol().sweeps(nb, tt, yv, xx, sw_part, bs, {&prof, cat_sweep, sample_lvl(13), cat_xsum, sample_lvl(21), cat_fwd, cat_bwd, 2});
             return;
         }
         if (sweep_epoch >= 0xfffffff0u) {
@@ -302,10 +308,8 @@
         const bool reuse = p.reuseFactor && factor_valid && fac_rho == rho && fac_sigma == sigma && fac_nb == nb && fac_premul == use_blocked();
         if (!reuse) factorize(rho, sigma, !p.reuseFactor || !have_AA || fac_sigma != sigma);
         upload_vec(xh, x, n);
-        HIPC(hipMemsetAsync(xp, 0, sizeof(T) * NP, st));
-        HIPC(hipMemsetAsync(z, 0, sizeof(T) * std::max(MP, 64), st));
-        HIPC(hipMemsetAsync(y, 0, sizeof(T) * std::max(MP, 64), st));
-        HIPC(hipMemsetAsync(zp, 0, sizeof(T) * std::max(MP, 64), st));
+        zero_buffers(st, {{xp, sizeof(T) * NP}, {z, sizeof(T) * std::max(MP, 64)}, {y, sizeof(T) * std::max(MP, 64)}, {zp, sizeof(T) * std::max(MP, 64)},
+                          {scratch, 16 * sizeof(unsigned long long)}, {stop_dev, sizeof(int)}});
         HIPC(hipStreamSynchronize(st));
         const double t1 = now_s();
         double rhorho = rho;
@@ -352,6 +356,26 @@
         int rhs_slabs = 0;
         static const int graph_env = [] { const char* e = getenv("QPS_GRAPH"); return e ? atoi(e) : -1; }();
         const bool use_graph = fused && prof.level == 0 && p.numItrConv >= 3 && !fac_premul && (graph_env >= 0 ? graph_env != 0 : NP <= 2048);
+        static const int lookahead_env = [] { const char* e = getenv("QPS_CHECK_LOOKAHEAD"); return e ? atoi(e) : 1; }();
+        const int look_want = (fused && lookahead_env != 0 && !use_graph && prof.level != 2) ? (NP >= 4096 ? 2 : (NP >= 2048 ? 4 : 8)) : 0;
+        bool prev_stopped = false; int nchk = 0;
+        auto plain_iteration = [&](int it, const int* guard) {
+            prof_iter = guard ? -1 : it;
+            {
+                ProfLaunchScope ps(prof, cat_colsum, sample_lvl(29));
+                BatchStride bs; bs.stop = guard;
+                colsum<T>(st, part, NP, rhs_slabs, x, (T)sigma, q, T(-1), tt, NP, bs);
+            }
+            sweeps(guard);
+            {
+                const int lvl = (prof.level == 1 && (guard || it % 50 != 38)) ? 3 : 1;
+                ProfLaunchScope ps(prof, cat_pass, lvl);
+                PassBatch pb; pb.stop = guard;
+                apass<T>(st, false, A, NP, NP, MP, xx, x, xp, z, y, l, u, (T)alpha, (T)rho, part, part2, NP, scratch, pb);
+            }
+            std::swap(x, xp);
+            rhs_slabs = pass_slabs;
+        };
         for (ii = 1; ii <= p.numIterations; ++ii) {
             bool changed = false;
             if (p.adptRho && ((rhorho * p.fctrRho < rho) || (rhorho > p.fctrRho * rho))) {
@@ -370,6 +394,9 @@
                     continue;
                 }
             }
+            double* const res_out = res_pin + kResSlot * (nchk & 1);
+            const double* const res_in = res_host + kResSlot * (nchk & 1);
+            int look = 0;
             if (!fused) {
                 linear_solve(rho, sigma);
                 {
@@ -382,9 +409,16 @@
                     gemv_rows<T>(st, P, NP, x, Px, nullptr, T(1), T(0), 0, NP, 0, NP, 0);
                     gemv_cols_partial<T>(st, A, NP, y, nullptr, T(1), T(0), part, NP, MP, NP);
                     colsum<T>(st, part, NP, part_tiles, nullptr, T(0), nullptr, T(0), Aty, NP);
-                    CheckScalars cs{p.epsAbs, p.epsRel, epsAdmm, rho, rhorho, p.adptRho, convFlag};
-                    check_convergence<T>(st, (int)n, (int)m, Ax, Px, Aty, q, x, xp, z, zp, scratch, res_dev, cs);
-                }
+                    CheckScalars cs{p.epsAbs, p.epsRel, epsAdmm, rho, rhorho, p.adptRho, convFlag, p.fctrRho};
+                    check_convergence<T>(st, (int)n, (int)m, Ax, Px, Aty, q, x, xp, z, zp, scratch, res_out, cs, 0, BatchStride(), nullptr, nullptr,
+                                         nullptr, abort_dev);
+                }
+            } else if (!check) {
+                if (changed && rhs_slabs > 0) {
+                    ProfScope ps(prof, cat_atw, 2);
+                    rhs_slabs = gemv_cols_partial<T>(st, A, NP, z, y, (T)rho, T(-1), part, NP, MP, NP);
+                }
+                plain_iteration(ii, nullptr);
             } else {
                 if (changed && rhs_slabs > 0) {
                     ProfScope ps(prof, cat_atw, 2);
@@ -396,28 +430,37 @@
                     colsum<T>(st, part, NP, rhs_slabs, x, (T)sigma, q, T(-1), tt, NP);
                 }
                 sweeps();
-                if (check) HIPC(hipMemsetAsync(scratch, 0, 16 * sizeof(unsigned long long), st));
                 {
-                    const int lvl = (prof.level == 1 && (check || ii % 50 != 38)) ? 3 : 1;
-                    ProfLaunchScope ps(prof, check ? cat_passchk : cat_pass, lvl);
-                    apass<T>(st, check, A, NP, NP, MP, xx, x, xp, z, y, l, u, (T)alpha, (T)rho, part, part2, NP, scratch);
+                    ProfLaunchScope ps(prof, cat_passchk, prof.level == 1 ? 3 : 1);
+                    apass<T>(st, true, A, NP, NP, MP, xx, x, xp, z, y, l, u, (T)alpha, (T)rho, part, part2, NP, scratch);
                 }
                 std::swap(x, xp);
                 rhs_slabs = pass_slabs;
-                if (check) {
+                if (!prev_stopped && !fac_premul) look = std::min(std::min(look_want, p.numItrConv - 1), p.numIterations - ii) & ~1;
+                {
                     ProfScope ps(prof, cat_chk, 2);
                     colsum<T>(st, part2, NP, pass_slabs, nullptr, T(0), nullptr, T(0), Aty, NP);
                     gemv_rows<T>(st, P, NP, x, Px, nullptr, T(1), T(0), 0, NP, 0, NP, 0);
-                    CheckScalars cs{p.epsAbs, p.epsRel, epsAdmm, rho, rhorho, p.adptRho, convFlag};
-                    check_convergence<T>(st, (int)n, (int)m, Ax, Px, Aty, q, x, xp, z, zp, scratch, res_dev, cs, 1);
+                    CheckScalars cs{p.epsAbs, p.epsRel, epsAdmm, rho, rhorho, p.adptRho, convFlag, p.fctrRho};
+                    check_convergence<T>(st, (int)n, (int)m, Ax, Px, Aty, q, x, xp, z, zp, scratch, res_out, cs, 1, BatchStride(), nullptr, nullptr,
+                                         stop_dev, abort_dev);
                 }
             }
             if (check) {
-                HIPC(hipMemcpyAsync(res_host, res_dev, 15 * sizeof(double), hipMemcpyDeviceToHost, st));
-                HIPC(hipStreamSynchronize(st));
+                ++nchk;
+                if (look > 0) {
+                    HIPC(hipEventRecord(check_ev, st));
+                    for (int k = 1; k <= look; ++k) plain_iteration(ii + k, stop_dev);
+                    HIPC(hipEventSynchronize(check_ev));
+                } else HIPC(hipStreamSynchronize(st));
                 prof.harvest();
-                if (sweep_gave_up(true)) return true;
-                resP = res_host[0]; resD = res_host[1]; rhorho = res_host[4]; convFlag = (int)res_host[5];
+                if (sweep_gave_up(true, res_in)) return true;
+                resP = res_in[0]; resD = res_in[1]; rhorho = res_in[4]; convFlag = (int)res_in[5];
+                prev_stopped = convFlag != QPS_CONV_NUM_ITR || (p.adptRho && ((rhorho * p.fctrRho < rho) || (rhorho > p.fctrRho * rho)));
+                if (fused && prev_stopped != (res_in[8] != 0.0))
+                    throw QpsError(QPS_ERR_HIP, "convergence check: the device's stop word disagrees with the host's loop-top tests");
+                if (prev_stopped) { if (fused) zero_buffers(st, {{stop_dev, sizeof(int)}}); }
+                else ii += look;
                 if (convFlag != QPS_CONV_NUM_ITR) break;
             }
         }
@@ -507,7 +550,7 @@
     T *x = nullptr, *xp = nullptr, *xres = nullptr, *z = nullptr, *y = nullptr, *xx = nullptr, *tt = nullptr, *yv = nullptr, *part = nullptr,
       *part2 = nullptr, *part_tmp = nullptr, *sw_part = nullptr, *Px = nullptr, *Aty = nullptr;
     int* fail = nullptr; int* d_active = nullptr; double *d_rho = nullptr, *d_rhorho = nullptr;
-    unsigned long long* scratch = nullptr; double* res_dev = nullptr; double* res_host = nullptr; double* stage = nullptr;
+    unsigned long long* scratch = nullptr; double* res_pin = nullptr; double* res_host = nullptr; double* stage = nullptr;
     int* h_int = nullptr; double* h_dbl = nullptr;
     bool have_AA = false; double fac_sigma = -1; int fac_nb = -1; std::vector<double> fac_rho;
     char* sb_args = nullptr; void* sb_host = nullptr;
@@ -536,8 +579,8 @@
         part = mem.dalloc<T>(part_slabs * NP, st); part2 = mem.dalloc<T>(c * slabs * NP, st); part_tmp = mem.dalloc<T>((int64_t)std::max(part_tiles, 1) * NP, st);
         const int sw_slabs = sweep_fused_slabs<T>(NP, count); sw_part = mem.dalloc<T>(c * std::max(sw_slabs, 1) * NP, st);
         fail = mem.dalloc<int>(count + 4, st); d_active = mem.dalloc<int>(count + 4, st); d_rho = mem.dalloc<double>(count + 4, st); d_rhorho = mem.dalloc<double>(count + 4, st);
-        scratch = mem.dalloc<unsigned long long>(16 * c, st); res_dev = mem.dalloc<double>(8 * c, st);
-        res_host = mem.pinned<double>(8 * c); h_int = mem.pinned<int>(count + 4); h_dbl = mem.pinned<double>(2 * (count + 4));
+        scratch = mem.dalloc<unsigned long long>(16 * c, st);
+        res_host = mem.pinned<double>(8 * c); HIPC(hipHostGetDevicePointer(reinterpret_cast<void**>(&res_pin), res_host, 0)); h_int = mem.pinned<int>(count + 4); h_dbl = mem.pinned<double>(2 * (count + 4));
         stage = mem.dalloc<double>(std::max<int64_t>((int64_t)MP * NP, nn) + 64, st);
     }
     ~BatchedDenseSolver() override {
@@ -607,6 +650,7 @@
         loader.reset();
         HIPC(hipMemsetAsync(z, 0, sizeof(T) * (size_t)count * MP, st));
         HIPC(hipMemsetAsync(y, 0, sizeof(T) * (size_t)count * MP, st));
+        HIPC(hipMemsetAsync(scratch, 0, 16 * sizeof(unsigned long long) * (size_t)count, st));
         push_state(rho, rhorho, active);
         const double t1 = now_s();
         BatchStride bsS; bsS.count = count; bsS.mat = (int64_t)NP * NP; bsS.vin = NP; bsS.vout = NP; bsS.active = d_active;
@@ -686,7 +730,6 @@
             const bool check = (ii % p.numItrConv == 0);
             colsum<T>(st, part, NP, rhs_slabs, x, (T)sigma, q, T(-1), tt, NP, bsC);
             ch.sweeps(nb, tt, yv, xx, sw_part, bsS, {&prof, cat_sweep, (prof.level == 1 && ii % 50 == 13) ? 1 : 2});
-            if (check) HIPC(hipMemsetAsync(scratch, 0, 16 * sizeof(unsigned long long) * count, st));
             {
                 ProfLaunchScope ps(prof, cat_pass, (prof.level == 1 && !check && ii % 50 == 38) ? 1 : (check ? 3 : 2));
                 apass<T>(st, check, A, NP, NP, MP, xx, x, xp, z, y, l, u, (T)alpha, T(1), part, part2, NP, scratch, pb);
@@ -698,8 +741,7 @@
                 BatchStride bsP = bsS; bsP.mat = (int64_t)NP * NP;
                 gemv_rows<T>(st, P, NP, x, Px, nullptr, T(1), T(0), 0, NP, 0, NP, 0, bsP);
                 CheckScalars cs{p.epsAbs, p.epsRel, epsAdmm, 0.0, 0.0, p.adptRho, QPS_CONV_NUM_ITR};
-                check_convergence<T>(st, (int)n, (int)m, (const T*)nullptr, Px, Aty, q, x, xp, z, z, scratch, res_dev, cs, 1, bsK, d_rho, d_rhorho);
-                HIPC(hipMemcpyAsync(res_host, res_dev, 8 * sizeof(double) * count, hipMemcpyDeviceToHost, st));
+                check_convergence<T>(st, (int)n, (int)m, (const T*)nullptr, Px, Aty, q, x, xp, z, z, scratch, res_pin, cs, 1, bsK, d_rho, d_rhorho);
                 HIPC(hipStreamSynchronize(st));
                 prof.harvest();
                 bool any_done = false;
diff --git a/quadraticprogramsolver_amd/csrc/qps_internal.h b/quadraticprogramsolver_amd/csrc/qps_internal.h
--- a/quadraticprogramsolver_amd/csrc/qps_internal.h
+++ b/quadraticprogramsolver_amd/csrc/qps_internal.h
@@ -40,12 +40,14 @@
     void begin(int cat, hipEvent_t& a) { a = get(); (void)hipEventRecord(a, st); (void)cat; }
     void end(int cat, hipEvent_t a) { hipEvent_t b = get(); (void)hipEventRecord(b, st); pending.push_back({cat, a, b}); }
     void harvest() {
+        size_t kept = 0;
         for (auto& p : pending) {
+            if (hipEventQuery(p.b) != hipSuccess) { (void)hipGetLastError(); pending[kept++] = p; continue; }
             float ms = 0; (void)hipEventElapsedTime(&ms, p.a, p.b);
             stats[p.cat].seconds += ms * 1e-3; stats[p.cat].launches += 1;
             pool.push_back(p.a); pool.push_back(p.b);
         }
-        pending.clear();
+        pending.resize(kept);
     }
     void reset() { for (auto& s : stats) { s.seconds = 0; s.launches = 0; } }
     void release_events() {
diff --git a/quadraticprogramsolver_amd/csrc/qps_kernels.h b/quadraticprogramsolver_amd/csrc/qps_kernels.h
--- a/quadraticprogramsolver_amd/csrc/qps_kernels.h
+++ b/quadraticprogramsolver_amd/csrc/qps_kernels.h
@@ -6,7 +6,9 @@
 #include <stdint.h>
 
 #include <atomic>
+#include <initializer_list>
 #include <thread>
+#include <utility>
 
 namespace qps {
 
@@ -28,7 +30,7 @@
 extern thread_local LaunchTiming g_launch_timing;
 
 
-struct BatchStride { int count = 1; int64_t mat = 0, vin = 0, vout = 0; const int* active = nullptr; };
+struct BatchStride { int count = 1; int64_t mat = 0, vin = 0, vout = 0; const int* active = nullptr; const int* stop = nullptr; };
 
 template <typename T> struct VecOf;
 template <> struct VecOf<double> { using type = double2; static constexpr int N = 2; };
@@ -51,16 +53,18 @@
 void admm_update(hipStream_t st, int NP, int MP, const T* xx, const T* zz, T* x, T* xp, T* z, T* zp, T* y,
                  const T* l, const T* u, T alpha, T rho);
 
-struct CheckScalars { double epsAbs, epsRel, epsAdmm, rho, rhorho; int adptRho; int convFlag; };
+struct CheckScalars { double epsAbs, epsRel, epsAdmm, rho, rhorho; int adptRho; int convFlag; double fctrRho; };
 template <typename T>
 void check_convergence(hipStream_t st, int n, int m, const T* Ax, const T* Px, const T* Aty, const T* q, const T* x,
-                       const T* xp, const T* z, const T* zp, unsigned long long* scratch , double* res_dev,
+                       const T* xp, const T* z, const T* zp, unsigned long long* scratch , double* res_out,
                        CheckScalars cs, int dual_only = 0, BatchStride bs = BatchStride(), const double* rho_arr = nullptr,
-                       const double* rhorho_arr = nullptr);
+                       const double* rhorho_arr = nullptr, int* stop = nullptr,
+                       const unsigned* abort_word = nullptr);
+void zero_buffers(hipStream_t st, std::initializer_list<std::pair<void*, size_t>> bufs);
 
 template <typename T> int apass_plan(int NP, int MP, int* rows_per_wg, int count = 1);
 template <typename T> int apass_max_np();
-struct PassBatch { int count = 1; int slabs = 0; const double* rho_arr = nullptr; const int* active = nullptr; int pq_me = 0; };
+struct PassBatch { int count = 1; int slabs = 0; const double* rho_arr = nullptr; const int* active = nullptr; int pq_me = 0; const int* stop = nullptr; };
 template <typename T>
 void apass(hipStream_t st, bool check, const T* A, int64_t ld, int NP, int MP, const T* xx, const T* x_old, T* x_new, T* z,
            T* y, const T* l, const T* u, T alpha, T rho, T* part, T* part2, int64_t part_ld, unsigned long long* slots,
```

After: 14720, median of 6. 1.01x the previous value.
